# 1fni/cuda-spmv-benchmark

Hardware: AMD Instinct MI355X
Metric: cg_iterations_per_second (higher is better)
Workload: dtype f64; 1 GPU; CG on the 20000x20000 5-point stencil (400000000 unknowns, 1999920000 nnz), b=1, x0=0, tol 1e-6; grid=20000, unknowns=400000000, nnz=1999920000, partition=1 row slab(s), transport=single rank (no communicator), converged=True

## Files before the change

### cuda-spmv-benchmark_amd/binding.py

```python
import ctypes as C
import os
import subprocess

import numpy as np

PKG_DIR = os.path.dirname(os.path.abspath(__file__))
LAB_LIB_PATH = os.path.join(PKG_DIR, "lib", "libspmv_amd_lab.so")
LIB_PATH = os.environ.get("SPMV_AMD_LIB") or os.path.join(PKG_DIR, "lib", "libspmv_amd.so")
if LIB_PATH == "lab":
    LIB_PATH = LAB_LIB_PATH

ENTRY_DTYPE = np.dtype([("row", np.int32), ("col", np.int32), ("value", np.float64)], align=True)
assert ENTRY_DTYPE.itemsize == 16
COMM_ID_BYTES = 256


class MatrixData(C.Structure):
    _fields_ = [("rows", C.c_int), ("cols", C.c_int), ("nnz", C.c_int), ("grid_size", C.c_int), ("entries", C.c_void_p)]


class CSRMatrix(C.Structure):
    _fields_ = [("nb_rows", C.c_int), ("nb_cols", C.c_int), ("nb_nonzeros", C.c_int), ("row_ptr", C.POINTER(C.c_int)), ("col_indices", C.POINTER(C.c_int)), ("values", C.POINTER(C.c_double))]


class ELLPACKMatrix(C.Structure):
    _fields_ = [("nb_rows", C.c_int), ("nb_cols", C.c_int), ("ell_width", C.c_int), ("grid_size", C.c_int), ("indices", C.POINTER(C.c_int)), ("nb_nonzeros", C.c_int), ("values", C.POINTER(C.c_double))]


INIT_FN = C.CFUNCTYPE(C.c_int, C.POINTER(MatrixData))
RUN_TIMED_FN = C.CFUNCTYPE(C.c_int, C.c_void_p, C.c_void_p, C.POINTER(C.c_double))
RUN_DEVICE_FN = C.CFUNCTYPE(C.c_int, C.c_void_p, C.c_void_p)
FREE_FN = C.CFUNCTYPE(None)


class SpmvOperator(C.Structure):
    _fields_ = [("name", C.c_char_p), ("init", INIT_FN), ("run_timed", RUN_TIMED_FN), ("run_device", RUN_DEVICE_FN), ("free", FREE_FN)]


class BenchmarkStats(C.Structure):
    _fields_ = [("median_ms", C.c_double), ("mean_ms", C.c_double), ("std_dev_ms", C.c_double), ("min_ms", C.c_double), ("max_ms", C.c_double), ("valid_runs", C.c_int), ("outliers_removed", C.c_int)]


class CGConfig(C.Structure):
    _fields_ = [("max_iters", C.c_int), ("tolerance", C.c_double), ("verbose", C.c_int), ("enable_detailed_timers", C.c_int)]


class CGStats(C.Structure):
    _fields_ = [("iterations", C.c_int), ("residual_norm", C.c_double), ("time_total_ms", C.c_double), ("time_spmv_ms", C.c_double), ("time_blas1_ms", C.c_double), ("time_reductions_ms", C.c_double), ("converged", C.c_int), ("solution_sum", C.c_double), ("solution_norm", C.c_double)]


CGConfigMultiGPU = CGConfig


class CGStatsMultiGPU(C.Structure):
    _fields_ = [
        ("iterations", C.c_int), ("residual_norm", C.c_double), ("time_total_ms", C.c_double), ("time_spmv_ms", C.c_double),
        ("time_blas1_ms", C.c_double), ("time_reductions_ms", C.c_double), ("time_allreduce_ms", C.c_double),
        ("time_allgather_ms", C.c_double), ("converged", C.c_int), ("time_dot_rs_initial_ms", C.c_double),
        ("time_dot_pAp_ms", C.c_double), ("time_dot_rs_new_ms", C.c_double), ("time_axpy_update_x_ms", C.c_double),
        ("time_axpy_update_r_ms", C.c_double), ("time_axpby_update_p_ms", C.c_double), ("time_initial_r_ms", C.c_double),
        ("solution_sum", C.c_double), ("solution_norm", C.c_double),
    ]


class PcgScalars(C.Structure):
    _fields_ = [("rz", C.c_double), ("pAp", C.c_double), ("alpha", C.c_double), ("beta", C.c_double), ("b_norm", C.c_double),
                ("residual", C.c_double), ("iterations", C.c_int), ("converged", C.c_int), ("breakdown", C.c_int), ("skip_update", C.c_int)]


class PcgStageArgs(C.Structure):
    _fields_ = [("n", C.c_size_t), ("b", C.c_void_p), ("Ap", C.c_void_p), ("dinv", C.c_void_p), ("r", C.c_void_p), ("p", C.c_void_p),
                ("x", C.c_void_p), ("partials", C.c_void_p), ("count", C.c_int), ("which", C.c_int), ("tol", C.c_double),
                ("hist", C.c_void_p), ("hist_cap", C.c_int)]


class MultiColumn(C.Structure):
    _fields_ = [("rr_old", C.c_double), ("pAp", C.c_double), ("alpha", C.c_double), ("beta", C.c_double), ("b_norm", C.c_double),
                ("residual", C.c_double), ("active", C.c_int), ("done", C.c_int), ("iterations", C.c_int), ("pad", C.c_int)]


class CgMultiStageArgs(C.Structure):
    _fields_ = [("mode", C.c_char_p), ("n", C.c_size_t), ("X", C.c_void_p), ("R", C.c_void_p), ("P", C.c_void_p), ("AP", C.c_void_p),
                ("cols", C.c_void_p), ("partials", C.c_void_p), ("count", C.c_longlong), ("which", C.c_int), ("tol", C.c_double),
                ("hist", C.c_void_p), ("hist_cap", C.c_int), ("xcd_run", C.c_int)]


HALO_FN = C.CFUNCTYPE(C.c_int, C.c_void_p, C.POINTER(C.c_double), C.POINTER(C.c_double), C.POINTER(C.c_double), C.POINTER(C.c_double), C.c_int)
ALLREDUCE_FN = C.CFUNCTYPE(C.c_int, C.c_void_p, C.POINTER(C.c_double), C.c_int)
GATHER_FN = C.CFUNCTYPE(C.c_int, C.c_void_p, C.POINTER(C.c_double), C.c_int, C.POINTER(C.c_double), C.POINTER(C.c_int), C.POINTER(C.c_int))
BARRIER_FN = C.CFUNCTYPE(C.c_int, C.c_void_p)

DECLARED_SYMBOLS = [
    "csr_mat", "ellpack_matrix", "build_ellpack_from_csr_local", "ensure_ellpack_structure_built", "get_operator",
    "calculate_spmv_metrics", "get_gpu_properties", "print_benchmark_metrics", "print_metrics_json", "print_metrics_csv",
    "read_matrix_type", "read_matrix_general", "read_matrix_symtogen", "load_matrix_market", "convert_csr_to_ellpack",
    "write_matrix_market_stencil5", "benchmark_with_stats", "cg_benchmark_with_stats_device",
    "cg_benchmark_with_stats_mgpu_partitioned", "export_cg_json", "export_cg_mgpu_json", "export_cg_csv",
    "spmv_amd_build_csr_struct", "spmv_amd_build_ellpack_from_csr_struct", "spmv_amd_cg_solve", "spmv_amd_cg_solve_device",
    "spmv_amd_cg_solve_mgpu_partitioned", "spmv_amd_reset_host_matrices", "spmv_amd_interior_csr_offset",
    "spmv_amd_partition_rows", "spmv_amd_device_count", "spmv_amd_set_device", "spmv_amd_current_device", "spmv_amd_stream_ceiling", "spmv_amd_stream_ceiling_mix", "spmv_amd_device_alloc", "spmv_amd_device_free",
    "spmv_amd_copy_to_device", "spmv_amd_copy_to_host", "spmv_amd_device_fill_f64", "spmv_amd_device_synchronize",
    "spmv_amd_init_stencil5_synthetic", "spmv_amd_ellpack_run_device_scaled", "spmv_amd_download_device_csr", "spmv_amd_time_run_device", "spmv_amd_operator_variant",
    "spmv_amd_operator_select_variant", "spmv_amd_cg_last_history", "spmv_amd_comm_unique_id", "spmv_amd_comm_create_rccl",
    "spmv_amd_comm_create_staged", "spmv_amd_comm_destroy", "spmv_amd_comm_set_world", "spmv_amd_comm_rank", "spmv_amd_comm_size", "spmv_amd_comm_selftest",
    "spmv_amd_comm_barrier", "spmv_amd_comm_transport", "spmv_amd_comm_transport_ranks",
    "spmv_amd_comm_mailbox_enable", "spmv_amd_comm_mailbox_prepare", "spmv_amd_comm_mailbox_connect", "spmv_amd_comm_mailbox_selftest",
    "spmv_amd_comm_mailbox_disable", "spmv_amd_comm_mailbox_ready",
    "spmv_amd_cg_slab_create", "spmv_amd_cg_slab_create_stencil5", "spmv_amd_cg_slab_set_vectors", "spmv_amd_cg_slab_solve",
    "spmv_amd_cg_slab_gather", "spmv_amd_cg_slab_loop_shape", "spmv_amd_cg_slab_history", "spmv_amd_cg_slab_spmv", "spmv_amd_cg_slab_info",
    "spmv_amd_cg_slab_time_spmv", "spmv_amd_cg_slab_set_timeline", "spmv_amd_operator_placement", "spmv_amd_cg_slab_placement", "spmv_amd_cg_slab_tile_runs", "spmv_amd_cg_slab_setup_ms", "spmv_amd_cg_slab_coefficient_form", "spmv_amd_cg_slab_uniform_tiles", "spmv_amd_cg_slab_spmv_launch_ms",  "spmv_amd_cg_release_workspace", "spmv_amd_cg_slab_timeline_names", "spmv_amd_cg_slab_timeline", "spmv_amd_cg_slab_variant", "spmv_amd_cg_slab_destroy", "spmv_amd_version", "spmv_amd_write_stencil5_values",
    "spmv_amd_blas1_axpy", "spmv_amd_blas1_axpby", "spmv_amd_blas1_axpy_dev", "spmv_amd_blas1_update_p_dev", "spmv_amd_blas1_dot",
    "spmv_amd_cg_fused_step",
    "spmv_amd_spmm_device", "spmv_amd_spmm_variant", "spmv_amd_block_to_device", "spmv_amd_block_to_host",
    "spmv_amd_cg_solve_device_multi", "spmv_amd_cg_last_history_multi", "spmv_amd_cg_multi_workspace_bytes",
    "spmv_amd_precond_create", "spmv_amd_precond_create_from_diagonal", "spmv_amd_precond_destroy", "spmv_amd_precond_kind",
    "spmv_amd_precond_inverse_diagonal", "spmv_amd_pcg_solve_device", "spmv_amd_pcg_last_history", "spmv_amd_pcg_release_workspace",
    "spmv_amd_precond_create_chebyshev", "spmv_amd_precond_chebyshev_info", "spmv_amd_precond_apply_device",
]
LAB_ONLY_SYMBOLS = ["spmv_amd_cg_slab_create_stencil5_as", "spmv_amd_cg_slab_set_option", "spmv_amd_cg_slab_tile_classes", "spmv_amd_cg_slab_block_map", "spmv_amd_pcg_stage",
                    "spmv_amd_pcg_last_step_launches", "spmv_amd_cg_multi_stage"]
DECLARED_CXX_SYMBOLS = [
    "SPMV_CSR", "SPMV_STENCIL5_CSR", "SPMV_STENCIL_HALO_MGPU", "SPMV_ELLPACK", "SPMV_STENCIL5_ELLPACK",
    "_Z16build_csr_structP10MatrixData",
    "_Z29build_ellpack_from_csr_structPK9CSRMatrixP13ELLPACKMatrixPi",
    "_Z8cg_solveP12SpmvOperatorP10MatrixDataPKdPd8CGConfigP7CGStats",
    "_Z15cg_solve_deviceP12SpmvOperatorP10MatrixDataPKdPd8CGConfigP7CGStats",
    "_Z25cg_solve_mgpu_partitionedP12SpmvOperatorP10MatrixDataPKdPd16CGConfigMultiGPUP15CGStatsMultiGPU",
]


def build(force=False):
    if force:
        subprocess.check_call(["make", "-C", PKG_DIR, "clean"], stdout=subprocess.DEVNULL)
    done = subprocess.run(["make", "-C", PKG_DIR, "-j8"], stdout=subprocess.PIPE, stderr=subprocess.STDOUT, text=True)
    if done.returncode != 0:
        raise RuntimeError(f"building libspmv_amd.so failed (make exit {done.returncode}); compiler output:\n{done.stdout[-8000:]}")
    for path in (LIB_PATH, LAB_LIB_PATH):
        if not os.path.exists(path):
            raise RuntimeError(f"{os.path.basename(path)} was not produced by the build")


_lib = None


def lib():
    global _lib
    if _lib is not None:
        return _lib
    if not os.path.exists(LIB_PATH):
        raise RuntimeError(f"{LIB_PATH} is missing: run `python -c 'import __graft_entry__ as g; g.build()'` (needs hipcc)")
    L = C.CDLL(LIB_PATH)
    L.get_operator.restype = C.POINTER(SpmvOperator)
    L.get_operator.argtypes = [C.c_char_p]
    L.spmv_amd_version.restype = C.c_char_p
    L.spmv_amd_operator_variant.restype = C.c_char_p
    L.spmv_amd_operator_variant.argtypes = [C.c_char_p]
    L.spmv_amd_operator_select_variant.argtypes = [C.c_char_p, C.c_char_p]
    L.spmv_amd_device_alloc.restype = C.c_void_p
    L.spmv_amd_device_alloc.argtypes = [C.c_size_t]
    L.spmv_amd_device_free.argtypes = [C.c_void_p]
    L.spmv_amd_blas1_axpy.argtypes = [C.c_size_t, C.c_double, C.c_void_p, C.c_void_p]
    L.spmv_amd_blas1_axpby.argtypes = [C.c_size_t, C.c_double, C.c_void_p, C.c_double, C.c_void_p, C.c_void_p]
    L.spmv_amd_blas1_axpy_dev.argtypes = [C.c_size_t, C.c_double, C.c_void_p, C.c_void_p, C.c_int]
    L.spmv_amd_blas1_update_p_dev.argtypes = [C.c_size_t, C.c_void_p, C.c_double, C.c_void_p]
    L.spmv_amd_blas1_dot.argtypes = [C.c_size_t, C.c_void_p, C.c_void_p, C.POINTER(C.c_double)]
    L.spmv_amd_cg_fused_step.argtypes = [C.c_int, C.c_size_t, C.POINTER(C.c_double), C.c_void_p, C.c_void_p, C.c_void_p, C.c_int, C.POINTER(C.c_double)]
    L.spmv_amd_current_device.argtypes = [C.c_char_p, C.c_int]
    L.spmv_amd_stream_ceiling.restype = C.c_double
    L.spmv_amd_stream_ceiling.argtypes = [C.c_size_t, C.c_int, C.c_int, C.POINTER(C.c_float)]
    L.spmv_amd_stream_ceiling_mix.restype = C.c_double
    L.spmv_amd_stream_ceiling_mix.argtypes = [C.c_int, C.c_size_t, C.c_int, C.c_int, C.POINTER(C.c_float)]
    L.spmv_amd_copy_to_device.argtypes = [C.c_void_p, C.c_void_p, C.c_size_t]
    L.spmv_amd_copy_to_host.argtypes = [C.c_void_p, C.c_void_p, C.c_size_t]
    L.spmv_amd_device_fill_f64.argtypes = [C.c_void_p, C.c_size_t, C.c_double]
    L.spmv_amd_init_stencil5_synthetic.argtypes = [C.c_char_p, C.c_int]
    L.spmv_amd_download_device_csr.argtypes = [C.c_char_p, C.c_void_p, C.c_void_p, C.c_void_p]
    L.spmv_amd_ellpack_run_device_scaled.argtypes = [C.c_char_p, C.c_void_p, C.c_void_p, C.c_double, C.c_double]
    L.spmv_amd_time_run_device.argtypes = [C.c_char_p, C.c_void_p, C.c_void_p, C.c_int, C.POINTER(C.c_float)]
    L.spmv_amd_cg_solve.argtypes = [C.POINTER(SpmvOperator), C.POINTER(MatrixData), C.c_void_p, C.c_void_p, C.POINTER(CGConfig), C.POINTER(CGStats)]
    L.spmv_amd_cg_solve_device.argtypes = L.spmv_amd_cg_solve.argtypes
    L.spmv_amd_cg_solve_mgpu_partitioned.argtypes = [C.POINTER(MatrixData), C.c_void_p, C.c_void_p, C.POINTER(CGConfig), C.POINTER(CGStatsMultiGPU)]
    L.spmv_amd_cg_last_history.argtypes = [C.c_void_p, C.c_int]
    L.spmv_amd_comm_unique_id.argtypes = [C.c_void_p]
    L.spmv_amd_comm_create_rccl.restype = C.c_void_p
    L.spmv_amd_comm_create_rccl.argtypes = [C.c_int, C.c_int, C.c_void_p]
    L.spmv_amd_comm_create_staged.restype = C.c_void_p
    L.spmv_amd_comm_create_staged.argtypes = [C.c_int, C.c_int, HALO_FN, ALLREDUCE_FN, GATHER_FN, BARRIER_FN, C.c_void_p]
    L.spmv_amd_comm_destroy.argtypes = [C.c_void_p]
    L.spmv_amd_comm_set_world.argtypes = [C.c_void_p]
    L.spmv_amd_comm_rank.argtypes = [C.c_void_p]
    L.spmv_amd_comm_size.argtypes = [C.c_void_p]
    L.spmv_amd_comm_selftest.argtypes = [C.c_void_p]
    L.spmv_amd_comm_barrier.argtypes = [C.c_void_p]
    L.spmv_amd_comm_mailbox_enable.argtypes = [C.c_void_p]
    L.spmv_amd_comm_mailbox_prepare.argtypes = [C.c_void_p, C.c_void_p]
    L.spmv_amd_comm_mailbox_connect.argtypes = [C.c_void_p, C.c_void_p, C.c_int]
    L.spmv_amd_comm_mailbox_selftest.argtypes = [C.c_void_p, C.c_int]
    L.spmv_amd_comm_mailbox_disable.argtypes = [C.c_void_p]
    L.spmv_amd_comm_mailbox_ready.argtypes = [C.c_void_p]
    L.spmv_amd_comm_transport.restype = C.c_char_p
    L.spmv_amd_comm_transport.argtypes = [C.c_void_p]
    L.spmv_amd_comm_transport_ranks.argtypes = [C.c_void_p]
    if hasattr(L, "spmv_amd_cg_slab_create_stencil5_as"):
        L.spmv_amd_cg_slab_create_stencil5_as.restype = C.c_void_p
        L.spmv_amd_cg_slab_create_stencil5_as.argtypes = [C.c_int, C.c_int, C.c_int, C.c_void_p]
        L.spmv_amd_cg_slab_set_option.argtypes = [C.c_void_p, C.c_char_p, C.c_longlong]
        L.spmv_amd_cg_slab_set_option.restype = C.c_int
        L.spmv_amd_cg_slab_tile_classes.argtypes = [C.c_void_p, C.c_void_p, C.c_longlong]
        L.spmv_amd_cg_slab_tile_classes.restype = C.c_longlong
        L.spmv_amd_cg_slab_block_map.argtypes = [C.c_void_p, C.c_int, C.c_void_p, C.c_longlong]
        L.spmv_amd_cg_slab_block_map.restype = C.c_longlong
        L.spmv_amd_pcg_stage.argtypes = [C.c_char_p, C.c_char_p, C.POINTER(PcgStageArgs), C.POINTER(PcgScalars)]
        L.spmv_amd_pcg_stage.restype = C.c_int
        L.spmv_amd_pcg_last_step_launches.argtypes = []
        L.spmv_amd_pcg_last_step_launches.restype = C.c_int
        L.spmv_amd_cg_multi_stage.argtypes = [C.c_char_p, C.c_int, C.POINTER(CgMultiStageArgs)]
        L.spmv_amd_cg_multi_stage.restype = C.c_int
    L.spmv_amd_cg_slab_create.restype = C.c_void_p
    L.spmv_amd_cg_slab_create.argtypes = [C.POINTER(MatrixData), C.c_void_p]
    L.spmv_amd_cg_slab_create_stencil5.restype = C.c_void_p
    L.spmv_amd_cg_slab_create_stencil5.argtypes = [C.c_int, C.c_void_p]
    L.spmv_amd_cg_slab_set_vectors.argtypes = [C.c_void_p, C.c_void_p, C.c_void_p]
    L.spmv_amd_cg_slab_solve.argtypes = [C.c_void_p, C.POINTER(CGConfig), C.POINTER(CGStatsMultiGPU)]
    L.spmv_amd_cg_slab_gather.argtypes = [C.c_void_p, C.c_void_p]
    L.spmv_amd_cg_slab_history.argtypes = [C.c_void_p, C.c_void_p, C.c_int]
    L.spmv_amd_cg_slab_spmv.argtypes = [C.c_void_p, C.c_void_p, C.c_void_p]
    L.spmv_amd_cg_slab_info.argtypes = [C.c_void_p, C.POINTER(C.c_int), C.POINTER(C.c_int), C.POINTER(C.c_int)]
    L.spmv_amd_cg_slab_time_spmv.argtypes = [C.c_void_p, C.c_int, C.POINTER(C.c_float)]
    L.spmv_amd_cg_slab_destroy.argtypes = [C.c_void_p]
    L.spmv_amd_cg_slab_set_timeline.argtypes = [C.c_void_p, C.c_int]
    L.spmv_amd_cg_slab_set_timeline.restype = None
    L.spmv_amd_cg_slab_timeline_names.restype = C.c_char_p
    L.spmv_amd_cg_slab_timeline.argtypes = [C.c_void_p, C.c_void_p, C.c_int]
    L.spmv_amd_cg_slab_variant.restype = C.c_char_p
    L.spmv_amd_cg_slab_variant.argtypes = [C.c_void_p]
    L.spmv_amd_cg_slab_coefficient_form.argtypes = [C.c_void_p]
    L.spmv_amd_cg_slab_coefficient_form.restype = C.c_int
    L.spmv_amd_cg_slab_uniform_tiles.argtypes = [C.c_void_p, C.POINTER(C.c_longlong), C.POINTER(C.c_longlong)]
    L.spmv_amd_cg_slab_uniform_tiles.restype = C.c_int
    L.spmv_amd_cg_slab_loop_shape.restype = C.c_char_p
    L.spmv_amd_cg_slab_loop_shape.argtypes = [C.c_void_p]
    L.load_matrix_market.argtypes = [C.c_char_p, C.POINTER(MatrixData)]
    L.write_matrix_market_stencil5.argtypes = [C.c_int, C.c_char_p]
    L.spmv_amd_write_stencil5_values.argtypes = [C.c_int, C.c_char_p, C.c_char_p, C.c_char_p]
    L.read_matrix_type.argtypes = [C.c_char_p]
    L.spmv_amd_partition_rows.argtypes = [C.c_int, C.c_int, C.c_int, C.POINTER(C.c_int), C.POINTER(C.c_int)]
    L.benchmark_with_stats.argtypes = [RUN_TIMED_FN, C.c_void_p, C.c_void_p, C.c_int, C.POINTER(BenchmarkStats)]
    _lib = L
    return L


def is_lab():
    return hasattr(lib(), "spmv_amd_cg_slab_set_option")


def use_lab():
    import importlib.util

    spec = importlib.util.spec_from_file_location("spmv_amd_binding_lab", os.path.abspath(__file__))
    mod = importlib.util.module_from_spec(spec)
    spec.loader.exec_module(mod)
    mod.LIB_PATH = LAB_LIB_PATH
    return mod


def require_gpu():
    if lib().spmv_amd_device_count() < 1:
        raise RuntimeError("no HIP device visible: libspmv_amd has no CPU path")


def current_device():
    buf = C.create_string_buffer(64)
    dev = lib().spmv_amd_current_device(buf, 64)
    return dev, buf.value.decode()


def stream_ceiling(rows, warmup=3, reps=20, mix="stencil5"):
    require_gpu()
    ms = (C.c_float * reps)()
    nbytes = lib().spmv_amd_stream_ceiling_mix({"stencil5": 0, "csr": 1, "ellpack": 2, "read-only": 3}[mix], int(rows), int(warmup), int(reps), ms)
    if nbytes <= 0:
        raise RuntimeError("spmv_amd_stream_ceiling failed")
    return np.array(ms[:], dtype=np.float64), nbytes


def csr_mat():
    return CSRMatrix.in_dll(lib(), "csr_mat")


def ellpack_matrix():
    return ELLPACKMatrix.in_dll(lib(), "ellpack_matrix")


class HostMatrix:

    def __init__(self, entries, rows, cols, grid_size=-1):
        self.entries = np.ascontiguousarray(entries, dtype=ENTRY_DTYPE)
        self.c = MatrixData(int(rows), int(cols), len(self.entries), int(grid_size), self.entries.ctypes.data)

    @property
    def ptr(self):
        return C.byref(self.c)


def load_matrix_market(path):
    m = MatrixData()
    rc = lib().load_matrix_market(os.fsencode(path), C.byref(m))
    if rc != 0:
        raise IOError(f"load_matrix_market({path}) -> {rc}")
    e = np.ctypeslib.as_array((C.c_byte * (16 * m.nnz)).from_address(m.entries)).view(ENTRY_DTYPE).copy()
    C.CDLL(None).free(C.c_void_p(m.entries))
    return HostMatrix(e, m.rows, m.cols, m.grid_size)


def read_matrix_symtogen(path):
    m = MatrixData()
    rows, cols, nnz, full = C.c_int(), C.c_int(), C.c_int(), C.c_int()
    rp, ci, va = C.POINTER(C.c_int)(), C.POINTER(C.c_int)(), C.POINTER(C.c_double)()
    lib().read_matrix_symtogen(C.byref(m), os.fsencode(path), C.byref(rows), C.byref(cols), C.byref(nnz), C.byref(rp), C.byref(ci),
                               C.byref(va), C.byref(full))
    if not m.entries:
        raise IOError(f"read_matrix_symtogen({path}) failed")
    out = (rows.value, cols.value, nnz.value, full.value, np.ctypeslib.as_array(rp, shape=(rows.value + 1,)).copy(),
           np.ctypeslib.as_array(ci, shape=(full.value,)).copy(), np.ctypeslib.as_array(va, shape=(full.value,)).copy(),
           np.ctypeslib.as_array((C.c_byte * (16 * m.nnz)).from_address(m.entries)).view(ENTRY_DTYPE).copy())
    libc = C.CDLL(None)
    for ptr in (rp, ci, va, C.c_void_p(m.entries)):
        libc.free(ptr)
    return out


def host_csr_arrays():
    m = csr_mat()
    rp = np.ctypeslib.as_array(m.row_ptr, shape=(m.nb_rows + 1,)).copy()
    ci = np.ctypeslib.as_array(m.col_indices, shape=(m.nb_nonzeros,)).copy()
    va = np.ctypeslib.as_array(m.values, shape=(m.nb_nonzeros,)).copy()
    return rp, ci, va


def host_ell_arrays():
    m = ellpack_matrix()
    n = m.nb_rows * m.ell_width
    return m.ell_width, np.ctypeslib.as_array(m.indices, shape=(n,)).copy(), np.ctypeslib.as_array(m.values, shape=(n,)).copy()


def partition_rows(n, world, rank):
    off, nl = C.c_int(), C.c_int()
    lib().spmv_amd_partition_rows(n, world, rank, C.byref(off), C.byref(nl))
    return off.value, nl.value


class DeviceVector:
    def __init__(self, count, fill=None):
        self.count = int(count)
        self.ptr = lib().spmv_amd_device_alloc(self.count * 8)
        if fill is not None:
            lib().spmv_amd_device_fill_f64(self.ptr, self.count, float(fill))

    @classmethod
    def from_host(cls, a):
        a = np.ascontiguousarray(a, dtype=np.float64)
        v = cls(len(a))
        lib().spmv_amd_copy_to_device(v.ptr, a.ctypes.data, a.nbytes)
        return v
# ... 346 lines not shown
                    t = torch.zeros(counts[r], dtype=torch.float64)
                    dist.recv(t, r)
                    out[displs[r]:displs[r] + counts[r]] = t.numpy()
            else:
                dist.send(mine, 0)
            return 0

        def barrier_cb(user):
            dist.barrier()
            return 0

        return cls.staged(rank, world, halo_cb, allreduce_cb, gather_cb, barrier_cb)

    def selftest(self):
        return lib().spmv_amd_comm_selftest(self.handle)

    def barrier(self):
        return lib().spmv_amd_comm_barrier(self.handle)

    def mailbox_enable(self):
        return lib().spmv_amd_comm_mailbox_enable(self.handle) == 1

    def mailbox_prepare(self):
        buf = C.create_string_buffer(64)
        return buf.raw if lib().spmv_amd_comm_mailbox_prepare(self.handle, buf) == 0 else None

    def mailbox_connect(self, handles):
        blob = b"".join(handles)
        return lib().spmv_amd_comm_mailbox_connect(self.handle, C.create_string_buffer(blob, len(blob)), len(handles)) == 0

    def mailbox_selftest(self, rounds=8):
        return lib().spmv_amd_comm_mailbox_selftest(self.handle, int(rounds))

    def mailbox_ready(self):
        return lib().spmv_amd_comm_mailbox_ready(self.handle) == 1

    def mailbox_disable(self):
        lib().spmv_amd_comm_mailbox_disable(self.handle)

    def transport(self):
        return lib().spmv_amd_comm_transport(self.handle).decode()

    def transport_ranks(self):
        return lib().spmv_amd_comm_transport_ranks(self.handle)

    @classmethod
    def staged(cls, rank, world, halo, allreduce, gather=None, barrier=None):
        cbs = (HALO_FN(halo), ALLREDUCE_FN(allreduce), GATHER_FN(gather) if gather else GATHER_FN(), BARRIER_FN(barrier) if barrier else BARRIER_FN())
        h = lib().spmv_amd_comm_create_staged(rank, world, cbs[0], cbs[1], cbs[2], cbs[3], None)
        if not h:
            raise RuntimeError("spmv_amd_comm_create_staged failed")
        return cls(h, cbs)

    @staticmethod
    def unique_id():
        buf = C.create_string_buffer(COMM_ID_BYTES)
        lib().spmv_amd_comm_unique_id(buf)
        return buf.raw

    def destroy(self):
        if self.handle:
            lib().spmv_amd_comm_destroy(self.handle)
            self.handle = None


class CgSlab:

    def __init__(self, handle, n_rows):
        if not handle:
            raise RuntimeError("spmv_amd_cg_slab_create failed")
        self.h = handle
        self.n_rows = n_rows
        off, nl, nz = C.c_int(), C.c_int(), C.c_int()
        lib().spmv_amd_cg_slab_info(self.h, C.byref(off), C.byref(nl), C.byref(nz))
        self.row_offset, self.n_local, self.local_nnz = off.value, nl.value, nz.value

    @classmethod
    def from_matrix(cls, host_matrix, comm=None):
        require_gpu()
        return cls(lib().spmv_amd_cg_slab_create(host_matrix.ptr, comm.handle if comm else None), host_matrix.c.rows)

    @classmethod
    def stencil5(cls, n, comm=None):
        require_gpu()
        return cls(lib().spmv_amd_cg_slab_create_stencil5(int(n), comm.handle if comm else None), n * n)

    @classmethod
    def stencil5_as(cls, n, as_rank, as_world, comm):
        require_gpu()
        if not is_lab():
            raise RuntimeError("stand-in slabs exist in the LAB build only (binding.use_lab(), lib/libspmv_amd_lab.so)")
        return cls(lib().spmv_amd_cg_slab_create_stencil5_as(int(n), int(as_rank), int(as_world), comm.handle), n * n)

    def set_vectors(self, b=None, x0=None):
        b = None if b is None else np.ascontiguousarray(b, dtype=np.float64)
        x0 = None if x0 is None else np.ascontiguousarray(x0, dtype=np.float64)
        lib().spmv_amd_cg_slab_set_vectors(self.h, None if b is None else b.ctypes.data, None if x0 is None else x0.ctypes.data)

    def solve(self, max_iters=1000, tol=1e-6, verbose=0, timers=0):
        cfg = CGConfig(max_iters, tol, verbose, timers)
        st = CGStatsMultiGPU()
        rc = lib().spmv_amd_cg_slab_solve(self.h, C.byref(cfg), C.byref(st))
        if rc != 0:
            raise RuntimeError(f"cg_slab_solve -> {rc}")
        return st

    def history(self, cap=1001):
        h = np.zeros(cap, dtype=np.float64)
        count = lib().spmv_amd_cg_slab_history(self.h, h.ctypes.data, cap)
        return h[: min(count, cap)].copy()

    def gather(self):
        x = np.zeros(self.n_rows, dtype=np.float64)
        lib().spmv_amd_cg_slab_gather(self.h, x.ctypes.data)
        return x

    def spmv(self, x_full):
        x_full = np.ascontiguousarray(x_full, dtype=np.float64)
        y = np.zeros(self.n_local, dtype=np.float64)
        lib().spmv_amd_cg_slab_spmv(self.h, x_full.ctypes.data, y.ctypes.data)
        return y

    def variant(self):
        return lib().spmv_amd_cg_slab_variant(self.h).decode()

    def coefficient_form(self):
        return int(lib().spmv_amd_cg_slab_coefficient_form(self.h))

    def uniform_tiles(self):
        u, t = C.c_longlong(), C.c_longlong()
        lib().spmv_amd_cg_slab_uniform_tiles(self.h, C.byref(u), C.byref(t))
        return int(u.value), int(t.value)

    def tile_classes(self):
        if not is_lab():
            raise RuntimeError("the tile class map is read through the LAB build only (binding.use_lab(), lib/libspmv_amd_lab.so)")
        count = int(lib().spmv_amd_cg_slab_tile_classes(self.h, None, 0))
        if count == 0:
            return None
        out = np.zeros(count, dtype=np.uint8)
        lib().spmv_amd_cg_slab_tile_classes(self.h, out.ctypes.data, count)
        return out

    def block_map(self, which):
        if not is_lab():
            raise RuntimeError("the block maps are read through the LAB build only (binding.use_lab(), lib/libspmv_amd_lab.so)")
        count = int(lib().spmv_amd_cg_slab_block_map(self.h, int(which), None, 0))
        if count == 0:
            return None
        out = np.zeros(count, dtype=np.uint8)
        lib().spmv_amd_cg_slab_block_map(self.h, int(which), out.ctypes.data, count)
        return out

    def set_block_rows(self, rows):
        self.set_option("block_rows", rows)

    def loop_shape(self):
        return lib().spmv_amd_cg_slab_loop_shape(self.h).decode()

    def timeline_solve(self, max_iters=1000, tol=1e-6):
        lib().spmv_amd_cg_slab_set_timeline(self.h, 1)
        try:
            st = self.solve(max_iters=max_iters, tol=tol)
        finally:
            lib().spmv_amd_cg_slab_set_timeline(self.h, 0)
        names = lib().spmv_amd_cg_slab_timeline_names().decode().split(",")
        v = np.zeros(len(names), dtype=np.float64)
        count = lib().spmv_amd_cg_slab_timeline(self.h, v.ctypes.data, len(v))
        return st, ({k: float(x) for k, x in zip(names, v)} if count == len(names) else {})

    def placement(self):
        v = (C.c_double * 4)()
        lib().spmv_amd_cg_slab_placement.argtypes = [C.c_void_p, C.c_void_p, C.c_int]
        if lib().spmv_amd_cg_slab_placement(self.h, v, 4) != 4:
            return None
        return {"kind": "coefficient candidates", "candidates": int(v[1]), "spmv_ms_before": float(v[2]), "spmv_ms_kept": float(v[3])}

    def setup_ms(self):
        v = (C.c_double * 5)()
        lib().spmv_amd_cg_slab_setup_ms.argtypes = [C.c_void_p, C.c_void_p, C.c_int]
        lib().spmv_amd_cg_slab_setup_ms(self.h, v, 5)
        return dict(zip(("matrix_to_hbm", "streams_and_vectors", "verify_and_plans", "coefficient_placement", "tile_runs"), (float(x) for x in v)))

    def tile_runs(self):
        v = (C.c_double * 4)()
        lib().spmv_amd_cg_slab_tile_runs.argtypes = [C.c_void_p, C.c_void_p, C.c_int]
        if lib().spmv_amd_cg_slab_tile_runs(self.h, v, 4) != 4:
            return None
        return {"rule": int(v[0]), "kept": int(v[1]), "spmv_ms_rule": float(v[2]), "spmv_ms_kept": float(v[3])}

    def spmv_launch_ms(self):
        out = (C.c_float * 1024)()
        lib().spmv_amd_cg_slab_spmv_launch_ms.argtypes = [C.c_void_p, C.c_void_p, C.c_int]
        count = lib().spmv_amd_cg_slab_spmv_launch_ms(self.h, out, 1024)
        return np.array(out[:min(count, 1024)], dtype=np.float64)

    def set_option(self, name, value):
        if not is_lab():
            raise RuntimeError("slab options exist in the LAB build only (binding.use_lab(), lib/libspmv_amd_lab.so)")
        if lib().spmv_amd_cg_slab_set_option(self.h, name.encode(), int(value)) != 0:
            raise ValueError(f"unknown slab option {name!r}")

    def time_spmv(self, reps):
        ms = (C.c_float * reps)()
        lib().spmv_amd_cg_slab_time_spmv(self.h, reps, ms)
        return np.array(ms[:], dtype=np.float64)

    def destroy(self):
        if self.h:
            lib().spmv_amd_cg_slab_destroy(self.h)
            self.h = None
```

### cuda-spmv-benchmark_amd/csrc/cg_kernels.hip

```cpp
#include "kernels.hpp"

#include <stdlib.h>

#include "reduce_device.hpp"
#include "spmv_amd/hip_check.h"
#include "stream_device.hpp"

namespace spmv_amd {
namespace {

constexpr int kBlock = kReduceBlock;
constexpr int kStream = 64;

#define SPMV_AMD_STREAM_LOOP(n)                                                     \
    const size_t pairs = (n) >> 1;                                                  \
    const size_t i = (size_t)blockIdx.x * kStream + threadIdx.x;                    \
    if (i < pairs)

__device__ __forceinline__ void block_partial(double acc, double* __restrict__ partials) {
    acc = wave_sum(acc);
    if (threadIdx.x == 0) partials[blockIdx.x] = acc;
}

__global__ __launch_bounds__(kStream) void fill_kernel(double* __restrict__ d, size_t n, double value) {
    SPMV_AMD_STREAM_LOOP(n) {
        d2 v = {value, value};
        reinterpret_cast<d2*>(d)[i] = v;
    }
    if ((n & 1) && blockIdx.x == 0 && threadIdx.x == 0) d[n - 1] = value;
}

__global__ __launch_bounds__(kStream) void axpy_kernel(size_t n, double a, const double* __restrict__ x,
                                                      double* __restrict__ y) {
    SPMV_AMD_STREAM_LOOP(n) {
        const d2 xv = load_once(x, i);
        d2 yv = load_once(y, i);
        yv.x = fma(a, xv.x, yv.x);
        yv.y = fma(a, xv.y, yv.y);
        store_once(y, i, yv);
    }
    if ((n & 1) && blockIdx.x == 0 && threadIdx.x == 0) y[n - 1] = fma(a, x[n - 1], y[n - 1]);
}

__global__ __launch_bounds__(kStream) void axpby_kernel(size_t n, double a, const double* __restrict__ x,
                                                       double b, const double* y, double* z) {
    SPMV_AMD_STREAM_LOOP(n) {
        const d2 xv = load_once(x, i);
        const d2 yv = load_once(y, i);
        d2 zv;
        zv.x = fma(a, xv.x, b * yv.x);
        zv.y = fma(a, xv.y, b * yv.y);
        store_once(z, i, zv);
    }
    if ((n & 1) && blockIdx.x == 0 && threadIdx.x == 0) z[n - 1] = fma(a, x[n - 1], b * y[n - 1]);
}

template <bool kSubtract>
__global__ __launch_bounds__(kStream) void axpy_dev_kernel(size_t n, const double* __restrict__ d_a,
                                                          const double* __restrict__ x,
                                                          double* __restrict__ y) {
    const double a = kSubtract ? -(*d_a) : *d_a;
    SPMV_AMD_STREAM_LOOP(n) {
        const d2 xv = load_once(x, i);
        d2 yv = load_once(y, i);
        yv.x = fma(a, xv.x, yv.x);
        yv.y = fma(a, xv.y, yv.y);
        store_once(y, i, yv);
    }
    if ((n & 1) && blockIdx.x == 0 && threadIdx.x == 0) y[n - 1] = fma(a, x[n - 1], y[n - 1]);
}

__global__ __launch_bounds__(kStream) void update_p_dev_kernel(size_t n, const double* __restrict__ r,
                                                              const double* __restrict__ d_b,
                                                              double* __restrict__ p) {
    const double b = *d_b;
    SPMV_AMD_STREAM_LOOP(n) {
        const d2 rv = load_once(r, i);
        d2 pv = load_once(p, i);
        pv.x = fma(b, pv.x, rv.x);
        pv.y = fma(b, pv.y, rv.y);
        reinterpret_cast<d2*>(p)[i] = pv;
    }
    if ((n & 1) && blockIdx.x == 0 && threadIdx.x == 0) p[n - 1] = fma(b, p[n - 1], r[n - 1]);
}

__global__ __launch_bounds__(kStream) void dot_partials_kernel(size_t n, const double* __restrict__ x,
                                                              const double* __restrict__ y,
                                                              double* __restrict__ partials) {
    double acc = 0.0;
    SPMV_AMD_STREAM_LOOP(n) {
        const d2 xv = load_once(x, i);
        const d2 yv = load_once(y, i);
        acc = fma(xv.x, yv.x, acc);
        acc = fma(xv.y, yv.y, acc);
    }
    if ((n & 1) && blockIdx.x == 0 && threadIdx.x == 0) acc = fma(x[n - 1], y[n - 1], acc);
    block_partial(acc, partials);
}


__global__ __launch_bounds__(kBlock) void reduce_one_launch_kernel(const double* __restrict__ partials, int count, int slice,
                                                                   const double* extra, int extra_count, ReduceStage stage, ReduceTail tail) {
    __shared__ double s[kBlock];
    __shared__ int s_last;
    if (tail.skip_flag != nullptr && *tail.skip_flag != 0) {
        reduce_skipped(tail, blockIdx.x == 0);
        return;
    }
    reduce_slice_block(partials, count, slice, (int)blockIdx.x, (int)gridDim.x, reinterpret_cast<const unsigned long long*>(extra), extra_count,
                       (int)gridDim.x, stage, tail, s, &s_last);
}

__global__ __launch_bounds__(kBlock) void reduce_single_kernel(const double* __restrict__ partials, int count, const double* __restrict__ extra,
                                                               int extra_count, ReduceTail tail) {
    __shared__ double s[kBlock];
    if (tail.skip_flag != nullptr && *tail.skip_flag != 0) {
        reduce_skipped(tail, true);
        return;
    }
    block_tree(strided_sum(partials, 0, count), s);
    const double slice_sum = s[0];
    __syncthreads();
    reduce_finish(1 + extra_count, [&](int i) { return i == 0 ? slice_sum : extra[i - 1]; }, s, tail);
}

__global__ void scalar_divide_kernel(const double* num, const double* den, double* out) {
    if (threadIdx.x == 0 && blockIdx.x == 0) *out = (*num) / (*den);
}

__global__ void check_convergence_kernel(const double* rr_new, double b_norm, double tol,
                                         int* converged, double* residual) {
    if (threadIdx.x == 0 && blockIdx.x == 0) {
        *residual = sqrt(*rr_new);
        const double rel = (*residual) / b_norm;
        *converged = (rel < tol) ? 1 : 0;
    }
}


__global__ __launch_bounds__(kStream) void cg_init_residual_kernel(size_t n, const double* __restrict__ b,
                                                                  const double* __restrict__ Ap,
                                                                  double* __restrict__ r,
                                                                  double* __restrict__ p,
                                                                  double* __restrict__ partials) {
    double acc = 0.0;
    SPMV_AMD_STREAM_LOOP(n) {
        const d2 bv = load_once(b, i);
        const d2 av = load_once(Ap, i);
        d2 rv;
        rv.x = fma(-1.0, av.x, bv.x);
        rv.y = fma(-1.0, av.y, bv.y);
        store_once(r, i, rv);
        reinterpret_cast<d2*>(p)[i] = rv;
        acc = fma(rv.x, rv.x, acc);
        acc = fma(rv.y, rv.y, acc);
    }
    if ((n & 1) && blockIdx.x == 0 && threadIdx.x == 0) {
        const double rv = fma(-1.0, Ap[n - 1], b[n - 1]);
        r[n - 1] = rv;
        p[n - 1] = rv;
        acc = fma(rv, rv, acc);
    }
    block_partial(acc, partials);
}

__global__ __launch_bounds__(kStream) void cg_update_r_kernel(size_t n, const CgScalars* __restrict__ s,
                                                             const double* __restrict__ Ap,
                                                             double* __restrict__ r,
                                                             double* __restrict__ partials, int reverse) {
    const unsigned block = reverse ? gridDim.x - 1 - blockIdx.x : blockIdx.x;
    const size_t pairs = n >> 1;
    const size_t i = (size_t)block * kStream + threadIdx.x;
    d2 av = {0.0, 0.0}, rv = {0.0, 0.0};
    if (i < pairs) {
        av = load_once(Ap, i);
        rv = load_once(r, i);
    }
    const int converged = s->converged;
    const double rr_old = s->rr_old, pAp = s->pAp;
    if (converged) return;
    const double alpha = rr_old / pAp;
    double acc = 0.0;
    if (i < pairs) {
        rv.x = fma(-alpha, av.x, rv.x);
        rv.y = fma(-alpha, av.y, rv.y);
        store_once(r, i, rv);
        acc = fma(rv.x, rv.x, acc);
        acc = fma(rv.y, rv.y, acc);
    }
    if ((n & 1) && block == 0 && threadIdx.x == 0) {
        const double rl = fma(-alpha, Ap[n - 1], r[n - 1]);
        r[n - 1] = rl;
        acc = fma(rl, rl, acc);
    }
    acc = wave_sum(acc);
    if (threadIdx.x == 0) partials[block] = acc;
}

__device__ __forceinline__ double direction(double r, double beta, double p, int fma_form) {
    return fma_form ? fma(beta, p, r) : fma(1.0, r, beta * p);
}

__global__ __launch_bounds__(kStream) void cg_update_px_kernel(size_t n, const CgScalars* __restrict__ s,
                                                              const double* __restrict__ r,
                                                              double* __restrict__ p,
                                                              const double* x_in, double* x, int iteration,
                                                              int reverse, int fma_form) {
    if (s->iterations != iteration) return;
    const bool advance = s->converged == 0;
    const double alpha = s->alpha, beta = s->beta;
    const unsigned block = reverse ? gridDim.x - 1 - blockIdx.x : blockIdx.x;
    const size_t pairs = n >> 1;
    const size_t i = (size_t)block * kStream + threadIdx.x;
    if (i < pairs) {
        d2 pv = load_once(p, i);
        d2 xv = load_once(x_in, i);
        xv.x = fma(alpha, pv.x, xv.x);
        xv.y = fma(alpha, pv.y, xv.y);
        store_once(x, i, xv);
        if (advance) {
            const d2 rv = load_once(r, i);
            pv.x = direction(rv.x, beta, pv.x, fma_form);
            pv.y = direction(rv.y, beta, pv.y, fma_form);
            reinterpret_cast<d2*>(p)[i] = pv;
        }
    }
    if ((n & 1) && block == 0 && threadIdx.x == 0) {
        const double pv = p[n - 1];
        x[n - 1] = fma(alpha, pv, x_in[n - 1]);
        if (advance) p[n - 1] = direction(r[n - 1], beta, pv, fma_form);
    }
}

__global__ void cg_scalars_init_kernel(CgScalars* s, double* history) {
    if (threadIdx.x != 0 || blockIdx.x != 0) return;
    s->rr_old = s->rr_new;
    s->rr_ring[0] = s->rr_new;
    s->b_norm = sqrt(s->rr_new);
    s->residual = s->b_norm;
    s->converged = 0;
    s->iterations = 0;
    if (history != nullptr && s->max_history > 0) history[0] = s->b_norm;
}

__global__ void cg_scalars_step_kernel(CgScalars* s, double tol, double* history, int* host_record,
                                       int sequence, double* alpha_ring, int ring_slots) {
    if (threadIdx.x != 0 || blockIdx.x != 0) return;
    cg_scalars_step(s, tol, history, host_record, sequence, alpha_ring, ring_slots);
}

struct DirectionArgs {
    StepArgs step;
    int iteration;
    const double* r;
    const double* p_in;
    double* p_out;
    size_t bulk_lo, bulk_pairs;
    unsigned edge_blocks;
    int reverse, fma_form;
};
__global__ __launch_bounds__(kStream) void cg_direction_kernel(DirectionArgs a, EdgeRows e, ReduceStage stage) {
    CgScalars* s = a.step.scalars;
    const bool edge_block = blockIdx.x < a.edge_blocks;
    const size_t pairs_a = e.count_a >> 1, edge_pairs = (e.count_a + e.count_b) >> 1, shift = (e.second - e.count_a) >> 1;
    size_t at = 0;
    bool live_lane = false;
    if (edge_block) {
        const size_t i = (size_t)blockIdx.x * kStream + threadIdx.x;
        live_lane = i < edge_pairs;
        at = i < pairs_a ? i : i + shift;
    } else {
        const unsigned bulk_blocks = gridDim.x - a.edge_blocks, logical = blockIdx.x - a.edge_blocks;
        const size_t i = (size_t)(a.reverse ? bulk_blocks - 1 - logical : logical) * kStream + threadIdx.x;
        live_lane = i < a.bulk_pairs;
        at = (a.bulk_lo >> 1) + i;
    }
    const int was_converged = __hip_atomic_load(&s->converged, __ATOMIC_RELAXED, __HIP_MEMORY_SCOPE_AGENT);
    const double rr_new = s->rr_new, rr_prev = s->rr_ring[(a.iteration - 1) & 1], b_norm = s->b_norm;
    const int stop_at = cg_stop_at(s);
    if (blockIdx.x == 0 && threadIdx.x == 0 && a.step.host_record != nullptr)
        cg_scalars_step(s, a.step.tol, a.step.history, a.step.host_record, a.step.sequence, a.step.alpha_ring, a.step.ring_slots);
    const bool live = was_converged == 0 && !cg_converging(rr_new, b_norm, a.step.tol, stop_at, a.iteration);
    if (live && live_lane) {
        const double beta = rr_new / rr_prev;
        const d2 rv = load_once(a.r, at);
        d2 pv = load_once(a.p_in, at);
        pv.x = direction(rv.x, beta, pv.x, a.fma_form);
        pv.y = direction(rv.y, beta, pv.y, a.fma_form);
        if (edge_block) {
            __hip_atomic_store(reinterpret_cast<unsigned long long*>(a.p_out + 2 * at), (unsigned long long)__double_as_longlong(pv.x),
                               __ATOMIC_RELAXED, __HIP_MEMORY_SCOPE_AGENT);
            __hip_atomic_store(reinterpret_cast<unsigned long long*>(a.p_out + 2 * at + 1), (unsigned long long)__double_as_longlong(pv.y),
                               __ATOMIC_RELAXED, __HIP_MEMORY_SCOPE_AGENT);
        } else {
            reinterpret_cast<d2*>(a.p_out)[at] = pv;
        }
    }
    if (edge_block) {
        asm volatile("s_waitcnt vmcnt(0)" ::: "memory");
        if (threadIdx.x == 0) {
            const unsigned drawn = __hip_atomic_fetch_add(stage.ticket, 1u, __ATOMIC_RELAXED, __HIP_MEMORY_SCOPE_AGENT);
            if (drawn == a.edge_blocks - 1) {
                __hip_atomic_store(stage.ticket, 0u, __ATOMIC_RELAXED, __HIP_MEMORY_SCOPE_AGENT);
                __hip_atomic_store(stage.edges_ready, (unsigned)a.step.sequence, __ATOMIC_RELAXED, __HIP_MEMORY_SCOPE_AGENT);
            }
        }
    }
}

__global__ void edges_wait_kernel(const unsigned* ready, unsigned sequence, long long timeout_ticks, int* late) {
    if (threadIdx.x != 0 || blockIdx.x != 0) return;
    const long long t0 = wall_clock64();
    while ((int)(__hip_atomic_load(ready, __ATOMIC_RELAXED, __HIP_MEMORY_SCOPE_AGENT) - sequence) < 0) {
        if (wall_clock64() - t0 > timeout_ticks) {
            __hip_atomic_store(late, 3, __ATOMIC_RELAXED, __HIP_MEMORY_SCOPE_SYSTEM);
            break;
        }
        __builtin_amdgcn_s_sleep(8);
    }
}

__global__ __launch_bounds__(kStream) void cg_update_p_ring_kernel(size_t n, const CgScalars* __restrict__ s,
                                                                   const double* __restrict__ r,
                                                                   const double* __restrict__ p_in,
                                                                   double* __restrict__ p_out, int iteration,
                                                                   int reverse, int fma_form) {
    if (s->iterations != iteration || s->converged != 0) return;
    const double beta = s->beta;
    const unsigned block = reverse ? gridDim.x - 1 - blockIdx.x : blockIdx.x;
    const size_t pairs = n >> 1;
    const size_t i = (size_t)block * kStream + threadIdx.x;
    if (i < pairs) {
        const d2 rv = load_once(r, i);
        d2 pv = load_once(p_in, i);
        pv.x = direction(rv.x, beta, pv.x, fma_form);
        pv.y = direction(rv.y, beta, pv.y, fma_form);
        reinterpret_cast<d2*>(p_out)[i] = pv;
    }
    if ((n & 1) && block == 0 && threadIdx.x == 0) p_out[n - 1] = direction(r[n - 1], beta, p_in[n - 1], fma_form);
}

template <int K>
__device__ __forceinline__ void flush_chunk(d2& xv, const RingSlots& ring, const double* __restrict__ alphas, int slots,
                                            int& slot, size_t i) {
    d2 pv[K];
    double a[K];
#pragma unroll
    for (int u = 0; u < K; ++u) {
        const int sl = (slot + u) % slots;
        pv[u] = load_once(ring.p[sl], i);
        a[u] = alphas[sl];
    }
#pragma unroll
    for (int u = 0; u < K; ++u) {
// ... 207 lines not shown
```

### cuda-spmv-benchmark_amd/csrc/cg_slab.hip

```cpp
#include <math.h>
#include <stdlib.h>
#include <string.h>

#include <algorithm>
#include <atomic>
#include <chrono>
#include <mutex>
#include <thread>
#include <vector>

#include "comm.hpp"
#include "device_runtime.hpp"
#include "multi_rhs.hpp"
#include "solve_common.hpp"
#include "stencil_geometry.hpp"
#include "trace_ranges.hpp"
#include "watchdog.hpp"

using namespace spmv_amd;

namespace spmv_amd {
std::vector<double>& last_cg_history();
}

struct SpmvAmdCgSlab {
    SpmvAmdComm* comm = nullptr;
    int part_rank = 0, part_world = 1;
    SpmvOperator* op = nullptr;
    bool op_failed = false;
    FusedSpmv fused;
    const char* label = nullptr;
    bool device_form = false;
    int n = 0, grid = -1, row_offset = 0, n_local = 0, halo = 0;
    bool has_prev = false, has_next = false;
    DeviceCsr A;
    double *x = nullptr, *x0 = nullptr, *r = nullptr, *Ap = nullptr, *b = nullptr;
    double* x0_alloc = nullptr;
    double* vec_arena = nullptr;
    double* planes_alloc = nullptr;
    size_t planes_doubles = 0, planes_s_offset = 0;
    SymPlanes planes;
    bool planes_on = false;
    unsigned char* tile_classes = nullptr;
    size_t tile_class_count = 0;
    long long tiles_uniform = 0, tiles_total = 0;
    double quintuple[5] = {0.0, 0.0, 0.0, 0.0, 0.0};
    bool stream_everywhere = false;
    unsigned char *block_map_whole = nullptr, *block_map_interior = nullptr;
    bool spmv_with_dot = false;
    const SymPlanes* sym() const { return planes_on ? &planes : nullptr; }
    std::vector<double> placement;
    std::vector<double> tile_runs;
    double setup_ms[5] = {0.0, 0.0, 0.0, 0.0, 0.0};
    bool setup_trials = true;
    double* p_alloc = nullptr;
    double* p = nullptr;
    size_t slot_doubles = 0, slot_lead = 0;
    std::vector<double*> ring_alloc;
    std::vector<double*> ring;
    int ring_slots = 1;
    double* d_alpha_ring = nullptr;
    double* partials_spmv = nullptr;
    double* partials_blas = nullptr;
    double* reduce_stage = nullptr;
    ReduceScratch scratch() const { return ReduceScratch{reduce_stage}; }
    CgScalars* d_s = nullptr;
    double* d_hist = nullptr;
    int hist_cap = 0;
    struct Poll { int sequence; int converged; int iterations; int progress; int halo_late; }* h_poll = nullptr;
    unsigned* d_halo_flag = nullptr;
    unsigned halo_sequence = 0;
#ifdef SPMV_AMD_LAB
    int stop_at = 0;
    int test_wedge_overlapped_exchange = 0;
    bool guess_far_always = false;
#endif
    const PeerMailbox* reduce_mailbox = nullptr;
    int* spmv_progress = nullptr;
    int spmv_progress_value = 0;
    const char* enqueued_stage = "";
    int enqueued_iteration = -1;
    hipStream_t compute = nullptr, side = nullptr;
    bool owns_streams = true;
    hipEvent_t ev_p_ready = nullptr, ev_halo_done = nullptr;
    bool timeline_on = false;
    std::vector<hipEvent_t> tl_compute, tl_side;
    hipEvent_t tl_after_interior = nullptr;
    std::vector<double> timeline_us;
    LaunchShape shape;
    Stencil5Plan plan_whole, plan_interior, plan_head, plan_tail;
    int partials_cap = 0;
    int spmv_split_at = -1;
    const char* variant_name = "";
    bool fused_dot = false;
    bool fuse_init_residual = false;
    std::vector<double> history;
    std::vector<hipEvent_t> spmv_ev;
    int spmv_event_stride = 7;
    int spmv_event_phase = 0;
    bool roctx_always = false;
    bool no_overlap = false;
    bool selfcheck = false, selfcheck_late = false;
    double wait_limit_s = 0.0;
    bool late_bulk = false;
    bool late_predict = true;
    bool run_ahead = true;
    size_t lead_rows = (size_t)1 << 25;
    int poll_sequence = 0;
    double last_spmv_ms = 0.0;
    int last_spmv_launches = 0;
    std::vector<float> last_spmv_each;
};

namespace {
constexpr int kTimelineMarks = 7;
const char* const kTimelineNames =
    "iterations,solve_ms,initial_residual_us,spmv_interior_us,halo_wait_and_boundary_rows_us,reduce_pAp_and_allreduce_us,"
    "update_r_us,reduce_rr_allreduce_and_scalar_step_us,direction_update_us,gap_before_next_iteration_us,iteration_us,"
    "halo_exchange_on_side_stream_us,final_x_flush_us,direction_updates";
}

namespace {

void adopt_operator(SpmvAmdCgSlab* s, SpmvOperator* op) {
    s->op = op;
    s->fused = fused_spmv_of(op);
    s->fused_dot = s->fused.partials > 0;
    s->fuse_init_residual = s->fused_dot && s->fused.can_init;
    s->variant_name = s->fused_dot ? "operator/fused-launch" : "operator/run_device+dot";
    if (s->fused.partials > s->partials_cap) {
        device_release(s->partials_spmv);
        s->partials_cap = s->fused.partials;
        s->partials_spmv = device_alloc<double>((size_t)s->partials_cap);
        HIP_CHECK(hipMemset(s->partials_spmv, 0, (size_t)s->partials_cap * sizeof(double)));
    }
}

void place_coefficients(SpmvAmdCgSlab* s);
void tune_tile_runs(SpmvAmdCgSlab* s);

SymPlanes plane_view(const SpmvAmdCgSlab* s, const double* base) {
    SymPlanes v;
    v.ce = base;
    v.s = base + s->planes_s_offset;
    v.cls = s->stream_everywhere ? nullptr : s->tile_classes;
    v.w = s->quintuple[0], v.c = s->quintuple[1], v.e = s->quintuple[2], v.n = s->quintuple[3], v.s5 = s->quintuple[4];
    return v;
}

bool may_take_planes(const SpmvAmdCgSlab* s) {
    const int n = s->grid;
    return s->op == nullptr && n >= 2 && n >= s->shape.knobs.rowlds_min_grid && s->n_local > 0 && s->n_local % n == 0 &&
           s->row_offset % n == 0;
}

void classify_tiles(SpmvAmdCgSlab* s) {
    const int n = s->grid;
    const int gfirst = s->row_offset / n, rows = s->n_local / n;
    const int lo = std::max(gfirst, 1), hi = std::min(gfirst + rows, n - 1);
    if (hi <= lo || n < 3) return;
    const int col_tiles = rowlds_col_tiles(n);
    s->tiles_total = (long long)(hi - lo) * col_tiles;
    const long long lr = (long long)(lo + (hi - lo) / 2 - gfirst) * n + n / 2;
    int first = 0;
    HIP_CHECK(hipMemcpy(&first, s->A.view.row_ptr + lr, sizeof(int), hipMemcpyDeviceToHost));
    double row[5];
    HIP_CHECK(hipMemcpy(row, s->A.view.values + first, sizeof(row), hipMemcpyDeviceToHost));
    const double q[5] = {row[1], row[2], row[3], row[0], row[4]};
    memcpy(s->quintuple, q, sizeof(q));
    s->tile_class_count = (size_t)rows * col_tiles;
    const size_t bytes = s->tile_class_count;
    s->tile_classes = device_try_alloc<unsigned char>(bytes);
    if (s->tile_classes == nullptr) {
        s->tile_class_count = 0;
        return;
    }
    unsigned long long* d_count = device_alloc<unsigned long long>(1);
    HIP_CHECK(hipMemsetAsync(s->tile_classes, 0, bytes, s->compute));
    HIP_CHECK(hipMemsetAsync(d_count, 0, sizeof(unsigned long long), s->compute));
    launch_classify_tiles(s->A.view, q, s->tile_classes, d_count, s->compute);
    unsigned long long h_count = 0;
    HIP_CHECK(hipMemcpyAsync(&h_count, d_count, sizeof(h_count), hipMemcpyDeviceToHost, s->compute));
    HIP_CHECK(hipStreamSynchronize(s->compute));
    device_release(d_count);
    s->tiles_uniform = (long long)h_count;
}

void attach_block_maps(SpmvAmdCgSlab* s) {
    s->plan_whole.block_map = s->block_map_whole;
    s->plan_interior.block_map = s->block_map_interior;
}

void build_block_maps(SpmvAmdCgSlab* s) {
    HIP_CHECK(hipStreamSynchronize(s->compute));
    device_release(s->block_map_whole);
    device_release(s->block_map_interior);
    if (s->tile_classes != nullptr) {
        const auto map_of = [&](const Stencil5Plan& p) -> unsigned char* {
            const int blocks = rowlds_block_tiles(p);
            unsigned char* map = blocks > 0 ? device_try_alloc<unsigned char>((size_t)blocks) : nullptr;
            if (map != nullptr) launch_block_map(s->tile_classes, p, map, s->compute);
            return map;
        };
        s->block_map_whole = map_of(s->plan_whole);
        s->block_map_interior = map_of(s->plan_interior);
        HIP_CHECK(hipStreamSynchronize(s->compute));
    }
    attach_block_maps(s);
}

void settle_planes(SpmvAmdCgSlab* s) {
    if (s->planes_alloc == nullptr) return;
    bool keep = s->A.view.verified_stencil && s->fuse_init_residual;
    if (keep) {
        launch_fill_sym_planes(s->A.view, s->planes_alloc, s->planes_alloc + s->planes_s_offset, s->compute);
        s->planes = plane_view(s, s->planes_alloc);
        int* d_flag = device_alloc<int>(1);
        HIP_CHECK(hipMemsetAsync(d_flag, 0, sizeof(int), s->compute));
        launch_verify_sym_planes(s->A.view, s->planes, d_flag, s->compute);
        int h_flag = 1;
        HIP_CHECK(hipMemcpyAsync(&h_flag, d_flag, sizeof(int), hipMemcpyDeviceToHost, s->compute));
        HIP_CHECK(hipStreamSynchronize(s->compute));
        device_release(d_flag);
        keep = h_flag == 0;
    }
    if (!keep) {
        device_release(s->planes_alloc);
        s->planes = SymPlanes{};
    } else {
        classify_tiles(s);
        s->planes = plane_view(s, s->planes_alloc);
        build_block_maps(s);
    }
    s->planes_on = keep;
}

double setup_phase_ms(std::chrono::steady_clock::time_point& from) {
    HIP_CHECK(hipDeviceSynchronize());
    const auto now = std::chrono::steady_clock::now();
    const double ms = std::chrono::duration<double, std::milli>(now - from).count();
    from = now;
    return ms;
}

void make_common(SpmvAmdCgSlab* s) {
    const size_t nl = (size_t)s->n_local;
    auto phase = std::chrono::steady_clock::now();
    const bool whole_grid_probe = s->comm->self_neighbour && s->part_world == 1;
    s->has_prev = s->comm->exchanges_halos() && (s->part_rank > 0 || whole_grid_probe);
    s->has_next = s->comm->exchanges_halos() && (s->part_rank < s->part_world - 1 || whole_grid_probe);
    s->halo = s->comm->exchanges_halos() ? s->grid : 0;
    s->A.view.halo_before = s->has_prev ? s->halo : 0;
    s->A.view.halo_after = s->has_next ? s->halo : 0;
    if (s->op != nullptr) {
        s->compute = nullptr;
        s->side = nullptr;
        s->owns_streams = false;
    } else {
        HIP_CHECK(hipStreamCreateWithFlags(&s->compute, hipStreamNonBlocking));
        HIP_CHECK(hipStreamCreateWithFlags(&s->side, hipStreamNonBlocking));
    }
    HIP_CHECK(hipEventCreateWithFlags(&s->ev_p_ready, hipEventDisableTiming));
    HIP_CHECK(hipEventCreateWithFlags(&s->ev_halo_done, hipEventDisableTiming));
    s->shape = current_launch_shape();
    constexpr size_t kLeadUnit = 512;
    const size_t lead = s->halo == 0 ? 0 : ((size_t)s->halo + kLeadUnit - 1) / kLeadUnit * kLeadUnit;
    const size_t slot_doubles = lead + nl + (size_t)s->halo + 2;
    s->slot_doubles = slot_doubles;
    s->slot_lead = lead;
    s->x = device_alloc<double>(nl);
    s->b = device_alloc<double>(nl);
    s->x0_alloc = device_alloc<double>(slot_doubles);
    s->x0 = s->x0_alloc + lead;
    HIP_CHECK(hipMemset(s->x0_alloc, 0, slot_doubles * sizeof(double)));
    {
        int want = kMaxRingSlots;
        const char* forced = getenv("SPMV_AMD_P_RING");
        if (forced) want = atoi(forced);
        want = want < 1 ? 1 : (want > kMaxRingSlots ? kMaxRingSlots : want);
        constexpr size_t k2MiB = (size_t)2 << 20, k4KiB = 4096;
        const size_t pitch = ((slot_doubles * sizeof(double) + k2MiB - 1) / k2MiB * k2MiB + k4KiB) / sizeof(double);
        size_t free_b = 0, total_b = 0;
        HIP_CHECK(hipMemGetInfo(&free_b, &total_b));
        const size_t keep_free = (size_t)4 << 30;
        const size_t per_slot = pitch * sizeof(double);
        const int asked = want;
        const size_t fixed = 3 * per_slot;
        if (may_take_planes(s)) {
            const size_t ce = (2 * nl + kLeadUnit - 1) / kLeadUnit * kLeadUnit;
            const size_t halo_lead = ((size_t)s->grid + kLeadUnit - 1) / kLeadUnit * kLeadUnit;
            const size_t bytes = (ce + halo_lead + nl) * sizeof(double);
            if (free_b > bytes + keep_free + fixed + 3 * per_slot) {
                s->planes_alloc = device_try_alloc<double>(ce + halo_lead + nl);
                if (s->planes_alloc != nullptr) {
                    s->planes_doubles = ce + halo_lead + nl;
                    s->planes_s_offset = ce + halo_lead;
                    HIP_CHECK(hipMemGetInfo(&free_b, &total_b));
                }
            }
        }
        const size_t budget = s->op != nullptr ? free_b / 4 : (free_b > keep_free + fixed ? free_b - keep_free - fixed : 0);
        while (want > 1 && (size_t)(want - 1) * per_slot > budget) --want;
        if (want < asked && want < 4) want = 1;
        s->vec_arena = device_alloc<double>((size_t)(2 + want) * pitch);
        HIP_CHECK(hipMemset(s->vec_arena, 0, (size_t)(2 + want) * pitch * sizeof(double)));
        s->r = s->vec_arena;
        s->Ap = s->vec_arena + pitch;
        s->ring_alloc.clear();
        s->ring.clear();
        for (int k = 0; k < want; ++k) {
            double* a = s->vec_arena + (size_t)(2 + k) * pitch;
            s->ring_alloc.push_back(a);
            s->ring.push_back(a + lead);
        }
        s->p_alloc = s->ring_alloc[0];
        s->p = s->ring[0];
        s->ring_slots = want;
        s->d_alpha_ring = device_alloc<double>(kMaxRingSlots);
        HIP_CHECK(hipMemset(s->d_alpha_ring, 0, kMaxRingSlots * sizeof(double)));
    }
    if (const char* v = getenv("SPMV_AMD_NO_OVERLAP")) s->no_overlap = v[0] == '1';
#ifdef SPMV_AMD_LAB
    if (const char* v = getenv("SPMV_AMD_TEST_WEDGE_OVERLAPPED_EXCHANGE")) s->test_wedge_overlapped_exchange = atoi(v);
#endif
    if (const char* v = getenv("SPMV_AMD_ROCTX")) s->roctx_always = v[0] == '1';
    s->late_bulk = nl >= 100000000;
    s->partials_blas = device_alloc<double>(dot_scratch_doubles(nl));
    HIP_CHECK(hipMemset(s->partials_blas, 0, dot_scratch_doubles(nl) * sizeof(double)));
    s->reduce_stage = reduce_scratch_alloc();
    s->d_halo_flag = device_alloc<unsigned>(1);
    HIP_CHECK(hipMemset(s->d_halo_flag, 0, sizeof(unsigned)));
    s->d_s = device_alloc<CgScalars>(1);
    HIP_CHECK(hipMemset(s->d_s, 0, sizeof(CgScalars)));
    HIP_CHECK(hipHostMalloc((void**)&s->h_poll, sizeof(*s->h_poll), hipHostMallocCoherent | hipHostMallocMapped));
    memset(s->h_poll, 0, sizeof(*s->h_poll));
    if (s->op != nullptr) {
        adopt_operator(s, s->op);
        launch_fill(s->b, nl, 1.0, s->compute);
        launch_fill(s->x0, nl, 0.0, s->compute);
        HIP_CHECK(hipDeviceSynchronize());
        return;
    }
    s->setup_ms[1] = setup_phase_ms(phase);
    s->A.verify_stencil(s->compute);
    {
        const SlabCsr& A = s->A.view;
        const int lo = s->has_prev ? s->halo : 0, hi = s->n_local - (s->has_next ? s->halo : 0);
        const auto plan = [&](int a, int b) { return plan_stencil5(A, a, b > a ? b : a, Stencil5Variant::Auto, s->shape); };
        s->plan_whole = plan(0, s->n_local);
        s->plan_interior = plan(lo, hi);
        s->plan_head = plan(0, lo);
        s->plan_tail = plan(hi, s->n_local);
        const int whole = s->plan_whole.partials;
        const int split = (hi > lo ? s->plan_interior.partials : 0) + (lo > 0 ? s->plan_head.partials : 0) +
                          (hi < s->n_local ? s->plan_tail.partials : 0);
        s->partials_cap = whole > split ? whole : split;
        s->partials_spmv = device_alloc<double>((size_t)s->partials_cap);
        HIP_CHECK(hipMemset(s->partials_spmv, 0, (size_t)s->partials_cap * sizeof(double)));
        s->variant_name = s->plan_whole.name;
        s->fused_dot = s->plan_whole.variant != Stencil5Variant::RowGeneric;
        const auto rowlds = [&](const Stencil5Plan& p) { return p.last_row <= p.first_row || p.variant == Stencil5Variant::RowLds; };
        s->fuse_init_residual = s->plan_whole.variant == Stencil5Variant::RowLds && rowlds(s->plan_interior) && rowlds(s->plan_head) && rowlds(s->plan_tail);
    }
    settle_planes(s);
    s->setup_ms[2] = setup_phase_ms(phase);
    if (s->setup_trials) place_coefficients(s);
    s->setup_ms[3] = setup_phase_ms(phase);
    if (s->setup_trials) tune_tile_runs(s);
    launch_fill(s->b, nl, 1.0, s->compute);
    launch_fill(s->x0, nl, 0.0, s->compute);
    s->setup_ms[4] = setup_phase_ms(phase);
}

bool wants_coefficient_placement(size_t n_local) { return n_local >= ((size_t)16 << 20) && placement_candidates() > 1; }

void place_coefficients(SpmvAmdCgSlab* s) {
    const size_t nl = (size_t)s->n_local;
    if (s->op != nullptr || !wants_coefficient_placement(nl) || s->ring.size() < 4 || s->A.values == nullptr) return;
    hipStream_t q = s->compute;
    const bool nothing_streamed = s->planes_on && s->tiles_total > 0 && s->tiles_uniform == s->tiles_total && !s->stream_everywhere;
    const bool planes = s->planes_on;
    const size_t count = planes ? s->planes_doubles : (size_t)s->A.view.nnz_local;
    const double* early = s->ring[1];
    const double* late = s->ring[s->ring.size() - 3];
    launch_fill(s->ring[1], nl, 1.0, q);
    launch_fill(s->ring[s->ring.size() - 3], nl, 1.0, q);
    HIP_CHECK(hipMemsetAsync(&s->d_s->converged, 0, sizeof(int), q));
    EventTimer timer;
    double* const original = planes ? s->planes_alloc : s->A.values;
    const auto point_at = [&](double* values) {
        if (planes) s->planes = plane_view(s, values);
        else s->A.view.values = values;
    };
    auto cost = [&](double* values) {
        point_at(values);
        double total = 0.0;
        for (const double* x : {early, late}) {
            float ms[3];
            for (int i = 0; i < 4; ++i) {
                timer.begin(q);
                (void)launch_stencil5_spmv(s->A.view, s->plan_whole, x, s->Ap, 1.0, s->fused_dot ? s->partials_spmv : nullptr, nullptr, false, q,
                                           nullptr, s->sym());
                timer.end(q);
                const float t = timer.elapsed_ms();
                if (i > 0) ms[i - 1] = t;
            }
            std::sort(ms, ms + 3);
            total += ms[1];
        }
        point_at(original);
        return 0.5 * total;
    };
    int tried = 0;
    double before = 0.0, after = 0.0;
    double* best = device_alloc_best_of<double>(count, 0, [&](double* cand) {
        if (cand != original && !nothing_streamed) HIP_CHECK(hipMemcpyAsync(cand, original, count * sizeof(double), hipMemcpyDeviceToDevice, q));
        const double ms = cost(cand);
        if (cand == original) before = ms;
        return ms;
    }, &tried, nullptr, original, false);
    after = best == original ? before : cost(best);
    HIP_CHECK(hipStreamSynchronize(q));
    const bool moved = best != original && after < 0.99 * before;
    if (moved && nothing_streamed) {
        HIP_CHECK(hipMemcpyAsync(best, original, count * sizeof(double), hipMemcpyDeviceToDevice, q));
        HIP_CHECK(hipStreamSynchronize(q));
    }
    if (best != original) {
        if (!moved) device_release(best);
        else if (planes) device_release(s->planes_alloc), s->planes_alloc = best;
        else s->A.replace_values(best);
    }
    s->A.view.values = s->A.values;
    if (planes) s->planes = plane_view(s, s->planes_alloc);
    for (double* a : s->ring_alloc) HIP_CHECK(hipMemsetAsync(a, 0, s->slot_doubles * sizeof(double), q));
    HIP_CHECK(hipStreamSynchronize(q));
    s->placement = {0.0, (double)tried, before, moved ? after : before};
}

void tune_tile_runs(SpmvAmdCgSlab* s) {
    if (s->op != nullptr || s->ring.size() < 2) return;
    const size_t nl = (size_t)s->n_local;
    hipStream_t q = s->compute;
    double* x = s->ring[1];
    launch_fill(x, nl, 1.0, q);
    HIP_CHECK(hipMemsetAsync(&s->d_s->converged, 0, sizeof(int), q));
    double rec[4] = {0, 0, 0, 0};
    const int run = tune_rowlds_xcd_run(s->A.view, s->shape, x, s->Ap, s->fused_dot ? s->partials_spmv : nullptr, q, rec, s->sym(),
                                        s->plan_whole.block_map);
    HIP_CHECK(hipMemsetAsync(s->ring_alloc[1], 0, s->slot_doubles * sizeof(double), q));
    HIP_CHECK(hipStreamSynchronize(q));
    if (run <= 0) return;
    s->shape.knobs.rowlds_group = run;
    const int lo = s->has_prev ? s->halo : 0, hi = s->n_local - (s->has_next ? s->halo : 0);
    const auto plan = [&](int a, int b) { return plan_stencil5(s->A.view, a, b > a ? b : a, Stencil5Variant::Auto, s->shape); };
    s->plan_whole = plan(0, s->n_local);
    s->plan_interior = plan(lo, hi);
    s->plan_head = plan(0, lo);
    s->plan_tail = plan(hi, s->n_local);
    attach_block_maps(s);
    s->tile_runs.assign(rec, rec + 4);
}

double halo_wait_limit_s(const SpmvAmdCgSlab* s) {
    if (s->wait_limit_s > 0.0) return s->wait_limit_s;
    const double w = watchdog_limit_seconds();
    return w > 0.0 && w < 40.0 ? 0.5 * w : 20.0;
}

bool partition_ok(const SpmvAmdComm* comm, int n, int grid, int n_local) {
    if (!comm->exchanges_halos()) return true;
    if (grid <= 0) {
        fprintf(stderr, "[cg-slab] multi-GPU solve needs a stencil matrix (grid_size > 0)\n");
        return false;
    }
    if (n_local < grid) {
        fprintf(stderr, "[cg-slab] slab of %d rows is thinner than one grid row (%d)\n", n_local, grid);
        return false;
    }
    (void)n;
    return true;
}

int slab_boundary_spmv(SpmvAmdCgSlab* s, const double* in, double* part, const int* skip, hipStream_t stream,
                       const ResidualOut* init = nullptr) {
    const SlabCsr& A = s->A.view;
    const int lo = s->has_prev ? s->halo : 0;
    const int hi = s->n_local - (s->has_next ? s->halo : 0);
    double* at = part ? part + (hi > lo ? s->plan_interior.partials : 0) : nullptr;
    int used = 0;
    if (lo > 0 && hi < s->n_local && lo == A.grid_size && s->n_local - hi == A.grid_size) {
        used += launch_stencil5_spmv_first_and_last_gridrow(A, s->plan_head, s->plan_tail, in, s->Ap, 1.0, at, skip, stream, init, s->sym());
    } else {
        if (lo > 0) used += launch_stencil5_spmv(A, s->plan_head, in, s->Ap, 1.0, at, skip, false, stream, init, s->sym());
        if (hi < s->n_local)
            used += launch_stencil5_spmv(A, s->plan_tail, in, s->Ap, 1.0, at ? at + used : nullptr, skip, false, stream, init, s->sym());
    }
    return part ? used : 0;
}

void reduce_spmv_partials(SpmvAmdCgSlab* s, int used, double* d_out, const int* skip, int* progress, int progress_value, const PeerMailbox* mailbox) {
    const int first = s->spmv_split_at >= 0 && s->spmv_split_at < used ? s->spmv_split_at : used;
    launch_reduce_partials(s->partials_spmv, first, d_out, skip, s->compute, s->scratch(), progress, progress_value, mailbox,
                           s->partials_spmv + first, used - first);
}

int slab_spmv(SpmvAmdCgSlab* s, bool with_dot, bool overlap, const int* skip,
              const double* input = nullptr, hipEvent_t spmv_done = nullptr, const ResidualOut* init = nullptr) {
    const SlabCsr& A = s->A.view;
    const double* in = input ? input : s->p;
    double* part = ((with_dot && s->fused_dot) || init) ? s->partials_spmv : nullptr;
    const int lo = s->has_prev ? s->halo : 0;
    const int hi = s->n_local - (s->has_next ? s->halo : 0);
    int used = 0;
    s->spmv_split_at = -1;
    if (s->op != nullptr) {
        if (part != nullptr) {
            used = s->fused.launch(in, s->Ap, part, skip, s->shape.reverse, init, s->compute);
        } else if (s->op->run_device(in, s->Ap) != 0) {
            fprintf(stderr, "[cg] operator '%s': run_device failed\n", s->op->name);
            s->op_failed = true;
        }
        if (s->tl_after_interior) HIP_CHECK(hipEventRecord(s->tl_after_interior, s->compute));
    } else if (hi <= lo || (lo == 0 && hi == s->n_local) || (part == nullptr && !overlap)) {
        if (overlap) HIP_CHECK(hipStreamWaitEvent(s->compute, s->ev_halo_done, 0));
        used = launch_stencil5_spmv(A, s->plan_whole, in, s->Ap, 1.0, part, skip, s->shape.reverse, s->compute, init, s->sym());
        if (s->tl_after_interior) HIP_CHECK(hipEventRecord(s->tl_after_interior, s->compute));
    } else {
        used = launch_stencil5_spmv(A, s->plan_interior, in, s->Ap, 1.0, part, skip, s->shape.reverse, s->compute, init, s->sym());
        s->spmv_split_at = used;
        if (s->tl_after_interior) HIP_CHECK(hipEventRecord(s->tl_after_interior, s->compute));
        const bool fused_tail = with_dot && part != nullptr && init == nullptr && lo % A.grid_size == 0 &&
                                (s->n_local - hi) % A.grid_size == 0 && lo <= A.grid_size && s->n_local - hi <= A.grid_size;
        if (fused_tail && spmv_done) HIP_CHECK(hipEventRecord(spmv_done, s->compute));
        HaloArrival arrival;
        if (fused_tail && overlap) {
            arrival = HaloArrival{s->d_halo_flag, s->halo_sequence, (long long)(halo_wait_limit_s(s) * 1e8), &s->h_poll->halo_late};
        } else if (overlap) {
            HIP_CHECK(hipStreamWaitEvent(s->compute, s->ev_halo_done, 0));
        }
        if (fused_tail && launch_stencil5_edges_and_reduce(A, s->plan_interior, lo > 0, hi < s->n_local, in, s->Ap, 1.0, part, &s->d_s->pAp, skip,
                                                           s->scratch(), s->spmv_progress, s->spmv_progress_value, s->reduce_mailbox, s->compute,
                                                           arrival, s->sym())) {
            return used;
        }
        if (arrival.flag != nullptr) HIP_CHECK(hipStreamWaitEvent(s->compute, s->ev_halo_done, 0));
        if (fused_tail) spmv_done = nullptr;
        used += slab_boundary_spmv(s, in, part, skip, s->compute, init);
    }
    if (spmv_done) HIP_CHECK(hipEventRecord(spmv_done, s->compute));
    if (with_dot) {
        if (part)
            reduce_spmv_partials(s, used, &s->d_s->pAp, skip, s->spmv_progress, s->spmv_progress_value, s->reduce_mailbox);
        else
            launch_dot((size_t)s->n_local, s->p, s->Ap, s->partials_blas, &s->d_s->pAp, s->compute);
    }
    return used;
}

const char* query_name(hipError_t e) {
    return e == hipSuccess ? "idle (all work done)" : e == hipErrorNotReady ? "busy (work pending)" : hipGetErrorString(e);
}

void report_slab_state(void* user, FILE* out) {
    const SpmvAmdCgSlab* s = static_cast<const SpmvAmdCgSlab*>(user);
    const int seq = __atomic_load_n(&s->h_poll->sequence, __ATOMIC_ACQUIRE);
    const int prog = __atomic_load_n(&s->h_poll->progress, __ATOMIC_ACQUIRE);
    fprintf(out, "[cg-slab] rank %d (slab %d of %d, rows [%d, %d)): last work enqueued by the host: %s of iteration %d\n",
            s->comm->rank, s->part_rank, s->part_world, s->row_offset, s->row_offset + s->n_local, s->enqueued_stage,
            s->enqueued_iteration);
    fprintf(out, "[cg-slab] status records: waiting for #%d, GPU has published #%d (iterations counted %d, converged %d)\n",
            s->poll_sequence, seq, s->h_poll->iterations, s->h_poll->converged);
    const char* where = "before the local p.Ap sum: in the SpMV, or waiting for the halo rows (see the events below)";
    if (prog == 4 * s->poll_sequence + 1)
        where = "local p.Ap summed: in the all-reduce of p.Ap, the r update or the local r.r sum";
    else if (prog == 4 * s->poll_sequence + 2)
        where = "local r.r summed: in the all-reduce of r.r or the scalar step";
    if (seq != s->poll_sequence) fprintf(out, "[cg-slab] GPU progress inside that iteration: %s\n", where);
    fprintf(out, "[cg-slab] compute stream: %s; side (halo) stream: %s\n", query_name(hipStreamQuery(s->compute)),
            query_name(hipStreamQuery(s->side)));
    fprintf(out, "[cg-slab] event 'direction vector ready for the halo exchange': %s; event 'halo rows received': %s\n",
            query_name(hipEventQuery(s->ev_p_ready)), query_name(hipEventQuery(s->ev_halo_done)));
    s->comm->describe(out);
}

bool record_arrived(const SpmvAmdCgSlab* s, int sequence) {
    return (int)(__atomic_load_n(&s->h_poll->sequence, __ATOMIC_ACQUIRE) - sequence) >= 0;
}

void wait_for_record(SpmvAmdCgSlab* s, int sequence) {
    if (record_arrived(s, sequence)) return;
    WatchdogScope guard("waiting for the iteration's status record", s->comm->rank, s->enqueued_iteration,
                        report_slab_state, s);
    long spins = 0;
    while (!record_arrived(s, sequence)) {
        __builtin_ia32_pause();
        if (++spins % (1L << 20) == 0) {
            const hipError_t e = hipStreamQuery(s->compute);
            if (e != hipSuccess && e != hipErrorNotReady) HIP_CHECK(e);
            if (e == hipSuccess && !record_arrived(s, sequence)) {
                fprintf(stderr, "[cg-slab] status record missing after the stream drained\n");
                exit(EXIT_FAILURE);
            }
        }
    }
}

void exchange_halo(SpmvAmdCgSlab* s, double* v, hipStream_t stream) {
    if (!s->comm->exchanges_halos()) return;
    WatchdogScope guard("halo exchange (send/recv of the first and last grid row)", s->comm->rank, s->enqueued_iteration,
                        report_slab_state, s);
#ifdef SPMV_AMD_LAB
    while (s->test_wedge_overlapped_exchange == 1 && stream == s->side && s->side != nullptr) std::this_thread::sleep_for(std::chrono::milliseconds(200));
    if (s->test_wedge_overlapped_exchange == 2 && stream == s->side && s->side != nullptr) {
        static const double nudged = 1.001;
        HIP_CHECK(hipMemcpyAsync(s->b, &nudged, sizeof nudged, hipMemcpyHostToDevice, stream));
        s->test_wedge_overlapped_exchange = 0;
    }
    if (s->test_wedge_overlapped_exchange == 3 && stream == s->side && s->side != nullptr) return;
#endif
    s->comm->halo_exchange(s->has_prev ? v : nullptr, s->has_next ? v + (s->n_local - s->halo) : nullptr,
                           s->has_prev ? v - s->halo : nullptr, s->has_next ? v + s->n_local : nullptr, s->halo, stream);
}
void allreduce_scalar(SpmvAmdCgSlab* s, double* d_value, const char* stage) {
    if (s->comm->mailbox_ready()) {
        launch_mailbox_allreduce(s->comm, d_value, s->compute);
        return;
    }
    WatchdogScope guard(stage, s->comm->rank, s->enqueued_iteration, report_slab_state, s);
    s->comm->allreduce_sum(d_value, 1, s->compute);
}

}

namespace {
struct LoopShape {
    bool multi = false;
    bool reduce = false;
    bool separate = false;
    const PeerMailbox* mailbox = nullptr;
    bool detail = false;
    bool pipeline = false;
    bool late = false;
    int slots = 1;
    EdgeRows edges{0, 0, 0};
    size_t bulk_lo = 0, bulk_hi = 0;
};


LoopShape loop_shape(const SpmvAmdCgSlab* s, const CGConfigMultiGPU* config) {
    LoopShape L;
    const SpmvAmdComm* comm = s->comm;
    const size_t nl = (size_t)s->n_local;
    L.multi = comm->exchanges_halos();
    L.reduce = comm->collective();
    L.mailbox = (L.reduce && comm->mailbox_ready()) ? comm->d_mailbox : nullptr;
    L.separate = L.reduce && L.mailbox == nullptr;
    L.detail = config->enable_detailed_timers != 0;
    L.slots = s->ring_slots;
    L.late = s->late_bulk && !L.detail && L.slots > 1;
    constexpr size_t kAlign = 512;
    const size_t head_rows = s->has_prev ? ((size_t)s->halo + kAlign - 1) / kAlign * kAlign : 0;
    const size_t tail_start = s->has_next ? (nl - (size_t)s->halo) / kAlign * kAlign : nl;
    L.pipeline = L.multi && !L.detail && !s->no_overlap && L.slots > 1 && s->reduce_stage != nullptr && (nl % 2) == 0 &&
                 nl >= 4 * (size_t)s->halo + 4 * kAlign && head_rows < tail_start;
    if (L.pipeline) {
        L.edges = EdgeRows{head_rows, tail_start, nl - tail_start};
        L.bulk_lo = head_rows, L.bulk_hi = tail_start;
    } else {
        L.bulk_lo = 0, L.bulk_hi = nl;
    }
    return L;
}

void poison_halos(SpmvAmdCgSlab* s) {
    if (s->halo == 0 || s->op != nullptr) return;
    const size_t bytes = (size_t)s->halo * sizeof(double);
    auto both_sides = [&](double* local) {
        if (s->has_prev) HIP_CHECK(hipMemsetAsync(local - s->halo, 0xFF, bytes, s->compute));
        if (s->has_next) HIP_CHECK(hipMemsetAsync(local + s->n_local, 0xFF, bytes, s->compute));
    };
    both_sides(s->x0);
    for (double* local : s->ring) both_sides(local);
}

void verify_pipeline(SpmvAmdCgSlab* s) {
    SpmvAmdComm* comm = s->comm;
    if (s->op != nullptr || !comm->exchanges_halos()) return;
    if (s->no_overlap) return;
    const CGConfigMultiGPU few = {4, 0.0, 0, 0};
    const bool mine = loop_shape(s, &few).pipeline;
    if (comm->world == 1 && !mine) return;
    if (comm->pipeline_verdict == 0) {
        CGStatsMultiGPU st;
        s->selfcheck = true, s->selfcheck_late = false, s->wait_limit_s = 2.0;
        s->no_overlap = true;
        poison_halos(s);
        spmv_amd_cg_slab_solve(s, &few, &st);
        const std::vector<double> plain = s->history;
        s->no_overlap = false;
        poison_halos(s);
        spmv_amd_cg_slab_solve(s, &few, &st);
        poison_halos(s);
        HIP_CHECK(hipStreamSynchronize(s->compute));
        if (s->side) HIP_CHECK(hipStreamSynchronize(s->side));
        __atomic_store_n(&s->h_poll->halo_late, 0, __ATOMIC_RELEASE);
        bool finite = true;
        for (double v : plain) finite = finite && std::isfinite(v);
        if (!finite)
            fprintf(stderr, "[cg-slab] rank %d: the plain order's residual history is not finite in the creation check: the communicator's halo "
                            "exchange does not deliver this rank's neighbour rows (transport: %s)\n", comm->rank, comm->transport());
        const bool same = finite && !s->selfcheck_late && plain.size() == s->history.size() && plain.size() == 5 &&
                          memcmp(plain.data(), s->history.data(), plain.size() * sizeof(double)) == 0;
        s->selfcheck = false, s->selfcheck_late = false, s->wait_limit_s = 0.0;
        double votes[2] = {same ? 0.0 : 1.0, mine ? 1.0 : 0.0};
        if (!same)
            fprintf(stderr, "[cg-slab] rank %d: the overlapped pipeline did NOT reproduce the plain order's residual history in the creation check\n", comm->rank);
        if (comm->world > 1) {
            double* d = device_alloc<double>(2);
            upload(d, votes, 2);
            WatchdogScope guard("creation check: all-reduce of the ranks' verdicts", comm->rank, -1, report_slab_state, s);
            comm->allreduce_sum(d, 2, s->compute);
            HIP_CHECK(hipStreamSynchronize(s->compute));
            download(votes, d, 2);
            device_release(d);
        }
        if (votes[0] != 0.0 || votes[1] != 0.0) comm->pipeline_verdict = votes[0] == 0.0 ? 1 : -1;
        if (comm->pipeline_verdict < 0 && comm->rank == 0)
            fprintf(stderr, "[cg-slab] %g rank(s) refused the overlapped pipeline: every solve on this communicator runs the plain order "
                            "(halo exchange on the compute stream, the reference's own)\n", votes[0]);
    }
    if (comm->pipeline_verdict < 0) s->no_overlap = true;
}

SpmvAmdCgSlab* create_from_matrix(MatrixData* mat, SpmvAmdComm* comm, bool setup_trials) {
    if (comm == nullptr) comm = self_comm();
    if (mat->rows != mat->cols) {
        fprintf(stderr, "[cg-slab] CG needs a square matrix\n");
        return nullptr;
    }
    int row_offset = 0, n_local = 0;
    spmv_amd_partition_rows(mat->rows, comm->world, comm->rank, &row_offset, &n_local);
    if (!partition_ok(comm, mat->rows, mat->grid_size, n_local)) return nullptr;
    if (build_csr_struct(mat) != EXIT_SUCCESS) return nullptr;
    SpmvAmdCgSlab* s = new SpmvAmdCgSlab();
    s->comm = comm;
    s->part_rank = comm->rank;
    s->part_world = comm->world;
    s->n = mat->rows;
    s->grid = mat->grid_size;
    s->row_offset = row_offset;
    s->n_local = n_local;
    s->setup_trials = setup_trials;
    s->A.separate_values = setup_trials && wants_coefficient_placement((size_t)n_local);
    auto phase = std::chrono::steady_clock::now();
    s->A.upload_slab(csr_mat, row_offset, n_local, mat->grid_size);
    s->setup_ms[0] = setup_phase_ms(phase);
    make_common(s);
    verify_pipeline(s);
    return s;
}
}

extern "C" SpmvAmdCgSlab* spmv_amd_cg_slab_create(MatrixData* mat, SpmvAmdComm* comm) { return create_from_matrix(mat, comm, true); }

extern "C" const char* spmv_amd_cg_slab_loop_shape(const SpmvAmdCgSlab* s) {
    if (!s->comm->exchanges_halos()) return "single rank";
    if (!s->no_overlap) {
        const CGConfigMultiGPU any = {1, 0.0, 0, 0};
        if (!loop_shape(s, &any).pipeline) return "plain: the in-place form (ring 1) or a slab too thin to split";
        return s->comm->pipeline_verdict > 0 ? "pipeline (verified against the plain order at creation)" : "pipeline";
    }
    return s->comm->pipeline_verdict < 0 ? "plain: the pipeline's residual history differed from the plain order's in the creation check"
                                         : "plain: SPMV_AMD_NO_OVERLAP=1";
}

namespace {
SpmvAmdCgSlab* create_stencil5_slab(int n, int part_rank, int part_world, SpmvAmdComm* comm) {
    if (n < 2 || (long long)n * n > 0x7fffffffLL || 5LL * n * n - 4LL * n > 0x7fffffffLL) {
        fprintf(stderr, "[cg-slab] grid %d does not fit 32-bit CSR indices\n", n);
        return nullptr;
    }
    int row_offset = 0, n_local = 0;
    spmv_amd_partition_rows(n * n, part_world, part_rank, &row_offset, &n_local);
    if (!partition_ok(comm, n * n, n, n_local)) return nullptr;
    SpmvAmdCgSlab* s = new SpmvAmdCgSlab();
    s->comm = comm;
    s->part_rank = part_rank;
    s->part_world = part_world;
    s->n = n * n;
    s->grid = n;
    s->row_offset = row_offset;
    s->n_local = n_local;
    s->A.separate_values = wants_coefficient_placement((size_t)n_local);
    auto phase = std::chrono::steady_clock::now();
    s->A.generate_stencil5(n, row_offset, n_local, 5.0, -1.0, nullptr);
    s->setup_ms[0] = setup_phase_ms(phase);
    make_common(s);
    verify_pipeline(s);
    return s;
}
}

extern "C" SpmvAmdCgSlab* spmv_amd_cg_slab_create_stencil5(int n, SpmvAmdComm* comm) {
    if (comm == nullptr) comm = self_comm();
    return create_stencil5_slab(n, comm->rank, comm->world, comm);
}

#ifdef SPMV_AMD_LAB
extern "C" SpmvAmdCgSlab* spmv_amd_cg_slab_create_stencil5_as(int n, int as_rank, int as_world, SpmvAmdComm* comm) {
    if (comm == nullptr || comm->world != 1 || (as_world > 1 && !comm->self_neighbour)) {
        fprintf(stderr, "[cg-slab] a stand-in slab needs a single-rank self-neighbour communicator\n");
        return nullptr;
    }
    if (as_world < 1 || as_rank < 0 || as_rank >= as_world) return nullptr;
    return create_stencil5_slab(n, as_rank, as_world, comm);
}
#endif

extern "C" int spmv_amd_cg_slab_set_vectors(SpmvAmdCgSlab* s, const double* b_full,
                                            const double* x0_full) {
    if (b_full) upload(s->b, b_full + s->row_offset, (size_t)s->n_local);
    if (x0_full) upload(s->x0, x0_full + s->row_offset, (size_t)s->n_local);
    return 0;
}

namespace {

struct SolveRun {
    SpmvAmdCgSlab* s;
    const CGConfigMultiGPU* config;
    CGStatsMultiGPU* stats;
    const LoopShape L;
    const TraceRanges trace;
    EventTimer total, part;
    const size_t nl;
    const int* skip;
    const bool timeline;
    RingSlots ring_view;
    int window_start = 0;
    int tl_exchanges = 0;
    bool halo_in_flight = false;
    bool step_in_direction = false;
    int sequence0 = 0, records_read = 0;
    bool backward = false;
    int enqueued = 0, sampled = 0;
    std::vector<int> sampled_iteration;

    SolveRun(SpmvAmdCgSlab* slab, const CGConfigMultiGPU* cfg, CGStatsMultiGPU* st)
        : s(slab), config(cfg), stats(st), L(loop_shape(slab, cfg)), trace(L.detail || slab->roctx_always), nl((size_t)slab->n_local),
          skip(&slab->d_s->converged), timeline(slab->timeline_on && !L.detail) {
        for (int k = 0; k < kMaxRingSlots; ++k) ring_view.p[k] = s->ring[(size_t)k % s->ring.size()];
    }

    template <class Work>
    void timed(double* bucket, double* bucket2, Work&& work) {
        if (!L.detail) {
            work();
            return;
        }
        part.begin(s->compute);
        work();
        part.end(s->compute);
        WatchdogScope guard("detailed timers: waiting for the stage just enqueued", s->comm->rank, s->enqueued_iteration, report_slab_state, s);
        const double ms = part.elapsed_ms();
        if (bucket) *bucket += ms;
        if (bucket2) *bucket2 += ms;
    }
    static hipEvent_t tl_event(std::vector<hipEvent_t>& pool, size_t index) {
        while (pool.size() <= index) {
            hipEvent_t e;
            HIP_CHECK(hipEventCreate(&e));
            pool.push_back(e);
        }
        return pool[index];
    }
    size_t mark_index(int iteration, int k) const { return 2 + (size_t)iteration * kTimelineMarks + k; }
    void mark(int iteration, int k) {
        if (timeline) HIP_CHECK(hipEventRecord(tl_event(s->tl_compute, mark_index(iteration, k)), s->compute));
    }

    void begin();
    void initial_residual();
    void start_halo(double* v, bool released_by_flag);
    void stage_spmv();
    void stage_allreduce_pAp();
    void stage_update_r();
    void stage_sum_rr_and_step();
    void stage_direction_and_halo();
    bool far_from_convergence(int iteration, int basis) const;
    bool converged_at(int k) const;
    void await_record(int iteration);
    bool read_status();
    void finish();
    void resolve_timeline(const CgScalars& fin, float total_ms);
};

void SolveRun::begin() {
    s->reduce_mailbox = nullptr;
    s->op_failed = false;
    memset(stats, 0, sizeof(*stats));
    const int want_hist = config->max_iters < (1 << 20) ? config->max_iters + 1 : (1 << 20);
    if (s->hist_cap < want_hist) {
        if (s->d_hist) HIP_CHECK(hipHostFree(s->d_hist));
        s->hist_cap = want_hist;
        HIP_CHECK(hipHostMalloc((void**)&s->d_hist, (size_t)s->hist_cap * sizeof(double), hipHostMallocCoherent | hipHostMallocMapped));
    }
    CgScalars init;
    memset(&init, 0, sizeof init);
    init.max_history = s->hist_cap;
#ifdef SPMV_AMD_LAB
    init.stop_at = s->stop_at;
#endif
    HIP_CHECK(hipMemcpyAsync(s->d_s, &init, sizeof init, hipMemcpyHostToDevice, s->compute));
#ifdef SPMV_AMD_LAB
    poison_halos(s);
#endif
    HIP_CHECK(hipStreamSynchronize(s->compute));
    s->timeline_us.clear();
    s->p = s->ring[0];
    sequence0 = s->poll_sequence;
    records_read = 0;
    s->h_poll->converged = 0, s->h_poll->iterations = 0;
    s->enqueued_stage = "barrier before the timed region";
    s->enqueued_iteration = -1;
    {
        WatchdogScope guard("barrier before the timed region", s->comm->rank, -1, report_slab_state, s);
        s->comm->barrier(s->compute);
    }
    total.begin(s->compute);
    if (timeline) HIP_CHECK(hipEventRecord(tl_event(s->tl_compute, 0), s->compute));
}

void SolveRun::start_halo(double* v, bool released_by_flag) {
    if (!L.multi) return;
    if (!L.pipeline) {
        timed(&stats->time_allgather_ms, nullptr, [&] { exchange_halo(s, v, s->compute); });
        halo_in_flight = false;
        return;
    }
    if (released_by_flag) {
        launch_edges_wait(s->scratch(), s->poll_sequence, (long long)(halo_wait_limit_s(s) * 1e8), &s->h_poll->halo_late, s->side);
    } else {
        HIP_CHECK(hipEventRecord(s->ev_p_ready, s->compute));
        HIP_CHECK(hipStreamWaitEvent(s->side, s->ev_p_ready, 0));
    }
    const bool in_loop = v != s->x0;
    if (timeline && in_loop) HIP_CHECK(hipEventRecord(tl_event(s->tl_side, 2 * (size_t)tl_exchanges), s->side));
    exchange_halo(s, v, s->side);
    ++s->halo_sequence;
#ifdef SPMV_AMD_LAB
    if (s->test_wedge_overlapped_exchange != 4)
#endif
        launch_halo_arrived(s->d_halo_flag, s->halo_sequence, s->side);
    if (timeline && in_loop) HIP_CHECK(hipEventRecord(tl_event(s->tl_side, 2 * (size_t)tl_exchanges++ + 1), s->side));
    HIP_CHECK(hipEventRecord(s->ev_halo_done, s->side));
    halo_in_flight = true;
}

void SolveRun::initial_residual() {
    start_halo(s->x0, false);
    if (s->fuse_init_residual) {
        const ResidualOut init{s->b, s->r, s->p};
        int used = 0;
        timed(&stats->time_initial_r_ms, nullptr, [&] { used = slab_spmv(s, false, halo_in_flight, nullptr, s->x0, nullptr, &init); });
        timed(&stats->time_dot_rs_initial_ms, nullptr, [&] { reduce_spmv_partials(s, used, &s->d_s->rr_new, nullptr, nullptr, 0, L.mailbox); });
    } else {
        slab_spmv(s, false, halo_in_flight, nullptr, s->x0);
        timed(&stats->time_initial_r_ms, nullptr, [&] { launch_cg_init_residual(nl, s->b, s->Ap, s->r, s->p, s->partials_blas, s->compute); });
        timed(&stats->time_dot_rs_initial_ms, nullptr, [&] {
            launch_reduce_partials(s->partials_blas, cg_partial_count(nl), &s->d_s->rr_new, nullptr, s->compute, s->scratch(), nullptr, 0, L.mailbox);
        });
    }
    s->enqueued_stage = "initial residual";
    if (L.separate) allreduce_scalar(s, &s->d_s->rr_new, "all-reduce of the initial r.r");
    s->reduce_mailbox = s->fused_dot ? L.mailbox : nullptr;
    launch_cg_scalars_init(s->d_s, s->d_hist, s->compute);
    if (timeline) HIP_CHECK(hipEventRecord(tl_event(s->tl_compute, 1), s->compute));
    if (s->label && config->verbose >= 1) {
        CgScalars now;
        HIP_CHECK(hipStreamSynchronize(s->compute));
        HIP_CHECK(hipMemcpy(&now, s->d_s, sizeof now, hipMemcpyDeviceToHost));
        printf("[%s] Initial residual: %e\n", s->label, now.b_norm);
    }
    start_halo(s->p, false);
}

void SolveRun::stage_spmv() {
    backward = (enqueued & 1) == 0;
    s->shape.reverse = backward;
    s->enqueued_iteration = enqueued;
    s->enqueued_stage = "SpMV";
    TraceScope range(trace, "SpMV");
    s->spmv_progress = &s->h_poll->progress;
    s->spmv_progress_value = 4 * (s->poll_sequence + 1) + 1;
    mark(enqueued, 0);
    if (timeline) {
        s->tl_after_interior = tl_event(s->tl_compute, mark_index(enqueued, 1));
        slab_spmv(s, true, halo_in_flight, skip, nullptr, tl_event(s->tl_compute, mark_index(enqueued, 2)));
        s->tl_after_interior = nullptr;
    } else if (L.detail) {
        timed(&stats->time_spmv_ms, nullptr, [&] { slab_spmv(s, true, halo_in_flight, skip); });
    } else if (s->spmv_event_stride > 0 && (enqueued + s->spmv_event_phase) % s->spmv_event_stride == 0) {
        while (s->spmv_ev.size() < 2 * (size_t)(sampled + 1)) {
            hipEvent_t e;
            HIP_CHECK(hipEventCreate(&e));
            s->spmv_ev.push_back(e);
        }
        HIP_CHECK(hipEventRecord(s->spmv_ev[2 * sampled], s->compute));
        slab_spmv(s, true, halo_in_flight, skip, nullptr, s->spmv_ev[2 * sampled + 1]);
        sampled_iteration.push_back(enqueued);
        ++sampled;
    } else {
        slab_spmv(s, true, halo_in_flight, skip);
    }
    s->spmv_progress = nullptr;
}

void SolveRun::stage_allreduce_pAp() {
    s->enqueued_stage = "all-reduce of p.Ap";
    if (L.separate || (L.reduce && !s->fused_dot)) {
        TraceScope r(trace, "AllReduce");
        timed(&stats->time_allreduce_ms, nullptr, [&] { allreduce_scalar(s, &s->d_s->pAp, "all-reduce of p.Ap"); });
    }
    mark(enqueued, 3);
}

void SolveRun::stage_update_r() {
    s->enqueued_stage = "r update";
    TraceScope range(trace, "BLAS_AXPY");
    timed(&stats->time_blas1_ms, &stats->time_axpy_update_r_ms,
          [&] { launch_cg_update_r(nl, s->d_s, s->Ap, s->r, s->partials_blas, s->compute, !backward); });
    mark(enqueued, 4);
}

void SolveRun::stage_sum_rr_and_step() {
    step_in_direction = L.pipeline && L.separate && (enqueued + 1) - window_start < L.slots;
    ++s->poll_sequence;
    TraceScope range(trace, "Dot_Product");
    if (L.separate) {
        timed(&stats->time_reductions_ms, &stats->time_dot_rs_new_ms, [&] {
            launch_reduce_partials(s->partials_blas, cg_partial_count(nl), &s->d_s->rr_new, skip, s->compute, s->scratch(), &s->h_poll->progress,
                                   4 * s->poll_sequence + 2);
        });
        s->enqueued_stage = "all-reduce of r.r";
        {
            TraceScope r(trace, "AllReduce");
            timed(&stats->time_allreduce_ms, nullptr, [&] { allreduce_scalar(s, &s->d_s->rr_new, "all-reduce of r.r"); });
        }
        if (!step_in_direction)
            launch_cg_scalars_step(s->d_s, config->tolerance, s->d_hist, &s->h_poll->sequence, s->poll_sequence, s->compute, s->d_alpha_ring, L.slots);
    } else {
        timed(&stats->time_reductions_ms, &stats->time_dot_rs_new_ms, [&] {
            launch_reduce_partials_and_step(s->partials_blas, cg_partial_count(nl), &s->d_s->rr_new, skip, s->compute, s->scratch(), s->d_s,
                                            config->tolerance, s->d_hist, &s->h_poll->sequence, s->poll_sequence, s->d_alpha_ring, L.slots, L.mailbox,
                                            &s->h_poll->progress, 4 * s->poll_sequence + 2);
        });
    }
    mark(enqueued, 5);
    ++enqueued;
}

bool SolveRun::far_from_convergence(int iteration, int basis) const {
#ifdef SPMV_AMD_LAB
    if (s->guess_far_always) return true;
    if (s->stop_at > 0) return iteration + 3 < s->stop_at;
#endif
    if (basis < 0 || basis > records_read || basis >= s->hist_cap || iteration <= basis) return false;
    const double ratio = basis == 0 ? 1.0 : s->d_hist[basis] / s->d_hist[0];
    double bar = config->tolerance;
    for (int k = basis; k < iteration; ++k) bar *= 16.0;
    return ratio > bar;
}

bool SolveRun::converged_at(int k) const {
    if (k < 1 || k >= s->hist_cap) return s->h_poll->converged != 0;
#ifdef SPMV_AMD_LAB
    if (s->stop_at > 0 && k == s->stop_at) return true;
#endif
    return s->d_hist[k] / s->d_hist[0] < config->tolerance;
}

void SolveRun::await_record(int iteration) {
    wait_for_record(s, sequence0 + iteration);
    if (iteration > records_read) records_read = iteration;
}

void SolveRun::stage_direction_and_halo() {
    trace.push("BLAS_AXPBY");
    const size_t lo = L.bulk_lo, hi = L.bulk_hi;
    const bool two_pieces = L.late && hi - lo >= 4 * s->lead_rows && !(s->late_predict && far_from_convergence(enqueued, records_read));
    const size_t cut = !two_pieces ? (backward ? lo : hi) : backward ? (hi - s->lead_rows) / 512 * 512 : lo + s->lead_rows;
    const size_t first_lo = backward ? cut : lo, first_rows = backward ? hi - cut : cut - lo;
    const size_t rest_lo = backward ? lo : cut, rest_rows = backward ? cut - lo : hi - cut;
    auto pieces = [&](auto&& first, auto&& rest) {
        timed(&stats->time_blas1_ms, &stats->time_axpby_update_p_ms, [&] {
            first(first_lo, first_rows);
            if (!two_pieces) return;
            s->enqueued_stage = "direction update (lead piece)";
            await_record(enqueued);
            if (!s->h_poll->converged) rest(rest_lo, rest_rows);
        });
    };
    if (L.slots == 1) {
        const double* x_in = enqueued == 1 ? s->x0 : s->x;
        auto px = [&](size_t off, size_t count) {
            if (count > 0) launch_cg_update_px(count, s->d_s, s->r + off, s->p + off, x_in + off, s->x + off, enqueued, s->compute, backward, s->device_form);
        };
        pieces(px, px);
    } else {
        if (enqueued - window_start == L.slots) {
            timed(&stats->time_blas1_ms, nullptr, [&] {
                launch_cg_flush_x(nl, s->d_alpha_ring, ring_view, L.slots, window_start % L.slots, L.slots, window_start == 0 ? s->x0 : s->x, s->x, s->compute,
                                  s->d_s, window_start);
            });
            window_start = enqueued;
        }
        double* p_next = s->ring[(size_t)(enqueued % L.slots)];
        const double* p_in = s->p;
        auto plain = [&](size_t off, size_t count) {
            if (count > 0) launch_cg_update_p_ring(count, s->d_s, s->r + off, p_in + off, p_next + off, enqueued, s->compute, backward, s->device_form);
        };
        auto fused = [&](size_t off, size_t count) {
            launch_cg_direction(DirectionLaunch{s->d_s, config->tolerance, enqueued, s->d_hist, step_in_direction ? &s->h_poll->sequence : nullptr,
                                                s->poll_sequence, s->d_alpha_ring, L.slots, s->r, p_in, p_next, off, count, backward, s->device_form},
                                &L.edges, s->scratch(), s->compute);
            s->p = p_next;
            trace.pop();
            {
                TraceScope r(trace, "Halo_Exchange");
                start_halo(s->p, true);
            }
            trace.push("BLAS_AXPBY");
        };
        if (L.pipeline) pieces(fused, plain);
        else pieces(plain, plain);
        s->p = p_next;
    }
    trace.pop();
    mark(enqueued - 1, 6);
    s->enqueued_stage = "direction update and halo exchange";
    if (!L.pipeline) {
        TraceScope r(trace, "Halo_Exchange");
        start_halo(s->p, false);
    }
}

bool SolveRun::read_status() {
    const int j = enqueued;
    if (records_read < j - 1) {
        await_record(j - 1);
        if (converged_at(j - 1)) {
            await_record(j);
            return true;
        }
    }
    const bool deferred = s->run_ahead && config->verbose < 2 && j + 1 < s->hist_cap && far_from_convergence(j, j - 1);
    if (!deferred) await_record(j);
    mailbox_check(s->comm);
    if (const int gave_up = __atomic_load_n(&s->h_poll->halo_late, __ATOMIC_ACQUIRE)) {
        if (s->selfcheck) {
            s->selfcheck_late = true;
            __atomic_store_n(&s->h_poll->halo_late, 0, __ATOMIC_RELEASE);
            return true;
        }
        fprintf(stderr, "\n[spmv_amd watchdog] rank %d: no progress for %.1f s in stage '%s' (CG iteration %d)\n", s->comm->rank, halo_wait_limit_s(s),
                gave_up == 3 ? "edge rows' ready flag (side-stream wait in front of the halo exchange)"
                             : "halo arrival flag (in-kernel wait of the boundary rows)",
                enqueued - 1);
        report_slab_state(s, stderr);
        exit(EXIT_FAILURE);
    }
    if (config->verbose >= 2 && s->comm->rank == 0) {
        CgScalars now;
        HIP_CHECK(hipMemcpy(&now, s->d_s, sizeof now, hipMemcpyDeviceToHost));
        if (s->label)
            printf("[%s] Iter %3d: residual = %e (rel = %e)\n", s->label, now.iterations, now.residual, now.residual / now.b_norm);
        else
            printf("[Iter %3d] Residual: %.6e (rel: %.6e, alpha: %.4e)\n", now.iterations, now.residual, now.residual / now.b_norm, now.alpha);
    }
    return deferred ? false : s->h_poll->converged != 0;
}

void SolveRun::resolve_timeline(const CgScalars& fin, float total_ms) {
    auto us = [&](hipEvent_t a, hipEvent_t b) {
        float ms = 0.f;
        HIP_CHECK(hipEventElapsedTime(&ms, a, b));
        return (double)ms * 1e3;
    };
    const std::vector<hipEvent_t>& E = s->tl_compute;
    const size_t tl_flush = mark_index(enqueued, 0);
    const int its = fin.iterations < enqueued ? fin.iterations : enqueued;
    const int direction_updates = fin.converged && its > 0 ? its - 1 : its;
    double stage[kTimelineMarks] = {0, 0, 0, 0, 0, 0, 0};
    double iteration_us = 0.0;
    for (int it = 0; it < its; ++it) {
        const size_t base = mark_index(it, 0);
        for (int k = 0; k < kTimelineMarks - 1; ++k)
            if (k != 5 || it < direction_updates) stage[k] += us(E[base + k], E[base + k + 1]);
        const hipEvent_t next = it + 1 < enqueued ? E[base + kTimelineMarks] : E[tl_flush];
        stage[6] += us(E[base + 6], next);
        iteration_us += us(E[base], next);
    }
    double side_us = 0.0;
    const int exchanges = tl_exchanges < its ? tl_exchanges : its;
    for (int j = 0; j < exchanges; ++j) side_us += us(s->tl_side[2 * (size_t)j], s->tl_side[2 * (size_t)j + 1]);
    const double per = its > 0 ? 1.0 / its : 0.0;
    s->timeline_us = {(double)its, (double)total_ms, us(E[0], E[1]), stage[0] * per, stage[1] * per, stage[2] * per, stage[3] * per,
                      stage[4] * per, direction_updates > 0 ? stage[5] / direction_updates : 0.0, stage[6] * per, iteration_us * per,
                      exchanges > 0 ? side_us / exchanges : 0.0, us(E[tl_flush], E[tl_flush + 1]), (double)direction_updates};
    stats->time_spmv_ms = (s->timeline_us[3] + s->timeline_us[4]) * s->timeline_us[0] / 1e3;
}

void SolveRun::finish() {
    s->shape.reverse = false;
    s->reduce_mailbox = nullptr;
    const size_t tl_flush = mark_index(enqueued, 0);
    if (timeline) HIP_CHECK(hipEventRecord(tl_event(s->tl_compute, tl_flush), s->compute));
    if (L.slots > 1 && enqueued > window_start)
        timed(&stats->time_blas1_ms, nullptr, [&] {
            launch_cg_flush_x(nl, s->d_alpha_ring, ring_view, L.slots, window_start % L.slots, enqueued - window_start, window_start == 0 ? s->x0 : s->x,
                              s->x, s->compute, s->d_s, window_start);
        });
    s->p = s->ring[0];
    if (enqueued == 0)
        HIP_CHECK(hipMemcpyAsync(s->x, s->x0, nl * sizeof(double), hipMemcpyDeviceToDevice, s->compute));
    if (timeline) HIP_CHECK(hipEventRecord(tl_event(s->tl_compute, tl_flush + 1), s->compute));
    total.end(s->compute);
    float total_ms = 0.f;
    {
        WatchdogScope guard("draining the streams after the loop", s->comm->rank, enqueued, report_slab_state, s);
        total_ms = total.elapsed_ms();
        if (s->side) HIP_CHECK(hipStreamSynchronize(s->side));
    }
    HIP_CHECK(hipGetLastError());
    CgScalars fin;
    memset(&fin, 0, sizeof fin);
    if (enqueued > 0 && !s->op_failed) {
        fin.iterations = s->h_poll->iterations;
        fin.converged = s->h_poll->converged;
    }
    if (fin.iterations < s->hist_cap && !s->op_failed) {
        fin.residual = s->d_hist[fin.iterations];
        fin.rr_old = fin.residual * fin.residual;
    } else {
        HIP_CHECK(hipMemcpy(&fin, s->d_s, sizeof fin, hipMemcpyDeviceToHost));
    }
    if (timeline) {
        resolve_timeline(fin, total_ms);
    } else if (!L.detail) {
        double ms_sum = 0.0;
        s->last_spmv_each.clear();
        for (int k = 0; k < sampled; ++k) {
            if (sampled_iteration[k] >= fin.iterations) continue;
            float ms = 0.f;
            HIP_CHECK(hipEventElapsedTime(&ms, s->spmv_ev[2 * k], s->spmv_ev[2 * k + 1]));
            ms_sum += ms;
            s->last_spmv_each.push_back(ms);
        }
        stats->time_spmv_ms = s->last_spmv_each.empty() ? 0.0 : ms_sum / (double)s->last_spmv_each.size() * fin.iterations;
    }
    ++s->spmv_event_phase;
    s->last_spmv_ms = stats->time_spmv_ms;
    s->last_spmv_launches = fin.iterations;
    stats->iterations = fin.iterations;
    stats->converged = fin.converged;
    stats->residual_norm = (fin.converged || fin.iterations < s->hist_cap) ? fin.residual : sqrt(fin.rr_old);
    stats->time_total_ms = total_ms;
    if (!fin.converged && s->comm->rank == 0 && s->label == nullptr) printf("\nMax iterations reached without convergence\n");
    if (L.detail && stats->iterations > 0) {
        stats->time_dot_rs_new_ms /= stats->iterations;
        stats->time_axpy_update_r_ms /= stats->iterations;
        stats->time_axpby_update_p_ms /= stats->iterations;
    }
    const int count = fin.iterations + 1 < s->hist_cap ? fin.iterations + 1 : s->hist_cap;
    s->history.assign(s->d_hist, s->d_hist + count);
    last_cg_history() = s->history;
}

}

extern "C" int spmv_amd_cg_slab_solve(SpmvAmdCgSlab* s, const CGConfigMultiGPU* config, CGStatsMultiGPU* stats) {
    SolveRun run(s, config, stats);
    TraceScope solver_range(run.trace, "CG_Solver");
    run.begin();
    run.initial_residual();
    bool done = false;
    while (!done && !s->op_failed && run.enqueued < config->max_iters) {
        TraceScope iteration_range(run.trace, "CG_Iteration");
        run.stage_spmv();
        if (s->op_failed) break;
        run.stage_allreduce_pAp();
        run.stage_update_r();
        run.stage_sum_rr_and_step();
        run.stage_direction_and_halo();
        done = run.read_status();
    }
    run.finish();
    return s->op_failed ? 1 : 0;
}

extern "C" int spmv_amd_cg_slab_gather(SpmvAmdCgSlab* s, double* x_full) {
    const int P = s->comm->world;
    std::vector<int> counts((size_t)P), displs((size_t)P);
    for (int r = 0; r < P; ++r) spmv_amd_partition_rows(s->n, P, r, &displs[r], &counts[r]);
    HIP_CHECK(hipStreamSynchronize(s->compute));
    if (s->comm->rank != 0)
        download(x_full + s->row_offset, s->x, (size_t)s->n_local);
    WatchdogScope guard("gathering the solution on rank 0", s->comm->rank, -1, report_slab_state, s);
    s->comm->gather_to_root(s->x, s->n_local, x_full, counts.data(), displs.data());
    return 0;
}

extern "C" int spmv_amd_cg_slab_history(SpmvAmdCgSlab* s, double* out, int cap) {
    return copy_history(s->history, out, cap);
}

extern "C" int spmv_amd_cg_slab_spmv(SpmvAmdCgSlab* s, const double* x_full, double* y_local) {
    upload(s->p, x_full + s->row_offset, (size_t)s->n_local);
    if (s->has_prev && s->row_offset >= s->halo)
        upload(s->p - s->halo, x_full + s->row_offset - s->halo, (size_t)s->halo);
    if (s->has_next && s->row_offset + s->n_local + s->halo <= s->n)
        upload(s->p + s->n_local, x_full + s->row_offset + s->n_local, (size_t)s->halo);
    slab_spmv(s, s->spmv_with_dot, false, nullptr);
    HIP_CHECK(hipStreamSynchronize(s->compute));
    HIP_CHECK(hipGetLastError());
    download(y_local, s->Ap, (size_t)s->n_local);
    return 0;
}

extern "C" void spmv_amd_cg_slab_info(const SpmvAmdCgSlab* s, int* row_offset, int* n_local,
                                      int* local_nnz) {
    if (row_offset) *row_offset = s->row_offset;
    if (n_local) *n_local = s->n_local;
    if (local_nnz) *local_nnz = (int)s->A.view.nnz_local;
}

extern "C" const char* spmv_amd_cg_slab_variant(const SpmvAmdCgSlab* s) { return s->variant_name; }

extern "C" int spmv_amd_cg_slab_coefficient_form(const SpmvAmdCgSlab* s) { return s->planes_on ? 1 : 0; }

extern "C" int spmv_amd_cg_slab_uniform_tiles(const SpmvAmdCgSlab* s, long long* uniform, long long* total) {
    const bool have = s->planes_alloc != nullptr && s->tile_classes != nullptr;
    if (uniform) *uniform = have ? s->tiles_uniform : 0;
    if (total) *total = have ? s->tiles_total : 0;
    return 0;
}

extern "C" int spmv_amd_cg_slab_placement(const SpmvAmdCgSlab* s, double* out, int cap) {
    const int count = (int)s->placement.size();
    for (int i = 0; i < count && i < cap; ++i) out[i] = s->placement[i];
    return count;
}
extern "C" int spmv_amd_cg_slab_setup_ms(const SpmvAmdCgSlab* s, double* out, int cap) {
    for (int i = 0; i < 5 && i < cap; ++i) out[i] = s->setup_ms[i];
    return 5;
}
extern "C" int spmv_amd_cg_slab_tile_runs(const SpmvAmdCgSlab* s, double* out, int cap) {
    const int count = (int)s->tile_runs.size();
    for (int i = 0; i < count && i < cap; ++i) out[i] = s->tile_runs[i];
    return count;
}

extern "C" int spmv_amd_cg_slab_spmv_launch_ms(const SpmvAmdCgSlab* s, float* out, int cap) {
    const int count = (int)s->last_spmv_each.size();
    for (int i = 0; i < count && i < cap; ++i) out[i] = s->last_spmv_each[i];
    return count;
}

extern "C" void spmv_amd_cg_slab_set_timeline(SpmvAmdCgSlab* s, int on) { s->timeline_on = on != 0; }

#ifdef SPMV_AMD_LAB
extern "C" int spmv_amd_cg_slab_set_option(SpmvAmdCgSlab* s, const char* name, long long value) {
    if (strcmp(name, "late_bulk") == 0) s->late_bulk = value != 0, s->late_predict = value == 2;
    else if (strcmp(name, "lead_rows") == 0) s->lead_rows = value < 512 ? 512 : (size_t)value / 512 * 512;
    else if (strcmp(name, "run_ahead") == 0) s->run_ahead = value != 0, s->guess_far_always = value == 2;
    else if (strcmp(name, "no_overlap") == 0) s->no_overlap = value != 0 || s->comm->pipeline_verdict < 0;
    else if (strcmp(name, "stop_at") == 0) s->stop_at = value > 0 ? (int)value : 0;
    else if (strcmp(name, "spmv_event_stride") == 0) s->spmv_event_stride = (int)value;
    else if (strcmp(name, "csr_coefficients") == 0) s->planes_on = value == 0 && s->planes_alloc != nullptr;
    else if (strcmp(name, "stream_coefficients") == 0) {
        s->stream_everywhere = value != 0;
        if (s->planes_alloc != nullptr) s->planes = plane_view(s, s->planes_alloc);
    }
    else if (strcmp(name, "block_rows") == 0) {
        if (value != 0 && value != 4 && value != 8) return -1;
        s->shape.knobs.rowlds_block_rows = (int)value;
        for (Stencil5Plan* p : {&s->plan_whole, &s->plan_interior, &s->plan_head, &s->plan_tail})
            if (p->variant == Stencil5Variant::RowLds) p->block_rows = (int)value;
        build_block_maps(s);
    }
    else if (strcmp(name, "spmv_with_dot") == 0) s->spmv_with_dot = value != 0;
    else return -1;
    return 0;
}

extern "C" long long spmv_amd_cg_slab_block_map(const SpmvAmdCgSlab* s, int which, unsigned char* out, long long cap) {
    const Stencil5Plan& p = which == 0 ? s->plan_whole : s->plan_interior;
    if (p.block_map == nullptr) return 0;
    const long long count = rowlds_block_tiles(p);
    if (out != nullptr && cap > 0) HIP_CHECK(hipMemcpy(out, p.block_map, (size_t)std::min(count, cap), hipMemcpyDeviceToHost));
    return count;
}

extern "C" long long spmv_amd_cg_slab_tile_classes(const SpmvAmdCgSlab* s, unsigned char* out, long long cap) {
    if (s->tile_classes == nullptr) return 0;
    const long long count = (long long)s->tile_class_count;
    if (out != nullptr && cap > 0) HIP_CHECK(hipMemcpy(out, s->tile_classes, (size_t)std::min(count, cap), hipMemcpyDeviceToHost));
    return count;
}
#endif
extern "C" const char* spmv_amd_cg_slab_timeline_names(void) { return kTimelineNames; }
extern "C" int spmv_amd_cg_slab_timeline(const SpmvAmdCgSlab* s, double* out, int cap) {
    const int count = (int)s->timeline_us.size();
    for (int i = 0; i < count && i < cap; ++i) out[i] = s->timeline_us[i];
    return count;
}

extern "C" int spmv_amd_cg_slab_time_spmv(SpmvAmdCgSlab* s, int reps, float* ms_each) {
    HIP_CHECK(hipMemsetAsync(&s->d_s->converged, 0, sizeof(int), s->compute));
    EventTimer t;
    for (int i = 0; i < reps; ++i) {
        t.begin(s->compute);
        (void)launch_stencil5_spmv(s->A.view, s->plan_whole, s->p, s->Ap, 1.0, s->fused_dot ? s->partials_spmv : nullptr,
                                   nullptr, false, s->compute, nullptr, s->sym());
        t.end(s->compute);
        ms_each[i] = t.elapsed_ms();
    }
    HIP_CHECK(hipGetLastError());
    return 0;
}

extern "C" void spmv_amd_cg_slab_destroy(SpmvAmdCgSlab* s) {
    if (!s) return;
    (void)hipStreamSynchronize(s->compute);
    (void)hipStreamSynchronize(s->side);
    s->A.release();
    device_release(s->x);
    device_release(s->x0_alloc);
    device_release(s->b);
    s->x0 = nullptr;
    device_release(s->vec_arena);
    device_release(s->planes_alloc);
    device_release(s->tile_classes);
    device_release(s->block_map_whole);
    device_release(s->block_map_interior);
    s->planes_on = false;
    s->r = s->Ap = s->p_alloc = s->p = nullptr;
    s->ring_alloc.clear();
    s->ring.clear();
    device_release(s->d_alpha_ring);
    device_release(s->partials_spmv);
    device_release(s->partials_blas);
    device_release(s->reduce_stage);
    device_release(s->d_halo_flag);
    device_release(s->d_s);
    if (s->d_hist) (void)hipHostFree(s->d_hist);
    if (s->h_poll) (void)hipHostFree(s->h_poll);
    for (hipEvent_t e : s->spmv_ev) (void)hipEventDestroy(e);
    for (hipEvent_t e : s->tl_compute) (void)hipEventDestroy(e);
    for (hipEvent_t e : s->tl_side) (void)hipEventDestroy(e);
    (void)hipEventDestroy(s->ev_p_ready);
    (void)hipEventDestroy(s->ev_halo_done);
    if (s->owns_streams) {
        (void)hipStreamDestroy(s->compute);
        (void)hipStreamDestroy(s->side);
    }
    delete s;
}

namespace {
SpmvAmdCgSlab* g_workspace = nullptr;
int g_workspace_device = -1;
std::mutex g_workspace_lock;
std::atomic<std::thread::id> g_workspace_owner{std::thread::id()};
bool g_release_pending = false;
void release_cg_workspace_locked() {
    spmv_amd::release_cg_multi_workspace_locked();
    spmv_amd::release_pcg_workspace_locked();
    if (g_workspace == nullptr) return;
    spmv_amd_cg_slab_destroy(g_workspace);
    g_workspace = nullptr;
}
}

namespace spmv_amd {

void release_cg_workspace() {
    if (g_workspace_owner.load(std::memory_order_acquire) == std::this_thread::get_id()) {
        g_release_pending = true;
        return;
    }
    std::lock_guard<std::mutex> guard(g_workspace_lock);
    release_cg_workspace_locked();
}

CgWorkspaceScope::CgWorkspaceScope() {
    g_workspace_lock.lock();
    g_release_pending = false;
    g_workspace_owner.store(std::this_thread::get_id(), std::memory_order_release);
}

CgWorkspaceScope::~CgWorkspaceScope() {
    g_workspace_owner.store(std::thread::id(), std::memory_order_release);
    if (g_release_pending) release_cg_workspace_locked();
    g_release_pending = false;
    g_workspace_lock.unlock();
}

int cg_solve_on_operator(SpmvOperator* op, int n, const double* b, double* x, const CGConfig& config, CGStats* stats,
                         std::vector<double>* history) {
    std::lock_guard<std::mutex> guard(g_workspace_lock);
    struct Owner {
        Owner() { g_release_pending = false, g_workspace_owner.store(std::this_thread::get_id(), std::memory_order_release); }
        ~Owner() {
            g_workspace_owner.store(std::thread::id(), std::memory_order_release);
            if (g_release_pending) release_cg_workspace_locked();
            g_release_pending = false;
        }
    } owner;
    int device = 0;
    HIP_CHECK(hipGetDevice(&device));
    if (g_workspace != nullptr && (g_workspace->n != n || g_workspace_device != device)) release_cg_workspace_locked();
    if (g_workspace == nullptr) {
        SpmvAmdCgSlab* s = new SpmvAmdCgSlab();
        s->comm = self_comm();
        s->op = op;
        s->n = s->n_local = n;
        s->grid = -1;
        s->label = "CG-DEVICE";
        s->device_form = true;
        make_common(s);
        g_workspace = s;
        g_workspace_device = device;
    } else {
        adopt_operator(g_workspace, op);
    }
    SpmvAmdCgSlab* s = g_workspace;
    upload(s->b, b, (size_t)n);
    upload(s->x0, x, (size_t)n);
    const CGConfigMultiGPU cfg = {config.max_iters, config.tolerance, config.verbose, config.enable_detailed_timers};
    CGStatsMultiGPU st;
    if (spmv_amd_cg_slab_solve(s, &cfg, &st) != 0) return 1;
    download(x, s->x, (size_t)n);
    *history = s->history;
    const double r0 = s->history.empty() ? 0.0 : s->history.front();
    const double last = st.converged ? st.residual_norm : (s->history.empty() ? 0.0 : s->history.back());
    fill_device_stats(stats, st.iterations, st.converged != 0, last, r0, config, st.time_total_ms,
                      st.time_spmv_ms + (config.enable_detailed_timers ? st.time_initial_r_ms : 0.0), st.time_blas1_ms,
                      st.time_reductions_ms + st.time_dot_rs_initial_ms);
    return 0;
}

}

int cg_solve_mgpu_partitioned(SpmvOperator* spmv_op, MatrixData* mat, const double* b, double* x,
                              CGConfigMultiGPU config, CGStatsMultiGPU* stats) {
    (void)spmv_op;
    SpmvAmdComm* comm = world_comm();
    const int rank = comm->rank, world = comm->world;
    if (rank == 0 && config.verbose >= 1) {
        printf("\n========================================\n");
        printf("Multi-GPU CG Solver (PARTITIONED CSR)\n");
        printf("========================================\n");
        printf("Ranks: %d (transport: %s)\n", world, comm->transport());
        printf("Problem size: %d unknowns\n", mat->rows);
        printf("Max iterations: %d\n", config.max_iters);
        printf("Tolerance: %.1e\n", config.tolerance);
        printf("========================================\n\n");
    }
    SpmvAmdCgSlab* s = create_from_matrix(mat, comm, false);
    if (!s) return 1;
    if (config.verbose >= 1)
        printf("[Rank %d] Rows: [%d:%d) (%d rows), local nnz %lld\n", rank, s->row_offset,
               s->row_offset + s->n_local, s->n_local, s->A.view.nnz_local);
    spmv_amd_cg_slab_set_vectors(s, b, x);
    spmv_amd_cg_slab_solve(s, &config, stats);

    if (world > 1) {
        std::vector<double> slots((size_t)world * 6, 0.0);
        double mine[6] = {stats->time_total_ms,       stats->time_spmv_ms,      stats->time_blas1_ms,
                          stats->time_reductions_ms, stats->time_allreduce_ms, stats->time_allgather_ms};
        memcpy(&slots[(size_t)rank * 6], mine, sizeof mine);
        double* d_slots = device_alloc<double>(slots.size());
        upload(d_slots, slots.data(), slots.size());
        {
            WatchdogScope guard("all-reduce of the ranks' timers", rank, -1, report_slab_state, s);
            comm->allreduce_sum(d_slots, (int)slots.size(), s->compute);
            HIP_CHECK(hipStreamSynchronize(s->compute));
        }
        download(slots.data(), d_slots, slots.size());
        device_release(d_slots);
        if (rank == 0) {
            double mx[6], mn[6];
            for (int k = 0; k < 6; ++k) {
                mx[k] = mn[k] = slots[k];
                for (int r = 1; r < world; ++r) {
                    const double v = slots[(size_t)r * 6 + k];
                    mx[k] = v > mx[k] ? v : mx[k];
// ... 30 lines not shown
```

### cuda-spmv-benchmark_amd/csrc/kernels.hpp

```cpp
#pragma once

#include <hip/hip_runtime.h>
#include <stddef.h>

struct PeerMailbox;

namespace spmv_amd {

struct SlabCsr {
    const int* row_ptr = nullptr;
    const int* col_idx = nullptr;
    const double* values = nullptr;
    int n_local = 0;
    int row_offset = 0;
    long long nnz_local = 0;
    int max_row_nnz = 0;
    long long nnz_base = 0;
    int n_global = 0;
    int grid_size = -1;
    bool verified_stencil = false;
    int halo_before = 0;
    int halo_after = 0;
};

struct Tunables {
    int rowlds_min_grid = 512;
    int rowlds_group = 0;
    int rowlds_block_rows = 4;
};

inline int xcd_run_group(int n, int block_columns, int small_grid_group) {
    if (n < 8000) return small_grid_group;
    const int g = (n + 1100 + 8 * block_columns - 1) / (8 * block_columns);
    return g < 1 ? 1 : (g > 64 ? 64 : g);
}

struct LaunchShape {
    Tunables knobs;
    bool reverse = false;
};

void launch_generate_stencil5_csr(int n, int row_offset, int n_local, long long nnz_base,
                                  double center, double off, int* row_ptr, int* col_idx,
                                  double* values, hipStream_t stream);
void launch_verify_stencil5_csr(const SlabCsr& m, int* d_mismatch, hipStream_t stream);

enum class Stencil5Variant { Auto, RowDirect, RowGeneric, RowLds };
struct Stencil5Plan {
    Stencil5Variant variant = Stencil5Variant::RowGeneric;
    int first_row = 0, last_row = 0;
    int gi_lo = 0, gi_hi = 0;
    int row_blocks = 0;
    int xcd_run = 0;
    int block_rows = 0;
    const unsigned char* block_map = nullptr;
    int partials = 0;
    const char* name = "";
};
Stencil5Plan plan_stencil5(const SlabCsr& m, int first_row, int last_row, Stencil5Variant variant,
                           const LaunchShape& shape);
int rowlds_xcd_run_rule(int n);
struct ResidualOut {
    const double* b;
    double* r;
    double* p;
};
struct SymPlanes {
    const double* ce = nullptr;
    const double* s = nullptr;
    const unsigned char* cls = nullptr;
    double w = 0.0, c = 0.0, e = 0.0, n = 0.0, s5 = 0.0;
};
void launch_fill_sym_planes(const SlabCsr& m, double* ce, double* s, hipStream_t stream);
void launch_classify_tiles(const SlabCsr& m, const double quintuple[5], unsigned char* cls, unsigned long long* d_uniform, hipStream_t stream);
struct ChebStep {
    const double* r = nullptr;
    const double* dinv = nullptr;
    double* d = nullptr;
    double* z_out = nullptr;
    double g = 0.0, h = 0.0;
    int last = 0;
    int* work_count = nullptr;
};
int rowlds_col_tiles(int n);
int rowlds_block_tiles(const Stencil5Plan& plan);
void launch_block_map(const unsigned char* cls, const Stencil5Plan& plan, unsigned char* out, hipStream_t stream);
void launch_verify_sym_planes(const SlabCsr& m, const SymPlanes& planes, int* d_mismatch, hipStream_t stream);

int launch_stencil5_spmv(const SlabCsr& m, const Stencil5Plan& plan, const double* x, double* y, double alpha,
                         double* d_dot_partials, const int* d_skip_flag, bool reverse, hipStream_t stream,
                         const ResidualOut* init = nullptr, const SymPlanes* planes = nullptr);
int launch_stencil5_cheb_step(const SlabCsr& m, const Stencil5Plan& plan, const double* z, const ChebStep& step, double* d_dot_partials,
                              const int* d_skip_flag, hipStream_t stream);
int launch_stencil5_spmv(const SlabCsr& m, const double* x, double* y, double alpha,
                          int first_row, int last_row, double* d_dot_partials,
                          const int* d_skip_flag, Stencil5Variant variant,
                          const LaunchShape& shape, hipStream_t stream);

int launch_stencil5_spmv_first_and_last_gridrow(const SlabCsr& m, const Stencil5Plan& head, const Stencil5Plan& tail, const double* x,
                                                double* y, double alpha, double* d_dot_partials, const int* d_skip_flag,
                                                hipStream_t stream, const ResidualOut* init = nullptr, const SymPlanes* planes = nullptr);

enum class CsrVariant { Auto, Stream, Adaptive, RowScalar, Wavefront };
CsrVariant csr_auto_variant(const SlabCsr& m);
void launch_csr_spmv(const SlabCsr& m, const double* x, double* y, double alpha,
                     CsrVariant variant, hipStream_t stream, double* d_dot_partials = nullptr);
int csr_fused_dot_partials(const SlabCsr& m, CsrVariant variant);

void launch_ell_transpose(int rows, int width, const int* idx_rowmajor, const double* val_rowmajor,
                          int* idx_slotmajor, double* val_slotmajor, hipStream_t stream);
void launch_ell_spmv(int rows, int width, const int* idx, const double* val, const double* x,
                     double* y, double alpha, double beta, hipStream_t stream,
                     int grid_hint = 0, double* d_dot_partials = nullptr);
int ell_fused_dot_partials(int rows);
void launch_ell_stencil5_spmv(int rows, int width, int grid_size, const int* idx,
                              const double* val, const double* x, double* y, double alpha,
                              double beta, hipStream_t stream, double* d_dot_partials = nullptr);

struct CgScalars {
    double rr_old;
    double rr_new;
    double pAp;
    double b_norm;
    double residual;
    double alpha;
    double beta;
    int converged;
    int iterations;
    int max_history;
    int stop_at;
    double rr_ring[2];
};

void launch_fill(double* d, size_t n, double value, hipStream_t stream);
void launch_axpy(size_t n, double a, const double* x, double* y, hipStream_t stream);
void launch_axpby(size_t n, double a, const double* x, double b, const double* y, double* z,
                  hipStream_t stream);
void launch_axpy_dev(size_t n, const double* d_a, const double* x, double* y, bool subtract,
                     hipStream_t stream);
void launch_update_p_dev(size_t n, const double* r, const double* d_b, double* p,
                         hipStream_t stream);
size_t dot_scratch_doubles(size_t n);
unsigned stream_grid(size_t n);
void launch_dot_partials(size_t n, const double* x, const double* y, double* partials, hipStream_t stream);
void launch_dot(size_t n, const double* x, const double* y, double* scratch, double* d_result,
                hipStream_t stream);
void launch_scalar_divide(const double* d_num, const double* d_den, double* d_out,
                          hipStream_t stream);
void launch_check_convergence(const double* d_rr_new, double b_norm, double tol, int* d_converged,
                              double* d_residual, hipStream_t stream);

struct ReduceScratch {
    double* base = nullptr;
};
int reduce_scratch_doubles();
double* reduce_scratch_alloc();

struct HaloArrival {
    const unsigned* flag = nullptr;
    unsigned expected = 0;
    long long timeout_ticks = 0;
    int* late = nullptr;
};
void launch_halo_arrived(unsigned* d_flag, unsigned sequence, hipStream_t stream);

bool launch_stencil5_edges_and_reduce(const SlabCsr& m, const Stencil5Plan& interior, bool first_gridrow, bool last_gridrow, const double* x,
                                      double* y, double alpha, const double* d_interior_partials, double* d_out, const int* d_skip_flag,
                                      const ReduceScratch& scratch, int* host_progress, int progress_value, const PeerMailbox* mailbox,
                                      hipStream_t stream, const HaloArrival& halo = HaloArrival{}, const SymPlanes* planes = nullptr);

void launch_cg_init_residual(size_t n, const double* b, const double* Ap, double* r, double* p,
                             double* partials, hipStream_t stream);
void launch_cg_update_r(size_t n, const CgScalars* s, const double* Ap, double* r, double* partials,
                        hipStream_t stream, bool reverse = false);
void launch_cg_update_px(size_t n, const CgScalars* s, const double* r, double* p, const double* x_in,
                         double* x, int iteration, hipStream_t stream, bool reverse = false, bool fma_form = false);
void launch_cg_update_p_ring(size_t n, const CgScalars* s, const double* r, const double* p_in, double* p_out,
                             int iteration, hipStream_t stream, bool reverse = false, bool fma_form = false);
constexpr int kMaxRingSlots = 16;
struct RingSlots {
    const double* p[kMaxRingSlots];
};
void launch_cg_flush_x(size_t n, const double* alphas, const RingSlots& ring, int slots, int first_slot, int count,
                       const double* x_in, double* x, hipStream_t stream, const CgScalars* s = nullptr, int window_start = 0);
int cg_partial_count(size_t n);
void launch_reduce_partials(const double* partials, int count, double* d_out,
                            const int* d_skip_flag, hipStream_t stream, const ReduceScratch& scratch = ReduceScratch{},
                            int* host_progress = nullptr, int progress_value = 0,
                            const PeerMailbox* mailbox = nullptr, const double* extra = nullptr, int extra_count = 0);
struct EdgeRows {
    size_t count_a, second, count_b;
};
void launch_reduce_partials_and_step(const double* partials, int count, double* d_out, const int* d_skip_flag,
                                     hipStream_t stream, const ReduceScratch& scratch, CgScalars* s, double tol, double* history,
                                     int* host_record, int sequence, double* alpha_ring = nullptr, int ring_slots = 0,
                                     const PeerMailbox* mailbox = nullptr, int* host_progress = nullptr,
                                     int progress_value = 0);
struct DirectionLaunch {
    CgScalars* s;
    double tol;
    int iteration;
    double* history;
    int* step_host_record;
    int sequence;
    double* alpha_ring;
    int ring_slots;
    const double* r;
    const double* p_in;
    double* p_out;
    size_t bulk_lo, bulk_rows;
    bool reverse, fma_form;
};
void launch_cg_direction(const DirectionLaunch& d, const EdgeRows* edge_rows, const ReduceScratch& scratch, hipStream_t stream);
void launch_edges_wait(const ReduceScratch& scratch, int sequence, long long timeout_ticks, int* late, hipStream_t stream);
void launch_cg_scalars_init(CgScalars* s, double* history, hipStream_t stream);
void launch_cg_scalars_step(CgScalars* s, double tol, double* history, int* host_record, int sequence,
                            hipStream_t stream, double* alpha_ring = nullptr, int ring_slots = 0);

}
```

### cuda-spmv-benchmark_amd/csrc/spmv_kernels.hip

```cpp
#include "kernels.hpp"

#include <stdlib.h>

#include <type_traits>

#include "reduce_device.hpp"
#include "stencil_geometry.hpp"
#include "stencil_row_device.hpp"
#include "stream_device.hpp"

namespace spmv_amd {
namespace {

constexpr int kBlock = 256;
constexpr int kWavesPerBlock = 4;
__device__ __forceinline__ long long logical_block(int group, long long total) {
    const long long b = blockIdx.x;
    if (group <= 1) return b;
    const long long t = xcd_run_tile<long long>(b, group);
    return t < total ? t : -1;
}

__device__ __forceinline__ double x_at(const double* __restrict__ x, long long local_col,
                                       int lo, int hi) {
    return (local_col >= lo && local_col < hi) ? x[local_col] : 0.0;
}

template <bool kAnalyticInterior>
__device__ __forceinline__ double row_reference(const SlabCsr& m, const double* __restrict__ x,
                                                int local_row, int i, int j) {
    const int n = m.grid_size;
    if (kAnalyticInterior && stencil_is_interior(i, j, n)) {
        const long long o = stencil_row_start(i, j, n) - m.nnz_base;
        const double* __restrict__ v = m.values + o;
        const double* __restrict__ xl = x + local_row;
        return stencil5_interior(v[1], xl[-1], v[2], xl[0], v[3], xl[1], v[0], xl[-n], v[4], xl[n]);
    }
    const int lo = -m.halo_before, hi = m.n_local + m.halo_after;
    const int k0 = m.row_ptr[local_row], k1 = m.row_ptr[local_row + 1];
    double sum = 0.0;
    for (int k = k0; k < k1; ++k)
        sum = fma(m.values[k], x_at(x, (long long)m.col_idx[k] - m.row_offset, lo, hi), sum);
    return sum;
}


template <bool kDot>
__global__ __launch_bounds__(kBlock) void stencil5_rowdirect_kernel(
    SlabCsr m, const double* __restrict__ x, double* __restrict__ y, double alpha, int gi_lo,
    int col_blocks, double* __restrict__ dot_partials, const int* __restrict__ skip_flag) {
    __shared__ double wave_part[kWavesPerBlock];
    if (skip_flag != nullptr && *skip_flag != 0) return;
    const int n = m.grid_size;
    const int row_group = (int)blockIdx.x / col_blocks;
    const int col_block = (int)blockIdx.x - row_group * col_blocks;
    const int li = gi_lo + row_group;
    const int gi = m.row_offset / n + li;
    const int j = col_block * kBlock + (int)threadIdx.x;
    double dot_acc = 0.0;
    if (j < n) {
        const long long lr = (long long)li * n + j;
        const double* __restrict__ xl = x + lr;
        double sum;
        if (j > 0 && j < n - 1 && gi > 0 && gi < n - 1) {
            const double* __restrict__ v = m.values + (stencil_gridrow_base(gi, n) + 5LL * j - 1 - m.nnz_base);
            const double v0 = v[0], v1 = v[1], v2 = v[2], v3 = v[3], v4 = v[4];
            sum = stencil5_interior(v1, xl[-1], v2, xl[0], v3, xl[1], v0, xl[-n], v4, xl[n]);
        } else {
            sum = row_reference<false>(m, x, (int)lr, gi, j);
        }
        if (kDot) dot_acc = fma(xl[0], sum, dot_acc);
        y[lr] = alpha * sum;
    }
    if (kDot) {
#pragma unroll
        for (int off = 32; off > 0; off >>= 1) dot_acc += __shfl_down(dot_acc, off);
        if ((threadIdx.x & 63) == 0) wave_part[threadIdx.x >> 6] = dot_acc;
        __syncthreads();
        if (threadIdx.x == 0)
            dot_partials[blockIdx.x] = ((wave_part[0] + wave_part[1]) + wave_part[2]) + wave_part[3];
    }
}

constexpr int kLdsTileCols = 128;

template <int kMode, bool kFreshHalo = false, bool kSym = false>
__device__ __forceinline__ bool rowlds_tile(const SlabCsr& m, const double* __restrict__ x, double* __restrict__ y, double alpha,
                                            int li, int gi, int j0, int lane, int skip, double* __restrict__ strip,
                                            double* __restrict__ xrow, const ResidualOut& res, double* dot, const SymPlanes& sp = SymPlanes{},
                                            int tile_class = 0, const ChebStep& step = ChebStep{}) {
    constexpr bool kDot = kMode == 1;
    constexpr bool kInit = kMode == 2;
    constexpr bool kCheb = kMode == 3;
    const int n = m.grid_size;
    double dot_acc = 0.0;
    if (gi > 0 && gi < n - 1) {
        const long long e = stencil_gridrow_base(gi, n) + 5LL * j0 - 1 - m.nnz_base + lane;
        const double* __restrict__ vals = m.values;
        double c[10];
        d2 ce[2];
        double cs[2], cn[2], cw = 0.0;
        if constexpr (kSym) {
        } else if (j0 == 0 || j0 + kLdsTileCols > n - 1) {
            const long long hi = m.nnz_local - 1;
#pragma unroll
            for (int k = 0; k < 10; ++k) {
                long long idx = e + 64 * k;
                idx = idx < 0 ? 0 : (idx > hi ? hi : idx);
                c[k] = __builtin_nontemporal_load(vals + idx);
            }
        } else {
#pragma unroll
            for (int k = 0; k < 10; ++k) c[k] = __builtin_nontemporal_load(vals + e + 64 * k);
        }
        double xc[2], xw[2], xe[2], xn[2], xs[2], bv[2];
        double cr[2] = {0.0, 0.0}, cdv[2] = {0.0, 0.0}, cd[2] = {0.0, 0.0};
#pragma unroll
        for (int h = 0; h < 2; ++h) {
            const int j = j0 + lane + 64 * h;
            xc[h] = xw[h] = xe[h] = xn[h] = xs[h] = bv[h] = 0.0;
            if (j < n) {
                const double* __restrict__ xl = x + ((long long)li * n + j);
                xc[h] = xl[0];
                if (kFreshHalo) {
                    xn[h] = published_by_any_agent(reinterpret_cast<const unsigned long long*>(xl - n));
                    xs[h] = published_by_any_agent(reinterpret_cast<const unsigned long long*>(xl + n));
                } else {
                    xn[h] = xl[-n], xs[h] = xl[n];
                }
                if (kInit) bv[h] = __builtin_nontemporal_load(res.b + ((long long)li * n + j));
                if constexpr (kCheb) {
                    cr[h] = __builtin_nontemporal_load(step.r + ((long long)li * n + j));
                    cdv[h] = __builtin_nontemporal_load(step.dinv + ((long long)li * n + j));
                    cd[h] = __builtin_nontemporal_load(step.d + ((long long)li * n + j));
                }
                if (h == 0 && lane == 0 && j > 0) xw[0] = xl[-1];
                if (h == 1 && lane == 63 && j < n - 1) xe[1] = xl[1];
            }
        }
        const auto finish = [&](auto uniform_tile) {
            constexpr bool kUniform = decltype(uniform_tile)::value;
            if constexpr (kSym) {
                if constexpr (!kUniform) {
                    strip[1 + lane] = ce[0].y;
                    strip[65 + lane] = ce[1].y;
                    if (lane == 0) strip[0] = cw;
                }
            } else {
#pragma unroll
                for (int k = 0; k < 10; ++k) strip[64 * k + lane] = c[k];
            }
            xrow[1 + lane] = xc[0];
            xrow[65 + lane] = xc[1];
            wave_lds_sync();
            tile_west_east(xrow, lane, j0, n, xw[0], xe[1], xw, xe);
            double cwv[2] = {0.0, 0.0};
            if constexpr (kSym && !kUniform) {
                cwv[0] = strip[lane];
                cwv[1] = strip[64 + lane];
            }
#pragma unroll
            for (int h = 0; h < 2; ++h) {
                const int j = j0 + lane + 64 * h;
                if (j < n) {
                    const double* __restrict__ v = strip + 5 * (lane + 64 * h);
                    double sum;
                    if constexpr (kSym) {
                        const double vw = kUniform ? sp.w : cwv[h], vc = kUniform ? sp.c : ce[h].x, ve = kUniform ? sp.e : ce[h].y,
                                     vn = kUniform ? sp.n : cn[h], vs = kUniform ? sp.s5 : cs[h];
                        sum = stencil5_row(j, n, vw, xw[h], vc, xc[h], ve, xe[h], vn, xn[h], vs, xs[h]);
                    }
                    else if (j > 0 && j < n - 1) {
                        sum = v[1] * xw[h];
                        sum = fma(v[2], xc[h], sum);
                        sum = fma(v[3], xe[h], sum);
                        sum = fma(v[0], xn[h], sum);
                        sum = fma(v[4], xs[h], sum);
                    } else if (j == 0) {
                        sum = fma(v[1], xn[h], 0.0);
                        sum = fma(v[2], xc[h], sum);
                        sum = fma(v[3], xe[h], sum);
                        sum = fma(v[4], xs[h], sum);
                    } else {
                        sum = fma(v[0], xn[h], 0.0);
                        sum = fma(v[1], xw[h], sum);
                        sum = fma(v[2], xc[h], sum);
                        sum = fma(v[3], xs[h], sum);
                    }
                    if (kDot) dot_acc = fma(xc[h], sum, dot_acc);
                    if constexpr (kCheb) {
                        const long long lr = (long long)li * n + j;
                        const double t = fma(-1.0, sum, cr[h]);
                        const double u = cdv[h] * t;
                        const double dn = fma(step.g, u, step.h * cd[h]);
                        const double zn = xc[h] + dn;
                        __builtin_nontemporal_store(dn, step.d + lr);
                        step.z_out[lr] = zn;
                        if (step.last) dot_acc = fma(cr[h], zn, dot_acc);
                    } else if (kInit) {
                        const long long lr = (long long)li * n + j;
                        const double rv = fma(-1.0, alpha * sum, bv[h]);
                        __builtin_nontemporal_store(rv, res.r + lr);
                        res.p[lr] = rv;
                        dot_acc = fma(rv, rv, dot_acc);
                    } else {
                        __builtin_nontemporal_store(alpha * sum, y + ((long long)li * n + j));
                    }
                }
            }
        };
        if constexpr (kSym) {
            if (__builtin_amdgcn_readfirstlane(tile_class) != 0) {
                if (skip != 0) return false;
                finish(std::true_type{});
            } else {
                const long long r0 = (long long)li * n + j0 + lane;
#pragma unroll
                for (int h = 0; h < 2; ++h) {
                    ce[h] = d2{0.0, 0.0};
                    cs[h] = cn[h] = 0.0;
                    if (j0 + lane + 64 * h < n) {
                        ce[h] = __builtin_nontemporal_load(reinterpret_cast<const d2*>(sp.ce) + r0 + 64 * h);
                        cs[h] = sp.s[r0 + 64 * h];
                        cn[h] = sp.s[r0 + 64 * h - n];
                    }
                }
                if (lane == 0 && j0 > 0) cw = sp.ce[2 * (r0 - 1) + 1];
                if (skip != 0) return false;
                finish(std::false_type{});
            }
        } else {
            if (skip != 0) return false;
            finish(std::false_type{});
        }
    } else {
        if (skip != 0) return false;
#pragma unroll
        for (int h = 0; h < 2; ++h) {
            const int j = j0 + lane + 64 * h;
            if (j < n) {
                const long long lr = (long long)li * n + j;
                const double sum = row_reference<false>(m, x, (int)lr, gi, j);
                if (kDot) dot_acc = fma(x[lr], sum, dot_acc);
                if constexpr (kCheb) {
                    const double rl = step.r[lr];
                    const double t = fma(-1.0, sum, rl);
                    const double u = step.dinv[lr] * t;
                    const double dn = fma(step.g, u, step.h * step.d[lr]);
                    const double zn = x[lr] + dn;
                    step.d[lr] = dn;
                    step.z_out[lr] = zn;
                    if (step.last) dot_acc = fma(rl, zn, dot_acc);
                } else if (kInit) {
                    const double rv = fma(-1.0, alpha * sum, res.b[lr]);
                    res.r[lr] = rv;
                    res.p[lr] = rv;
                    dot_acc = fma(rv, rv, dot_acc);
                } else {
                    y[lr] = alpha * sum;
                }
            }
        }
    }
    if (kDot || kInit || kCheb) dot_acc = wave_sum(dot_acc);
    *dot = dot_acc;
    return true;
}

__device__ __forceinline__ int rowlds_tile_class(const SymPlanes& sp, int li, int col_tiles, int col_tile) {
    return sp.cls != nullptr ? (int)sp.cls[li * col_tiles + col_tile] : 0;
}

__device__ __forceinline__ int rowlds_tile_of_block(int b, int run, int total, int reverse) {
    const int tile = xcd_run_tile<int>(b, run);
    if (tile >= total) return -1;
    return reverse ? total - 1 - tile : tile;
}

template <int kMode>
__global__ __launch_bounds__(64) void stencil5_rowlds_kernel(
    SlabCsr m, const double* __restrict__ x, double* __restrict__ y, double alpha, int gi_lo, int row_step,
    int gfirst, int col_tiles, int total_tiles, int run, int reverse, double* __restrict__ dot_partials,
    const int* __restrict__ skip_flag, ResidualOut res, SymPlanes sp, ChebStep step) {
    __shared__ double strip[5 * kLdsTileCols];
    __shared__ double xrow[kLdsTileCols + 2];
    const int skip = skip_flag != nullptr ? __builtin_nontemporal_load(skip_flag) : 0;
    const int tile = rowlds_tile_of_block((int)blockIdx.x, run, total_tiles, reverse);
    if (tile < 0) return;
    const int row_group = tile / col_tiles;
    const int col_tile = tile - row_group * col_tiles;
    const int li = gi_lo + row_group * row_step;
    const int uniform = rowlds_tile_class(sp, li, col_tiles, col_tile);
    double dot = 0.0;
    if constexpr (kMode == 3) {
        if (!rowlds_tile<3>(m, x, y, alpha, li, gfirst + li, col_tile * kLdsTileCols, (int)threadIdx.x, skip, strip, xrow, res, &dot, sp, 0, step))
            return;
        if (threadIdx.x == 0) {
            if (step.last) dot_partials[tile] = dot;
            if (tile == 0 && step.work_count != nullptr) *step.work_count += 1;
        }
        return;
    }
    const bool live = sp.ce != nullptr
                          ? rowlds_tile<kMode, false, true>(m, x, y, alpha, li, gfirst + li, col_tile * kLdsTileCols, (int)threadIdx.x, skip, strip,
                                                            xrow, res, &dot, sp, uniform)
                          : rowlds_tile<kMode>(m, x, y, alpha, li, gfirst + li, col_tile * kLdsTileCols, (int)threadIdx.x, skip, strip, xrow, res, &dot);
    if (!live) return;
    if (kMode != 0 && threadIdx.x == 0) dot_partials[tile] = dot;
}

template <int kRows>
__global__ __launch_bounds__(64) void stencil5_rowlds_block_kernel(
    SlabCsr m, const double* __restrict__ x, double* __restrict__ y, double alpha, int gi_lo, int gi_hi, int gfirst, int col_tiles,
    int total_blocks, int run, int reverse, double* __restrict__ dot_partials, const int* __restrict__ skip_flag,
    const unsigned char* __restrict__ block_map, SymPlanes sp) {
    constexpr int kRowDoubles = kLdsTileCols + 2;
    constexpr int kFastDoubles = kRows * kRowDoubles, kOneRowDoubles = 5 * kLdsTileCols + kRowDoubles;
    __shared__ double lds[kFastDoubles > kOneRowDoubles ? kFastDoubles : kOneRowDoubles];
    const int skip = skip_flag != nullptr ? __builtin_nontemporal_load(skip_flag) : 0;
    const int block = rowlds_tile_of_block((int)blockIdx.x, run, total_blocks, reverse);
    if (block < 0) return;
    const int row_block = block / col_tiles;
    const int col_tile = block - row_block * col_tiles;
    const int li0 = gi_lo + row_block * kRows;
    const int j0 = col_tile * kLdsTileCols, lane = (int)threadIdx.x;
    const int n = m.grid_size;
    const int fast = (int)block_map[block];
    const int row_lo = -(m.halo_before / n), row_hi = (m.n_local + m.halo_after) / n;
    double xv[kRows + 2][2];
    double xo[kRows];
#pragma unroll
    for (int r = 0; r < kRows + 2; ++r) {
        const int li = li0 - 1 + r;
        xv[r][0] = xv[r][1] = 0.0;
        if (li >= row_lo && li < row_hi) {
            const double* __restrict__ xr = x + ((long long)li * n + j0);
            if (j0 + lane < n) xv[r][0] = xr[lane];
            if (j0 + lane + 64 < n) xv[r][1] = xr[lane + 64];
        }
    }
#pragma unroll
    for (int r = 0; r < kRows; ++r) {
        const int li = li0 + r;
        xo[r] = 0.0;
        if (li < row_hi) {
            const double* __restrict__ xr = x + ((long long)li * n + j0);
            if (lane == 0 && j0 > 0) xo[r] = xr[-1];
            if (lane == 63 && j0 + kLdsTileCols < n) xo[r] = xr[kLdsTileCols];
        }
    }
    if (__builtin_amdgcn_readfirstlane(fast) != 0) {
        if (skip != 0) return;
#pragma unroll
        for (int r = 0; r < kRows; ++r) {
            lds[r * kRowDoubles + 1 + lane] = xv[r + 1][0];
            lds[r * kRowDoubles + 65 + lane] = xv[r + 1][1];
        }
        wave_lds_sync();
#pragma unroll
        for (int r = 0; r < kRows; ++r) {
            const int li = li0 + r;
            double xw[2], xe[2];
            tile_west_east(lds + r * kRowDoubles, lane, j0, n, xo[r], xo[r], xw, xe);
            double dot = 0.0;
#pragma unroll
            for (int h = 0; h < 2; ++h) {
                const int j = j0 + lane + 64 * h;
                if (j < n) {
                    const double xc = xv[r + 1][h], xn = xv[r][h], xs = xv[r + 2][h];
                    const double sum = stencil5_row(j, n, sp.w, xw[h], sp.c, xc, sp.e, xe[h], sp.n, xn, sp.s5, xs);
                    dot = fma(xc, sum, dot);
                    __builtin_nontemporal_store(alpha * sum, y + ((long long)li * n + j));
                }
            }
            dot = wave_sum(dot);
            if (lane == 0) dot_partials[(li - gi_lo) * col_tiles + col_tile] = dot;
        }
    } else {
        double* __restrict__ strip = lds;
        double* __restrict__ xrow = lds + 5 * kLdsTileCols;
        const ResidualOut none{nullptr, nullptr, nullptr};
        const int held = gi_hi - li0 < kRows ? gi_hi - li0 : kRows;
#pragma unroll 1
        for (int r = 0; r < held; ++r) {
            const int li = li0 + r;
            const int uniform = rowlds_tile_class(sp, li, col_tiles, col_tile);
            double dot = 0.0;
            if (!rowlds_tile<1, false, true>(m, x, y, alpha, li, gfirst + li, j0, lane, skip, strip, xrow, none, &dot, sp, uniform)) return;
            if (lane == 0) dot_partials[(li - gi_lo) * col_tiles + col_tile] = dot;
            wave_lds_sync();
        }
    }
}

__global__ __launch_bounds__(kBlock) void block_map_kernel(const unsigned char* __restrict__ cls, int col_tiles, int gi_lo, int gi_hi,
                                                           int block_rows, int total_blocks, unsigned char* __restrict__ out) {
    const int block = (int)(blockIdx.x * (unsigned)kBlock + threadIdx.x);
    if (block >= total_blocks) return;
    const int row_block = block / col_tiles, col_tile = block - row_block * col_tiles;
    const int li0 = gi_lo + row_block * block_rows;
    bool fast = li0 + block_rows <= gi_hi;
    for (int r = 0; fast && r < block_rows; ++r) fast = cls[(long long)(li0 + r) * col_tiles + col_tile] == 1;
    out[block] = fast ? 1 : 0;
}

__global__ __launch_bounds__(kReduceBlock) void stencil5_rowlds_edges_reduce_kernel(
    SlabCsr m, const double* __restrict__ x, double* __restrict__ y, double alpha, int li_first, int li_step, int gfirst,
    int col_tiles, int edge_tiles, int edge_blocks, const double* __restrict__ interior_partials, int interior_count, int slice,
    int slice_blocks, ReduceStage stage, ReduceTail tail, HaloArrival halo, SymPlanes sp) {
    __shared__ double strip[kWavesPerBlock][5 * kLdsTileCols];
    __shared__ double xrow[kWavesPerBlock][kLdsTileCols + 2];
    __shared__ double s[kReduceBlock];
    __shared__ int s_last;
    const int skip = tail.skip_flag != nullptr ? __builtin_nontemporal_load(tail.skip_flag) : 0;
    const int tickets = edge_blocks + slice_blocks;
    if ((int)blockIdx.x < edge_blocks) {
        const int wave = (int)(threadIdx.x >> 6), lane = (int)(threadIdx.x & 63);
        const int tile = (int)blockIdx.x * kWavesPerBlock + wave;
        if (tile < edge_tiles) {
            const int row_group = tile / col_tiles;
            const int li = li_first + row_group * li_step;
            const int uniform = rowlds_tile_class(sp, li, col_tiles, tile - row_group * col_tiles);
            double dot = 0.0;
            const ResidualOut none{nullptr, nullptr, nullptr};
            bool live;
            if (halo.flag != nullptr) {
                if (skip == 0 && lane == 0) {
                    const long long t0 = wall_clock64();
                    while ((int)(__hip_atomic_load(halo.flag, __ATOMIC_RELAXED, __HIP_MEMORY_SCOPE_AGENT) - halo.expected) < 0) {
                        if (wall_clock64() - t0 > halo.timeout_ticks) {
                            __hip_atomic_store(halo.late, 1, __ATOMIC_RELAXED, __HIP_MEMORY_SCOPE_SYSTEM);
                            break;
                        }
                        __builtin_amdgcn_s_sleep(4);
                    }
                }
                __builtin_amdgcn_wave_barrier();
                __builtin_amdgcn_fence(__ATOMIC_ACQUIRE, "wavefront");
                const int j0 = (tile - row_group * col_tiles) * kLdsTileCols;
                live = sp.ce != nullptr ? rowlds_tile<1, true, true>(m, x, y, alpha, li, gfirst + li, j0, lane, skip, strip[wave], xrow[wave], none, &dot, sp, uniform)
                                        : rowlds_tile<1, true>(m, x, y, alpha, li, gfirst + li, j0, lane, skip, strip[wave], xrow[wave], none, &dot);
            } else {
                const int j0 = (tile - row_group * col_tiles) * kLdsTileCols;
                live = sp.ce != nullptr ? rowlds_tile<1, false, true>(m, x, y, alpha, li, gfirst + li, j0, lane, skip, strip[wave], xrow[wave], none, &dot, sp, uniform)
                                        : rowlds_tile<1>(m, x, y, alpha, li, gfirst + li, j0, lane, skip, strip[wave], xrow[wave], none, &dot);
            }
            if (live && lane == 0) publish(stage.extra + tile, dot);
        }
        if (skip != 0) {
            reduce_skipped(tail, blockIdx.x == 0);
            return;
        }
        draw_ticket_and_finish_if_last(stage, slice_blocks, stage.extra, edge_tiles, tickets, tail, s, &s_last);
    } else {
        if (skip != 0) return;
        reduce_slice_block(interior_partials, interior_count, slice, (int)blockIdx.x - edge_blocks, slice_blocks, stage.extra, edge_tiles,
                           tickets, stage, tail, s, &s_last);
    }
}

template <bool kAnalytic, bool kDot>
__global__ __launch_bounds__(kBlock) void stencil5_row_kernel(SlabCsr m, const double* __restrict__ x,
                                                              double* __restrict__ y, double alpha,
                                                              int first_row, int last_row,
                                                              double* __restrict__ dot_partials,
                                                              const int* __restrict__ skip_flag) {
    if (skip_flag != nullptr && *skip_flag != 0) return;
    const long long row = (long long)first_row + (long long)blockIdx.x * kBlock + threadIdx.x;
    double dot_acc = 0.0;
    if (row < last_row) {
        int i = -1, j = 0;
        if (kAnalytic) {
            const int g = m.row_offset + (int)row;
            i = g / m.grid_size;
            j = g - i * m.grid_size;
        }
        const double sum = row_reference<kAnalytic>(m, x, (int)row, i, j);
        if (kDot) dot_acc = x[row] * sum;
        y[row] = alpha * sum;
    }
    if (kDot) {
#pragma unroll
        for (int off = 32; off > 0; off >>= 1) dot_acc += __shfl_down(dot_acc, off);
        if ((threadIdx.x & 63) == 0) dot_partials[blockIdx.x * kWavesPerBlock + (threadIdx.x >> 6)] = dot_acc;
    }
}

__global__ __launch_bounds__(kBlock) void csr_row_scalar_kernel(SlabCsr m, const double* __restrict__ x,
                                                                double* __restrict__ y, double alpha) {
    const long long row = (long long)blockIdx.x * kBlock + threadIdx.x;
    if (row >= m.n_local) return;
    const int lo = -m.halo_before, hi = m.n_local + m.halo_after;
    const int k0 = m.row_ptr[row], k1 = m.row_ptr[row + 1];
    double sum = 0.0;
    for (int base = k0; base < k1; base += 8) {
        int c[8];
        double v[8], xv[8];
#pragma unroll
        for (int u = 0; u < 8; ++u) {
            const bool live = base + u < k1;
            c[u] = live ? m.col_idx[base + u] : m.row_offset;
            v[u] = live ? m.values[base + u] : 0.0;
        }
#pragma unroll
        for (int u = 0; u < 8; ++u) xv[u] = x_at(x, (long long)c[u] - m.row_offset, lo, hi);
#pragma unroll
        for (int u = 0; u < 8; ++u)
            if (base + u < k1) sum = fma(v[u], xv[u], sum);
    }
    y[row] = alpha * sum;
}

template <int kThreads, int kPerThread, bool kVectorLong = false>
__global__ __launch_bounds__(kThreads) void csr_stream_kernel(SlabCsr m, const double* __restrict__ x,
                                                              double* __restrict__ y, double alpha,
                                                              int rows_per_block, int xcd_group, int total_blocks,
                                                              double* __restrict__ dot_partials) {
    constexpr int kCsrStreamCap = kThreads * kPerThread;
    constexpr int kCsrStreamPerThread = kPerThread;
    __shared__ double sv[kCsrStreamCap];
    __shared__ double sx[kCsrStreamCap];
    __shared__ int s_owner[2];
    __shared__ double s_wave[kThreads / 64];
    const int lo = -m.halo_before, hi = m.n_local + m.halo_after;
    const long long blk = logical_block(xcd_group, total_blocks);
    if (blk < 0) return;
    const long long r0 = blk * rows_per_block;
    const long long r1 = min(r0 + rows_per_block, (long long)m.n_local);
    const int kb = m.row_ptr[r0], ke = m.row_ptr[r1];
    const long long row = r0 + threadIdx.x;
    const bool has_row = (int)threadIdx.x < rows_per_block && row < r1;
    int k0 = 0, k1 = 0;
    if (has_row) {
        k0 = m.row_ptr[row];
        k1 = m.row_ptr[row + 1];
    }
    double row_sum = 0.0;
    if (ke - kb <= kCsrStreamCap) {
        int c[kCsrStreamPerThread];
        double v[kCsrStreamPerThread], xv[kCsrStreamPerThread];
#pragma unroll
        for (int u = 0; u < kCsrStreamPerThread; ++u) {
            const int e = kb + (int)threadIdx.x + u * kThreads;
            const bool live = e < ke;
            c[u] = live ? m.col_idx[e] : m.row_offset;
// ... 353 lines not shown
}

void launch_verify_sym_planes(const SlabCsr& m, const SymPlanes& planes, int* d_mismatch, hipStream_t stream) {
    if (m.n_local == 0) return;
    hipLaunchKernelGGL(verify_sym_planes_kernel, dim3(blocks_for(m.n_local)), dim3(kBlock), 0, stream, m, planes, d_mismatch);
}

int rowlds_col_tiles(int n) { return (n + kLdsTileCols - 1) / kLdsTileCols; }

void launch_classify_tiles(const SlabCsr& m, const double q[5], unsigned char* cls, unsigned long long* d_uniform, hipStream_t stream) {
    const int n = m.grid_size;
    if (m.n_local == 0 || n <= 0 || m.n_local % n != 0) return;
    const int col_tiles = rowlds_col_tiles(n);
    hipLaunchKernelGGL(classify_tiles_kernel, dim3((unsigned)(m.n_local / n) * (unsigned)col_tiles), dim3(64), 0, stream, m, q[0], q[1], q[2], q[3],
                       q[4], col_tiles, cls, d_uniform);
}

int rowlds_xcd_run_rule(int n) {
    if (n < 8000) return 4;
    const int tiles = (n + kLdsTileCols - 1) / kLdsTileCols;
    const int run = (int)(1.05 * tiles / 8.0 + 0.5);
    return run < 1 ? 1 : (run > 64 ? 64 : run);
}

Stencil5Plan plan_stencil5(const SlabCsr& m, int first_row, int last_row, Stencil5Variant variant,
                           const LaunchShape& shape) {
    Stencil5Plan p;
    const Tunables& knobs = shape.knobs;
    const int n = m.grid_size;
    const bool direct_ok = m.verified_stencil && n >= 2 && m.row_offset % n == 0 &&
                           m.n_local % n == 0 && first_row % n == 0 && last_row % n == 0;
    if (variant == Stencil5Variant::Auto)
        variant = !direct_ok ? Stencil5Variant::RowGeneric : n >= knobs.rowlds_min_grid ? Stencil5Variant::RowLds : Stencil5Variant::RowDirect;
    if (variant != Stencil5Variant::RowGeneric && !direct_ok) variant = Stencil5Variant::RowGeneric;
    p.variant = variant;
    if (variant == Stencil5Variant::RowGeneric) {
        p.row_blocks = (int)blocks_for((long long)last_row - first_row);
        p.partials = p.row_blocks * kWavesPerBlock;
        p.name = m.verified_stencil ? "stencil5/row-generic" : "stencil5/row-generic(csr-loop)";
    } else {
        p.gi_lo = first_row / n;
        p.gi_hi = last_row / n;
        if (variant == Stencil5Variant::RowDirect) {
            p.row_blocks = (int)blocks_for(n);
            p.name = "stencil5/row-direct";
        } else {
            p.row_blocks = (n + kLdsTileCols - 1) / kLdsTileCols;
            p.xcd_run = knobs.rowlds_group > 0 ? knobs.rowlds_group : rowlds_xcd_run_rule(n);
            if (p.xcd_run < 1 || p.xcd_run > 64) p.xcd_run = 4;
            p.name = "stencil5/row-lds";
            p.block_rows = knobs.rowlds_block_rows == 4 || knobs.rowlds_block_rows == 8 ? knobs.rowlds_block_rows : 0;
        }
        p.partials = p.row_blocks * (p.gi_hi - p.gi_lo);
    }
    p.first_row = first_row;
    p.last_row = last_row;
    return p;
}

int launch_stencil5_spmv(const SlabCsr& m, const double* x, double* y, double alpha,
                         int first_row, int last_row, double* d_dot_partials,
                         const int* d_skip_flag, Stencil5Variant variant,
                         const LaunchShape& shape, hipStream_t stream) {
    if (last_row <= first_row) return 0;
    return launch_stencil5_spmv(m, plan_stencil5(m, first_row, last_row, variant, shape), x, y, alpha, d_dot_partials,
                                d_skip_flag, shape.reverse, stream);
}

namespace {
void launch_rowlds(const SlabCsr& m, const Stencil5Plan& p, const double* x, double* y, double alpha, int gi_lo, int row_step,
                   int tiles, double* d_dot_partials, const int* d_skip_flag, bool reverse, hipStream_t stream, const ResidualOut* init,
                   const SymPlanes* planes, const ChebStep* step = nullptr) {
    const dim3 grid((unsigned)xcd_padded_grid(tiles, p.xcd_run));
    const int gfirst = m.row_offset / m.grid_size;
    const ResidualOut res = init ? *init : ResidualOut{nullptr, nullptr, nullptr};
    const SymPlanes sp = planes ? *planes : SymPlanes{};
#define SPMV_AMD_LAUNCH_ROWLDS(MODE)                                                                                   \
    hipLaunchKernelGGL((stencil5_rowlds_kernel<MODE>), grid, dim3(64), 0, stream, m, x, y, alpha, gi_lo, row_step, gfirst, \
                       p.row_blocks, tiles, p.xcd_run, reverse ? 1 : 0, d_dot_partials, d_skip_flag, res, sp, cs)
    const ChebStep cs = step ? *step : ChebStep{};
    if (step) SPMV_AMD_LAUNCH_ROWLDS(3);
    else if (init) SPMV_AMD_LAUNCH_ROWLDS(2);
    else if (d_dot_partials) SPMV_AMD_LAUNCH_ROWLDS(1);
    else SPMV_AMD_LAUNCH_ROWLDS(0);
#undef SPMV_AMD_LAUNCH_ROWLDS
}

void launch_rowlds_block(const SlabCsr& m, const Stencil5Plan& p, const double* x, double* y, double alpha, double* d_dot_partials,
                         const int* d_skip_flag, bool reverse, hipStream_t stream, const SymPlanes& sp) {
    const int blocks = rowlds_block_tiles(p);
    const dim3 grid((unsigned)xcd_padded_grid(blocks, p.xcd_run));
    const int gfirst = m.row_offset / m.grid_size;
#define SPMV_AMD_LAUNCH_ROWLDS_BLOCK(ROWS)                                                                                      \
    hipLaunchKernelGGL((stencil5_rowlds_block_kernel<ROWS>), grid, dim3(64), 0, stream, m, x, y, alpha, p.gi_lo, p.gi_hi, gfirst, \
                       p.row_blocks, blocks, p.xcd_run, reverse ? 1 : 0, d_dot_partials, d_skip_flag, p.block_map, sp)
    if (p.block_rows == 4) SPMV_AMD_LAUNCH_ROWLDS_BLOCK(4);
    else SPMV_AMD_LAUNCH_ROWLDS_BLOCK(8);
#undef SPMV_AMD_LAUNCH_ROWLDS_BLOCK
}
}

int rowlds_block_tiles(const Stencil5Plan& p) {
    if (p.variant != Stencil5Variant::RowLds || p.block_rows <= 0 || p.gi_hi <= p.gi_lo) return 0;
    return (p.gi_hi - p.gi_lo + p.block_rows - 1) / p.block_rows * p.row_blocks;
}

void launch_block_map(const unsigned char* cls, const Stencil5Plan& p, unsigned char* out, hipStream_t stream) {
    const int blocks = rowlds_block_tiles(p);
    if (blocks <= 0) return;
    hipLaunchKernelGGL(block_map_kernel, dim3(blocks_for(blocks)), dim3(kBlock), 0, stream, cls, p.row_blocks, p.gi_lo, p.gi_hi, p.block_rows,
                       blocks, out);
}

int launch_stencil5_spmv(const SlabCsr& m, const Stencil5Plan& p, const double* x, double* y, double alpha,
                         double* d_dot_partials, const int* d_skip_flag, bool reverse, hipStream_t stream,
                         const ResidualOut* init, const SymPlanes* planes) {
    if (p.last_row <= p.first_row) return 0;
    if (init != nullptr && (p.variant != Stencil5Variant::RowLds || d_dot_partials == nullptr)) {
        fprintf(stderr, "[spmv] the fused initial residual exists for the row-lds kernel only\n");
        exit(EXIT_FAILURE);
    }
    const bool dot = d_dot_partials != nullptr;
    if (p.variant == Stencil5Variant::RowLds && p.block_rows > 0 && p.block_map != nullptr && dot && init == nullptr && planes != nullptr &&
        planes->ce != nullptr && planes->cls != nullptr) {
        launch_rowlds_block(m, p, x, y, alpha, d_dot_partials, d_skip_flag, reverse, stream, *planes);
    } else if (p.variant == Stencil5Variant::RowLds) {
        launch_rowlds(m, p, x, y, alpha, p.gi_lo, 1, p.partials, d_dot_partials, d_skip_flag, reverse, stream, init, planes);
    } else if (p.variant == Stencil5Variant::RowDirect) {
        const dim3 grid((unsigned)p.partials);
        if (dot)
            hipLaunchKernelGGL((stencil5_rowdirect_kernel<true>), grid, dim3(kBlock), 0, stream, m, x, y, alpha, p.gi_lo, p.row_blocks,
                               d_dot_partials, d_skip_flag);
        else
            hipLaunchKernelGGL((stencil5_rowdirect_kernel<false>), grid, dim3(kBlock), 0, stream, m, x, y, alpha, p.gi_lo, p.row_blocks,
                               d_dot_partials, d_skip_flag);
    } else {
        const dim3 grid((unsigned)p.row_blocks);
        const bool analytic = m.verified_stencil && m.grid_size >= 2;
#define SPMV_AMD_LAUNCH_ROWS(AN, DOT)                                                                           \
    hipLaunchKernelGGL((stencil5_row_kernel<AN, DOT>), grid, dim3(kBlock), 0, stream, m, x, y, alpha, p.first_row, \
                       p.last_row, d_dot_partials, d_skip_flag)
        if (analytic) {
            if (dot) SPMV_AMD_LAUNCH_ROWS(true, true);
            else SPMV_AMD_LAUNCH_ROWS(true, false);
        } else {
            if (dot) SPMV_AMD_LAUNCH_ROWS(false, true);
            else SPMV_AMD_LAUNCH_ROWS(false, false);
        }
#undef SPMV_AMD_LAUNCH_ROWS
    }
    return dot ? p.partials : 0;
}

int launch_stencil5_cheb_step(const SlabCsr& m, const Stencil5Plan& p, const double* z, const ChebStep& step, double* d_dot_partials,
                              const int* d_skip_flag, hipStream_t stream) {
    if (p.variant != Stencil5Variant::RowLds || p.last_row <= p.first_row) return -1;
    launch_rowlds(m, p, z, nullptr, 1.0, p.gi_lo, 1, p.partials, d_dot_partials, d_skip_flag, false, stream, nullptr, nullptr, &step);
    return p.partials;
}

int launch_stencil5_spmv_first_and_last_gridrow(const SlabCsr& m, const Stencil5Plan& head, const Stencil5Plan& tail, const double* x,
                                                double* y, double alpha, double* d_dot_partials, const int* d_skip_flag,
                                                hipStream_t stream, const ResidualOut* init, const SymPlanes* planes) {
    const int n = m.grid_size;
    const int local_gridrows = n > 0 ? m.n_local / n : 0;
    if (head.variant != Stencil5Variant::RowLds || tail.variant != Stencil5Variant::RowLds || local_gridrows < 2) {
        int used = launch_stencil5_spmv(m, head, x, y, alpha, d_dot_partials, d_skip_flag, false, stream, init, planes);
        used += launch_stencil5_spmv(m, tail, x, y, alpha, d_dot_partials ? d_dot_partials + used : nullptr, d_skip_flag, false, stream, init,
                                     planes);
        return used;
    }
    const int tiles = 2 * head.row_blocks;
    launch_rowlds(m, head, x, y, alpha, 0, local_gridrows - 1, tiles, d_dot_partials, d_skip_flag, false, stream, init, planes);
    return d_dot_partials ? tiles : 0;
}

namespace {
__global__ void halo_arrived_kernel(unsigned* flag, unsigned sequence) {
    if (threadIdx.x == 0 && blockIdx.x == 0) __hip_atomic_store(flag, sequence, __ATOMIC_RELAXED, __HIP_MEMORY_SCOPE_AGENT);
}
}

void launch_halo_arrived(unsigned* d_flag, unsigned sequence, hipStream_t stream) {
    hipLaunchKernelGGL(halo_arrived_kernel, dim3(1), dim3(64), 0, stream, d_flag, sequence);
}

bool launch_stencil5_edges_and_reduce(const SlabCsr& m, const Stencil5Plan& interior, bool first_gridrow, bool last_gridrow, const double* x,
                                      double* y, double alpha, const double* d_interior_partials, double* d_out, const int* d_skip_flag,
                                      const ReduceScratch& scratch, int* host_progress, int progress_value, const PeerMailbox* mailbox,
                                      hipStream_t stream, const HaloArrival& halo, const SymPlanes* planes) {
    const int n = m.grid_size;
    if (interior.variant != Stencil5Variant::RowLds || scratch.base == nullptr || (!first_gridrow && !last_gridrow) ||
        interior.partials <= 0 || n <= 0 || m.n_local % n != 0)
        return false;
    const int local_gridrows = m.n_local / n;
    const int col_tiles = interior.row_blocks;
    const int edge_tiles = (first_gridrow && last_gridrow ? 2 : 1) * col_tiles;
    if (local_gridrows < 3 || edge_tiles > kReduceExtraMax) return false;
    const int edge_blocks = (edge_tiles + kWavesPerBlock - 1) / kWavesPerBlock;
    int slice = 0, slice_blocks = 0;
    reduce_geometry(interior.partials, &slice, &slice_blocks);
    const ReduceTail tail{d_out, d_skip_flag, host_progress, progress_value, mailbox, StepArgs{nullptr, 0.0, nullptr, nullptr, 0, nullptr, 0}};
    hipLaunchKernelGGL(stencil5_rowlds_edges_reduce_kernel, dim3((unsigned)(edge_blocks + slice_blocks)), dim3(kReduceBlock), 0, stream, m, x, y,
                       alpha, first_gridrow ? 0 : local_gridrows - 1, local_gridrows - 1, m.row_offset / n, col_tiles, edge_tiles, edge_blocks,
                       d_interior_partials, interior.partials, slice, slice_blocks, reduce_stage_of(scratch.base), tail, halo,
                       planes ? *planes : SymPlanes{});
    return true;
}

CsrVariant csr_auto_variant(const SlabCsr& m) {
    const double mean = m.n_local > 0 ? (double)m.nnz_local / (double)m.n_local : 0.0;
    if (mean > 192.0) return CsrVariant::Wavefront;
    return m.max_row_nnz > 1024 ? CsrVariant::Adaptive : CsrVariant::Stream;
}

namespace {
constexpr int kCsrStreamThreads = 256, kCsrStreamCap = 1024;
void csr_stream_geometry(const SlabCsr& m, int* per_block_out, long long* blocks_out) {
    const long long rows = m.n_local;
    const double avg = rows > 0 ? (double)m.nnz_local / rows : 1.0;
    int per_block = (int)(0.9 * kCsrStreamCap / (avg > 1.0 ? avg : 1.0));
    per_block = per_block > kCsrStreamThreads ? kCsrStreamThreads : (per_block < 16 ? 16 : per_block & ~15);
    *per_block_out = per_block;
    *blocks_out = (rows + per_block - 1) / per_block;
}
}

int csr_fused_dot_partials(const SlabCsr& m, CsrVariant variant) {
    if (variant == CsrVariant::Auto) variant = csr_auto_variant(m);
    if ((variant != CsrVariant::Stream && variant != CsrVariant::Adaptive) || m.n_local == 0) return 0;
    int per_block = 0;
    long long blocks = 0;
    csr_stream_geometry(m, &per_block, &blocks);
    return blocks <= 0x7fffffffLL ? (int)blocks : 0;
}

void launch_csr_spmv(const SlabCsr& m, const double* x, double* y, double alpha,
                     CsrVariant variant, hipStream_t stream, double* d_dot_partials) {
    if (m.n_local == 0) return;
    if (variant == CsrVariant::Auto) variant = csr_auto_variant(m);
    const long long rows = m.n_local;
    switch (variant) {
        case CsrVariant::Adaptive:
        case CsrVariant::Stream: {
            int per_block = 0;
            long long blocks = 0;
            csr_stream_geometry(m, &per_block, &blocks);
            const dim3 grid((unsigned)blocks);
            if (variant == CsrVariant::Adaptive)
                hipLaunchKernelGGL((csr_stream_kernel<256, 4, true>), grid, dim3(256), 0, stream, m, x, y, alpha, per_block, 1, (int)blocks, d_dot_partials);
            else
                hipLaunchKernelGGL((csr_stream_kernel<256, 4, false>), grid, dim3(256), 0, stream, m, x, y, alpha, per_block, 1, (int)blocks, d_dot_partials);
            break;
        }
        case CsrVariant::RowScalar:
            hipLaunchKernelGGL(csr_row_scalar_kernel, dim3(blocks_for(rows)), dim3(kBlock), 0, stream, m, x, y, alpha);
            break;
        default:
            hipLaunchKernelGGL(csr_wavefront_kernel, dim3((unsigned)((rows + kWavesPerBlock - 1) / kWavesPerBlock)), dim3(kBlock), 0, stream, m, x, y, alpha);
            break;
    }
}

void launch_ell_transpose(int rows, int width, const int* idx_rowmajor, const double* val_rowmajor,
                          int* idx_slotmajor, double* val_slotmajor, hipStream_t stream) {
    if (rows == 0) return;
    hipLaunchKernelGGL(ell_transpose_kernel, dim3(blocks_for(rows)), dim3(kBlock), 0, stream, rows,
                       width, idx_rowmajor, val_rowmajor, idx_slotmajor, val_slotmajor);
}

constexpr int kEllBlock = 256;

int ell_fused_dot_partials(int rows) { return (int)(((long long)rows + kEllBlock - 1) / kEllBlock); }

void launch_ell_spmv(int rows, int width, const int* idx, const double* val, const double* x,
                     double* y, double alpha, double beta, hipStream_t stream, int grid_hint,
                     double* d_dot_partials) {
    if (rows == 0) return;
    const int run = grid_hint > 0 ? xcd_run_group(grid_hint, kEllBlock, 7) + 1 : 8;
    const int blocks = ell_fused_dot_partials(rows);
    hipLaunchKernelGGL((ell_spmv_kernel<kEllBlock, true>), dim3((unsigned)xcd_padded_grid(blocks, run)), dim3(kEllBlock), 0, stream, rows,
                       width, idx, val, x, y, alpha, beta, run, blocks, d_dot_partials);
}

void launch_ell_stencil5_spmv(int rows, int width, int grid_size, const int* idx,
                              const double* val, const double* x, double* y, double alpha,
                              double beta, hipStream_t stream, double* d_dot_partials) {
    if (rows == 0) return;
    if (grid_size < 3 || (long long)grid_size * grid_size != rows) {
        launch_ell_spmv(rows, width, idx, val, x, y, alpha, beta, stream, 0, d_dot_partials);
        return;
    }
    const int run = xcd_run_group(grid_size, kEllBlock, 8);
    const int blocks = ell_fused_dot_partials(rows);
    hipLaunchKernelGGL((ell_stencil5_kernel<kEllBlock, true>), dim3((unsigned)xcd_padded_grid(blocks, run)), dim3(kEllBlock), 0, stream, rows,
                       width, grid_size, idx, val, x, y, alpha, beta, run, blocks, d_dot_partials);
}

}
```

### include/spmv_amd/lab.h

```cpp
#ifndef SPMV_AMD_LAB_H
#define SPMV_AMD_LAB_H

#include "spmv_amd/api.h"

#ifdef __cplusplus
extern "C" {
#endif

SpmvAmdCgSlab* spmv_amd_cg_slab_create_stencil5_as(int n, int as_rank, int as_world, SpmvAmdComm* comm);

int spmv_amd_cg_slab_set_option(SpmvAmdCgSlab* s, const char* name, long long value);

long long spmv_amd_cg_slab_tile_classes(const SpmvAmdCgSlab* s, unsigned char* out, long long cap);

long long spmv_amd_cg_slab_block_map(const SpmvAmdCgSlab* s, int which, unsigned char* out, long long cap);

typedef struct SpmvAmdPcgScalars {
    double rz;
    double pAp, alpha, beta;
    double b_norm;
    double residual;
    int iterations;
    int converged;
    int breakdown;
    int skip_update;
} SpmvAmdPcgScalars;

typedef struct SpmvAmdPcgStageArgs {
    size_t n;
    const double* b;
    const double* Ap;
    const double* dinv;
    double* r;
    double* p;
    double* x;
    double* partials;
    int count;
    int which;
    double tol;
    double* hist;
    int hist_cap;
} SpmvAmdPcgStageArgs;

int spmv_amd_pcg_stage(const char* stage, const char* kind, SpmvAmdPcgStageArgs* a, SpmvAmdPcgScalars* scalars);

int spmv_amd_pcg_last_step_launches(void);

typedef struct SpmvAmdMultiColumn {
    double rr_old;
    double pAp, alpha, beta;
    double b_norm;
    double residual;
    int active;
    int done;
    int iterations;
    int pad;
} SpmvAmdMultiColumn;

typedef struct SpmvAmdCgMultiStageArgs {
    const char* mode;
    size_t n;
    double* X;
    double* R;
    double* P;
    double* AP;
    SpmvAmdMultiColumn* cols;
    double* partials;
    long long count;
    int which;
    double tol;
    double* hist;
    int hist_cap;
    int xcd_run;
} SpmvAmdCgMultiStageArgs;

int spmv_amd_cg_multi_stage(const char* stage, int k, SpmvAmdCgMultiStageArgs* a);

#ifdef __cplusplus
}
#endif

#endif
```

Before: 212.7 CG iterations/s.

## Fuse CG direction update p = r + beta*p into the block SpMV kernel

Adds a kernel that computes the new search direction from r and the old p inside the row-LDS block SpMV. It writes p_out and computes Ap and the pAp partials in the same pass. Slow (non-uniform) blocks only write the direction and are finished afterwards by a second list-driven kernel over a precomputed slow-block list. The goal is to drop the separate AXPBY pass over p, saving one read and write of the vectors per iteration. In exchange the kernel needs more registers and launches an extra small kernel, and the path only turns on for single-rank ring-buffered slabs with few slow blocks.

```diff
diff --git a/cuda-spmv-benchmark_amd/binding.py b/cuda-spmv-benchmark_amd/binding.py
--- a/cuda-spmv-benchmark_amd/binding.py
+++ b/cuda-spmv-benchmark_amd/binding.py
@@ -117,7 +117,8 @@
     "spmv_amd_precond_inverse_diagonal", "spmv_amd_pcg_solve_device", "spmv_amd_pcg_last_history", "spmv_amd_pcg_release_workspace",
     "spmv_amd_precond_create_chebyshev", "spmv_amd_precond_chebyshev_info", "spmv_amd_precond_apply_device",
 ]
-LAB_ONLY_SYMBOLS = ["spmv_amd_cg_slab_create_stencil5_as", "spmv_amd_cg_slab_set_option", "spmv_amd_cg_slab_tile_classes", "spmv_amd_cg_slab_block_map", "spmv_amd_pcg_stage",
+LAB_ONLY_SYMBOLS = ["spmv_amd_cg_slab_create_stencil5_as", "spmv_amd_cg_slab_set_option", "spmv_amd_cg_slab_tile_classes", "spmv_amd_cg_slab_block_map", "spmv_amd_cg_slab_slow_blocks",
+                    "spmv_amd_cg_slab_direction_spmv", "spmv_amd_cg_slab_spmv_dot", "spmv_amd_pcg_stage",
                     "spmv_amd_pcg_last_step_launches", "spmv_amd_cg_multi_stage"]
 DECLARED_CXX_SYMBOLS = [
     "SPMV_CSR", "SPMV_STENCIL5_CSR", "SPMV_STENCIL_HALO_MGPU", "SPMV_ELLPACK", "SPMV_STENCIL5_ELLPACK",
@@ -210,6 +211,13 @@
         L.spmv_amd_cg_slab_tile_classes.restype = C.c_longlong
         L.spmv_amd_cg_slab_block_map.argtypes = [C.c_void_p, C.c_int, C.c_void_p, C.c_longlong]
         L.spmv_amd_cg_slab_block_map.restype = C.c_longlong
+        L.spmv_amd_cg_slab_slow_blocks.argtypes = [C.c_void_p, C.c_int, C.c_void_p, C.c_longlong]
+        L.spmv_amd_cg_slab_slow_blocks.restype = C.c_longlong
+        L.spmv_amd_cg_slab_direction_spmv.argtypes = [C.c_void_p, C.c_void_p, C.c_void_p, C.c_double, C.c_int, C.c_int, C.c_void_p, C.c_void_p,
+                                                      C.POINTER(C.c_double), C.c_void_p, C.c_int]
+        L.spmv_amd_cg_slab_direction_spmv.restype = C.c_int
+        L.spmv_amd_cg_slab_spmv_dot.argtypes = [C.c_void_p, C.POINTER(C.c_double), C.c_void_p, C.c_int]
+        L.spmv_amd_cg_slab_spmv_dot.restype = C.c_int
         L.spmv_amd_pcg_stage.argtypes = [C.c_char_p, C.c_char_p, C.POINTER(PcgStageArgs), C.POINTER(PcgScalars)]
         L.spmv_amd_pcg_stage.restype = C.c_int
         L.spmv_amd_pcg_last_step_launches.argtypes = []
@@ -862,6 +870,38 @@
         lib().spmv_amd_cg_slab_block_map(self.h, int(which), out.ctypes.data, count)
         return out
 
+    def slow_blocks(self, which):
+        if not is_lab():
+            raise RuntimeError("the slow-block lists are read through the LAB build only (binding.use_lab(), lib/libspmv_amd_lab.so)")
+        count = int(lib().spmv_amd_cg_slab_slow_blocks(self.h, int(which), None, 0))
+        out = np.zeros(max(count, 0), dtype=np.int32)
+        if count > 0:
+            lib().spmv_amd_cg_slab_slow_blocks(self.h, int(which), out.ctypes.data, count)
+        return out
+
+    def spmv_dot(self):
+        if not is_lab():
+            raise RuntimeError("the in-loop SpMV's sum is read through the LAB build only (binding.use_lab(), lib/libspmv_amd_lab.so)")
+        pAp = C.c_double(0.0)
+        count = lib().spmv_amd_cg_slab_spmv_dot(self.h, C.byref(pAp), None, 0)
+        partials = np.empty(count, dtype=np.float64)
+        lib().spmv_amd_cg_slab_spmv_dot(self.h, C.byref(pAp), partials.ctypes.data, count)
+        return partials, pAp.value
+
+    def direction_spmv(self, r, p_in, beta, iteration_matches=1, converged=0):
+        if not is_lab():
+            raise RuntimeError("the fused launch alone runs in the LAB build only (binding.use_lab(), lib/libspmv_amd_lab.so)")
+        r = np.ascontiguousarray(r, dtype=np.float64)
+        p_in = np.ascontiguousarray(p_in, dtype=np.float64)
+        p_out, Ap = np.empty_like(r), np.empty_like(r)
+        partials = np.empty(len(r), dtype=np.float64)
+        pAp = C.c_double(0.0)
+        used = lib().spmv_amd_cg_slab_direction_spmv(self.h, r.ctypes.data, p_in.ctypes.data, float(beta), int(iteration_matches), int(converged),
+                                                     p_out.ctypes.data, Ap.ctypes.data, C.byref(pAp), partials.ctypes.data, len(partials))
+        if used < 0:
+            raise RuntimeError("this slab cannot take the direction update inside the block SpMV (no block map, neighbours, or ring 1)")
+        return p_out, Ap, partials[:used], pAp.value
+
     def set_block_rows(self, rows):
         self.set_option("block_rows", rows)
 
diff --git a/cuda-spmv-benchmark_amd/csrc/cg_kernels.hip b/cuda-spmv-benchmark_amd/csrc/cg_kernels.hip
--- a/cuda-spmv-benchmark_amd/csrc/cg_kernels.hip
+++ b/cuda-spmv-benchmark_amd/csrc/cg_kernels.hip
@@ -2,6 +2,7 @@
 
 #include <stdlib.h>
 
+#include "direction_device.hpp"
 #include "reduce_device.hpp"
 #include "spmv_amd/hip_check.h"
 #include "stream_device.hpp"
@@ -197,9 +198,6 @@
     if (threadIdx.x == 0) partials[block] = acc;
 }
 
-__device__ __forceinline__ double direction(double r, double beta, double p, int fma_form) {
-    return fma_form ? fma(beta, p, r) : fma(1.0, r, beta * p);
-}
 
 __global__ __launch_bounds__(kStream) void cg_update_px_kernel(size_t n, const CgScalars* __restrict__ s,
                                                               const double* __restrict__ r,
diff --git a/cuda-spmv-benchmark_amd/csrc/cg_slab.hip b/cuda-spmv-benchmark_amd/csrc/cg_slab.hip
--- a/cuda-spmv-benchmark_amd/csrc/cg_slab.hip
+++ b/cuda-spmv-benchmark_amd/csrc/cg_slab.hip
@@ -5,6 +5,7 @@
 #include <algorithm>
 #include <atomic>
 #include <chrono>
+#include <limits>
 #include <mutex>
 #include <thread>
 #include <vector>
@@ -47,6 +48,9 @@
     double quintuple[5] = {0.0, 0.0, 0.0, 0.0, 0.0};
     bool stream_everywhere = false;
     unsigned char *block_map_whole = nullptr, *block_map_interior = nullptr;
+    int *slow_list_whole = nullptr, *slow_list_interior = nullptr;
+    int slow_count_whole = 0, slow_count_interior = 0;
+    int fused_direction = 1;
     bool spmv_with_dot = false;
     const SymPlanes* sym() const { return planes_on ? &planes : nullptr; }
     std::vector<double> placement;
@@ -195,6 +199,9 @@
     HIP_CHECK(hipStreamSynchronize(s->compute));
     device_release(s->block_map_whole);
     device_release(s->block_map_interior);
+    device_release(s->slow_list_whole);
+    device_release(s->slow_list_interior);
+    s->slow_count_whole = s->slow_count_interior = 0;
     if (s->tile_classes != nullptr) {
         const auto map_of = [&](const Stencil5Plan& p) -> unsigned char* {
             const int blocks = rowlds_block_tiles(p);
@@ -205,6 +212,26 @@
         s->block_map_whole = map_of(s->plan_whole);
         s->block_map_interior = map_of(s->plan_interior);
         HIP_CHECK(hipStreamSynchronize(s->compute));
+        const auto list_of = [&](const Stencil5Plan& p, const unsigned char* map, int* count) -> int* {
+            *count = 0;
+            if (map == nullptr) return nullptr;
+            std::vector<unsigned char> h((size_t)rowlds_block_tiles(p));
+            HIP_CHECK(hipMemcpy(h.data(), map, h.size(), hipMemcpyDeviceToHost));
+            std::vector<int> slow;
+            for (size_t b = 0; b < h.size(); ++b)
+                if (h[b] == 0) slow.push_back((int)b);
+            if (slow.empty()) return nullptr;
+            int* list = device_try_alloc<int>(slow.size());
+            if (list == nullptr) {
+                *count = -1;
+                return nullptr;
+            }
+            HIP_CHECK(hipMemcpy(list, slow.data(), slow.size() * sizeof(int), hipMemcpyHostToDevice));
+            *count = (int)slow.size();
+            return list;
+        };
+        s->slow_list_whole = list_of(s->plan_whole, s->block_map_whole, &s->slow_count_whole);
+        s->slow_list_interior = list_of(s->plan_interior, s->block_map_interior, &s->slow_count_interior);
     }
     attach_block_maps(s);
 }
@@ -320,6 +347,7 @@
         HIP_CHECK(hipMemset(s->d_alpha_ring, 0, kMaxRingSlots * sizeof(double)));
     }
     if (const char* v = getenv("SPMV_AMD_NO_OVERLAP")) s->no_overlap = v[0] == '1';
+    if (const char* v = getenv("SPMV_AMD_FUSED_DIRECTION")) s->fused_direction = v[0] == '1' ? 1 : 0;
 #ifdef SPMV_AMD_LAB
     if (const char* v = getenv("SPMV_AMD_TEST_WEDGE_OVERLAPPED_EXCHANGE")) s->test_wedge_overlapped_exchange = atoi(v);
 #endif
@@ -558,6 +586,24 @@
     return used;
 }
 
+bool direction_spmv_available(const SpmvAmdCgSlab* s, bool cap) {
+    const Stencil5Plan& p = s->plan_whole;
+    const SymPlanes* sp = s->sym();
+    if (s->op != nullptr || !s->fused_dot || sp == nullptr || sp->ce == nullptr || sp->cls == nullptr) return false;
+    if (p.variant != Stencil5Variant::RowLds || p.block_rows <= 0 || p.block_map == nullptr || s->slow_count_whole < 0) return false;
+    return !cap || 16LL * s->slow_count_whole <= rowlds_block_tiles(p);
+}
+
+int slab_direction_spmv(SpmvAmdCgSlab* s, const double* p_in, double* p_out, int iteration, hipEvent_t spmv_done = nullptr) {
+    s->spmv_split_at = -1;
+    const DirectionSpmv d{s->d_s, iteration, s->device_form, s->r, p_in, p_out, s->slow_list_whole, s->slow_count_whole};
+    const int used = launch_stencil5_direction_spmv(s->A.view, s->plan_whole, d, s->Ap, 1.0, s->partials_spmv, s->shape.reverse, s->compute, *s->sym());
+    if (s->tl_after_interior) HIP_CHECK(hipEventRecord(s->tl_after_interior, s->compute));
+    if (spmv_done) HIP_CHECK(hipEventRecord(spmv_done, s->compute));
+    reduce_spmv_partials(s, used, &s->d_s->pAp, &s->d_s->converged, s->spmv_progress, s->spmv_progress_value, s->reduce_mailbox);
+    return used;
+}
+
 const char* query_name(hipError_t e) {
     return e == hipSuccess ? "idle (all work done)" : e == hipErrorNotReady ? "busy (work pending)" : hipGetErrorString(e);
 }
@@ -642,6 +688,7 @@
     bool detail = false;
     bool pipeline = false;
     bool late = false;
+    bool fused_direction = false;
     int slots = 1;
     EdgeRows edges{0, 0, 0};
     size_t bulk_lo = 0, bulk_hi = 0;
@@ -658,7 +705,9 @@
     L.separate = L.reduce && L.mailbox == nullptr;
     L.detail = config->enable_detailed_timers != 0;
     L.slots = s->ring_slots;
-    L.late = s->late_bulk && !L.detail && L.slots > 1;
+    L.fused_direction = s->fused_direction != 0 && !L.multi && s->op == nullptr && L.slots > 1 && !L.detail &&
+                        direction_spmv_available(s, s->fused_direction != 2);
+    L.late = s->late_bulk && !L.detail && L.slots > 1 && !L.fused_direction;
     constexpr size_t kAlign = 512;
     const size_t head_rows = s->has_prev ? ((size_t)s->halo + kAlign - 1) / kAlign * kAlign : 0;
     const size_t tail_start = s->has_next ? (nl - (size_t)s->halo) / kAlign * kAlign : nl;
@@ -765,7 +814,10 @@
 extern "C" SpmvAmdCgSlab* spmv_amd_cg_slab_create(MatrixData* mat, SpmvAmdComm* comm) { return create_from_matrix(mat, comm, true); }
 
 extern "C" const char* spmv_amd_cg_slab_loop_shape(const SpmvAmdCgSlab* s) {
-    if (!s->comm->exchanges_halos()) return "single rank";
+    if (!s->comm->exchanges_halos()) {
+        const CGConfigMultiGPU any = {1, 0.0, 0, 0};
+        return loop_shape(s, &any).fused_direction ? "single rank: direction update inside the block SpMV" : "single rank";
+    }
     if (!s->no_overlap) {
         const CGConfigMultiGPU any = {1, 0.0, 0, 0};
         if (!loop_shape(s, &any).pipeline) return "plain: the in-place form (ring 1) or a slab too thin to split";
@@ -842,6 +894,7 @@
     int tl_exchanges = 0;
     bool halo_in_flight = false;
     bool step_in_direction = false;
+    const double* direction_from = nullptr;
     int sequence0 = 0, records_read = 0;
     bool backward = false;
     int enqueued = 0, sampled = 0;
@@ -995,12 +1048,16 @@
     s->spmv_progress = &s->h_poll->progress;
     s->spmv_progress_value = 4 * (s->poll_sequence + 1) + 1;
     mark(enqueued, 0);
+    const auto spmv = [&](hipEvent_t spmv_done) {
+        if (L.fused_direction && enqueued > 0) return slab_direction_spmv(s, direction_from, s->p, enqueued, spmv_done);
+        return slab_spmv(s, true, halo_in_flight, skip, nullptr, spmv_done);
+    };
     if (timeline) {
         s->tl_after_interior = tl_event(s->tl_compute, mark_index(enqueued, 1));
-        slab_spmv(s, true, halo_in_flight, skip, nullptr, tl_event(s->tl_compute, mark_index(enqueued, 2)));
+        spmv(tl_event(s->tl_compute, mark_index(enqueued, 2)));
         s->tl_after_interior = nullptr;
     } else if (L.detail) {
-        timed(&stats->time_spmv_ms, nullptr, [&] { slab_spmv(s, true, halo_in_flight, skip); });
+        timed(&stats->time_spmv_ms, nullptr, [&] { spmv(nullptr); });
     } else if (s->spmv_event_stride > 0 && (enqueued + s->spmv_event_phase) % s->spmv_event_stride == 0) {
         while (s->spmv_ev.size() < 2 * (size_t)(sampled + 1)) {
             hipEvent_t e;
@@ -1008,11 +1065,11 @@
             s->spmv_ev.push_back(e);
         }
         HIP_CHECK(hipEventRecord(s->spmv_ev[2 * sampled], s->compute));
-        slab_spmv(s, true, halo_in_flight, skip, nullptr, s->spmv_ev[2 * sampled + 1]);
+        spmv(s->spmv_ev[2 * sampled + 1]);
         sampled_iteration.push_back(enqueued);
         ++sampled;
     } else {
-        slab_spmv(s, true, halo_in_flight, skip);
+        spmv(nullptr);
     }
     s->spmv_progress = nullptr;
 }
@@ -1133,7 +1190,8 @@
             }
             trace.push("BLAS_AXPBY");
         };
-        if (L.pipeline) pieces(fused, plain);
+        if (L.fused_direction) direction_from = p_in;
+        else if (L.pipeline) pieces(fused, plain);
         else pieces(plain, plain);
         s->p = p_next;
     }
@@ -1390,6 +1448,10 @@
             if (p->variant == Stencil5Variant::RowLds) p->block_rows = (int)value;
         build_block_maps(s);
     }
+    else if (strcmp(name, "fused_direction") == 0) {
+        if (value < 0 || value > 2) return -1;
+        s->fused_direction = (int)value;
+    }
     else if (strcmp(name, "spmv_with_dot") == 0) s->spmv_with_dot = value != 0;
     else return -1;
     return 0;
@@ -1403,6 +1465,53 @@
     return count;
 }
 
+extern "C" long long spmv_amd_cg_slab_slow_blocks(const SpmvAmdCgSlab* s, int which, int* out, long long cap) {
+    const int* list = which == 0 ? s->slow_list_whole : s->slow_list_interior;
+    const long long count = which == 0 ? s->slow_count_whole : s->slow_count_interior;
+    if (count <= 0) return count;
+    if (out != nullptr && cap > 0) HIP_CHECK(hipMemcpy(out, list, (size_t)std::min(count, cap) * sizeof(int), hipMemcpyDeviceToHost));
+    return count;
+}
+
+extern "C" int spmv_amd_cg_slab_spmv_dot(const SpmvAmdCgSlab* s, double* pAp, double* partials, int cap) {
+    HIP_CHECK(hipStreamSynchronize(s->compute));
+    HIP_CHECK(hipMemcpy(pAp, &s->d_s->pAp, sizeof(double), hipMemcpyDeviceToHost));
+    const int count = s->plan_whole.partials;
+    if (partials != nullptr && cap > 0) HIP_CHECK(hipMemcpy(partials, s->partials_spmv, (size_t)std::min(count, cap) * sizeof(double), hipMemcpyDeviceToHost));
+    return count;
+}
+
+extern "C" int spmv_amd_cg_slab_direction_spmv(SpmvAmdCgSlab* s, const double* r, const double* p_in, double beta, int iteration_matches,
+                                               int converged, double* p_out, double* Ap, double* pAp, double* partials, int cap) {
+    if (s->ring.size() < 2 || s->comm->exchanges_halos() || !direction_spmv_available(s, false)) return -1;
+    const size_t nl = (size_t)s->n_local;
+    const int iteration = 3;
+    CgScalars sc;
+    memset(&sc, 0, sizeof sc);
+    sc.beta = beta;
+    sc.iterations = iteration;
+    sc.converged = converged != 0 ? 1 : 0;
+    sc.pAp = std::numeric_limits<double>::quiet_NaN();
+    HIP_CHECK(hipMemcpy(s->d_s, &sc, sizeof sc, hipMemcpyHostToDevice));
+    upload(s->r, r, nl);
+    upload(s->ring[0], p_in, nl);
+    HIP_CHECK(hipMemsetAsync(s->ring[1], 0xFF, nl * sizeof(double), s->compute));
+    HIP_CHECK(hipMemsetAsync(s->Ap, 0xFF, nl * sizeof(double), s->compute));
+    HIP_CHECK(hipMemsetAsync(s->partials_spmv, 0xFF, (size_t)s->plan_whole.partials * sizeof(double), s->compute));
+    s->shape.reverse = false;
+    s->reduce_mailbox = nullptr;
+    const int used = slab_direction_spmv(s, s->ring[0], s->ring[1], iteration_matches != 0 ? iteration : iteration + 1);
+    HIP_CHECK(hipStreamSynchronize(s->compute));
+    HIP_CHECK(hipGetLastError());
+    download(p_out, s->ring[1], nl);
+    download(Ap, s->Ap, nl);
+    if (partials != nullptr && cap > 0) download(partials, s->partials_spmv, (size_t)std::min(used, cap));
+    HIP_CHECK(hipMemcpy(&sc, s->d_s, sizeof sc, hipMemcpyDeviceToHost));
+    *pAp = sc.pAp;
+    s->p = s->ring[0];
+    return used;
+}
+
 extern "C" long long spmv_amd_cg_slab_tile_classes(const SpmvAmdCgSlab* s, unsigned char* out, long long cap) {
     if (s->tile_classes == nullptr) return 0;
     const long long count = (long long)s->tile_class_count;
@@ -1420,10 +1529,24 @@
 extern "C" int spmv_amd_cg_slab_time_spmv(SpmvAmdCgSlab* s, int reps, float* ms_each) {
     HIP_CHECK(hipMemsetAsync(&s->d_s->converged, 0, sizeof(int), s->compute));
     EventTimer t;
+    const CGConfigMultiGPU any = {1, 0.0, 0, 0};
+    const bool fused = loop_shape(s, &any).fused_direction;
+    if (fused) {
+        CgScalars sc;
+        memset(&sc, 0, sizeof sc);
+        sc.beta = 0.5, sc.iterations = 1;
+        HIP_CHECK(hipMemcpyAsync(s->d_s, &sc, sizeof sc, hipMemcpyHostToDevice, s->compute));
+        HIP_CHECK(hipStreamSynchronize(s->compute));
+    }
     for (int i = 0; i < reps; ++i) {
         t.begin(s->compute);
-        (void)launch_stencil5_spmv(s->A.view, s->plan_whole, s->p, s->Ap, 1.0, s->fused_dot ? s->partials_spmv : nullptr,
-                                   nullptr, false, s->compute, nullptr, s->sym());
+        if (fused) {
+            const DirectionSpmv d{s->d_s, 1, s->device_form, s->r, s->ring[0], s->ring[1], s->slow_list_whole, s->slow_count_whole};
+            (void)launch_stencil5_direction_spmv(s->A.view, s->plan_whole, d, s->Ap, 1.0, s->partials_spmv, false, s->compute, *s->sym());
+        } else {
+            (void)launch_stencil5_spmv(s->A.view, s->plan_whole, s->p, s->Ap, 1.0, s->fused_dot ? s->partials_spmv : nullptr,
+                                       nullptr, false, s->compute, nullptr, s->sym());
+        }
         t.end(s->compute);
         ms_each[i] = t.elapsed_ms();
     }
@@ -1445,6 +1568,8 @@
     device_release(s->tile_classes);
     device_release(s->block_map_whole);
     device_release(s->block_map_interior);
+    device_release(s->slow_list_whole);
+    device_release(s->slow_list_interior);
     s->planes_on = false;
     s->r = s->Ap = s->p_alloc = s->p = nullptr;
     s->ring_alloc.clear();
diff --git a/cuda-spmv-benchmark_amd/csrc/direction_device.hpp b/cuda-spmv-benchmark_amd/csrc/direction_device.hpp
--- /dev/null
+++ b/cuda-spmv-benchmark_amd/csrc/direction_device.hpp
@@ -0,0 +1,11 @@
+#pragma once
+
+#include <hip/hip_runtime.h>
+
+namespace spmv_amd {
+
+__device__ __forceinline__ double direction(double r, double beta, double p, int fma_form) {
+    return fma_form ? fma(beta, p, r) : fma(1.0, r, beta * p);
+}
+
+}
diff --git a/cuda-spmv-benchmark_amd/csrc/kernels.hpp b/cuda-spmv-benchmark_amd/csrc/kernels.hpp
--- a/cuda-spmv-benchmark_amd/csrc/kernels.hpp
+++ b/cuda-spmv-benchmark_amd/csrc/kernels.hpp
@@ -90,6 +90,19 @@
 int launch_stencil5_spmv(const SlabCsr& m, const Stencil5Plan& plan, const double* x, double* y, double alpha,
                          double* d_dot_partials, const int* d_skip_flag, bool reverse, hipStream_t stream,
                          const ResidualOut* init = nullptr, const SymPlanes* planes = nullptr);
+struct CgScalars;
+struct DirectionSpmv {
+    const CgScalars* s;
+    int iteration;
+    bool fma_form;
+    const double* r;
+    const double* p_in;
+    double* p_out;
+    const int* slow_list;
+    int slow_count;
+};
+int launch_stencil5_direction_spmv(const SlabCsr& m, const Stencil5Plan& plan, const DirectionSpmv& d, double* y, double alpha,
+                                   double* d_dot_partials, bool reverse, hipStream_t stream, const SymPlanes& planes);
 int launch_stencil5_cheb_step(const SlabCsr& m, const Stencil5Plan& plan, const double* z, const ChebStep& step, double* d_dot_partials,
                               const int* d_skip_flag, hipStream_t stream);
 int launch_stencil5_spmv(const SlabCsr& m, const double* x, double* y, double alpha,
diff --git a/cuda-spmv-benchmark_amd/csrc/spmv_kernels.hip b/cuda-spmv-benchmark_amd/csrc/spmv_kernels.hip
--- a/cuda-spmv-benchmark_amd/csrc/spmv_kernels.hip
+++ b/cuda-spmv-benchmark_amd/csrc/spmv_kernels.hip
@@ -4,6 +4,7 @@
 
 #include <type_traits>
 
+#include "direction_device.hpp"
 #include "reduce_device.hpp"
 #include "stencil_geometry.hpp"
 #include "stencil_row_device.hpp"
@@ -309,6 +310,25 @@
     if (kMode != 0 && threadIdx.x == 0) dot_partials[tile] = dot;
 }
 
+__device__ __forceinline__ bool rowlds_block_slow_rows(const SlabCsr& m, const double* __restrict__ x, double* __restrict__ y, double alpha,
+                                                       int gi_lo, int gi_hi, int gfirst, int col_tiles, int li0, int block_rows, int col_tile, int j0, int lane, int skip,
+                                                       double* __restrict__ lds, double* __restrict__ dot_partials, const SymPlanes& sp) {
+    double* __restrict__ strip = lds;
+    double* __restrict__ xrow = lds + 5 * kLdsTileCols;
+    const ResidualOut none{nullptr, nullptr, nullptr};
+    const int held = gi_hi - li0 < block_rows ? gi_hi - li0 : block_rows;
+#pragma unroll 1
+    for (int r = 0; r < held; ++r) {
+        const int li = li0 + r;
+        const int uniform = rowlds_tile_class(sp, li, col_tiles, col_tile);
+        double dot = 0.0;
+        if (!rowlds_tile<1, false, true>(m, x, y, alpha, li, gfirst + li, j0, lane, skip, strip, xrow, none, &dot, sp, uniform)) return false;
+        if (lane == 0) dot_partials[(li - gi_lo) * col_tiles + col_tile] = dot;
+        wave_lds_sync();
+    }
+    return true;
+}
+
 template <int kRows>
 __global__ __launch_bounds__(64) void stencil5_rowlds_block_kernel(
     SlabCsr m, const double* __restrict__ x, double* __restrict__ y, double alpha, int gi_lo, int gi_hi, int gfirst, int col_tiles,
@@ -377,20 +397,112 @@
             if (lane == 0) dot_partials[(li - gi_lo) * col_tiles + col_tile] = dot;
         }
     } else {
-        double* __restrict__ strip = lds;
-        double* __restrict__ xrow = lds + 5 * kLdsTileCols;
-        const ResidualOut none{nullptr, nullptr, nullptr};
+        rowlds_block_slow_rows(m, x, y, alpha, gi_lo, gi_hi, gfirst, col_tiles, li0, kRows, col_tile, j0, lane, skip, lds, dot_partials, sp);
+    }
+}
+
+template <int kRows>
+__global__ __launch_bounds__(64) void stencil5_direction_block_kernel(
+    SlabCsr m, const CgScalars* __restrict__ s, int iteration, int fma_form, const double* __restrict__ rvec, const double* __restrict__ p_in,
+    double* __restrict__ p_out, double* __restrict__ y, double alpha, int gi_lo, int gi_hi, int col_tiles, int total_blocks, int run, int reverse,
+    double* __restrict__ dot_partials, const unsigned char* __restrict__ block_map, SymPlanes sp) {
+    constexpr int kRowDoubles = kLdsTileCols + 2;
+    __shared__ double lds[kRows * kRowDoubles];
+    if (s->iterations != iteration || s->converged != 0) return;
+    const double beta = s->beta;
+    const int block = rowlds_tile_of_block((int)blockIdx.x, run, total_blocks, reverse);
+    if (block < 0) return;
+    const int row_block = block / col_tiles;
+    const int col_tile = block - row_block * col_tiles;
+    const int li0 = gi_lo + row_block * kRows;
+    const int j0 = col_tile * kLdsTileCols, lane = (int)threadIdx.x;
+    const int n = m.grid_size;
+    const int fast = (int)block_map[block];
+    const int rows = m.n_local / n;
+    const bool in0 = j0 + lane < n, in1 = j0 + lane + 64 < n;
+    double rv[kRows + 2][2], pv[kRows + 2][2];
+    double ro[kRows], po[kRows];
+#pragma unroll
+    for (int r = 0; r < kRows + 2; ++r) {
+        const int li = li0 - 1 + r;
+        rv[r][0] = rv[r][1] = pv[r][0] = pv[r][1] = 0.0;
+        if (li >= 0 && li < rows) {
+            const double* __restrict__ rr = rvec + ((long long)li * n + j0);
+            const double* __restrict__ pr = p_in + ((long long)li * n + j0);
+            if (in0) rv[r][0] = rr[lane], pv[r][0] = pr[lane];
+            if (in1) rv[r][1] = rr[lane + 64], pv[r][1] = pr[lane + 64];
+        }
+    }
+    const bool outer = (lane == 0 && j0 > 0) || (lane == 63 && j0 + kLdsTileCols < n);
+    const int outer_col = lane == 0 ? -1 : kLdsTileCols + lane - 63;
+#pragma unroll
+    for (int r = 0; r < kRows; ++r) {
+        const int li = li0 + r;
+        ro[r] = po[r] = 0.0;
+        if (li < rows && outer) {
+            const long long at = (long long)li * n + j0 + outer_col;
+            ro[r] = rvec[at], po[r] = p_in[at];
+        }
+    }
+    if (__builtin_amdgcn_readfirstlane(fast) != 0) {
+#pragma unroll
+        for (int r = 0; r < kRows + 2; ++r) {
+            pv[r][0] = in0 ? direction(rv[r][0], beta, pv[r][0], fma_form) : 0.0;
+            pv[r][1] = in1 ? direction(rv[r][1], beta, pv[r][1], fma_form) : 0.0;
+        }
+#pragma unroll
+        for (int r = 0; r < kRows; ++r) {
+            po[r] = outer ? direction(ro[r], beta, po[r], fma_form) : 0.0;
+            double* __restrict__ out = p_out + ((long long)(li0 + r) * n + j0);
+            if (in0) out[lane] = pv[r + 1][0];
+            if (in1) out[lane + 64] = pv[r + 1][1];
+            lds[r * kRowDoubles + 1 + lane] = pv[r + 1][0];
+            lds[r * kRowDoubles + 65 + lane] = pv[r + 1][1];
+        }
+        wave_lds_sync();
+#pragma unroll
+        for (int r = 0; r < kRows; ++r) {
+            const int li = li0 + r;
+            double xw[2], xe[2];
+            tile_west_east(lds + r * kRowDoubles, lane, j0, n, po[r], po[r], xw, xe);
+            double dot = 0.0;
+#pragma unroll
+            for (int h = 0; h < 2; ++h) {
+                const int j = j0 + lane + 64 * h;
+                if (j < n) {
+                    const double xc = pv[r + 1][h], xn = pv[r][h], xs = pv[r + 2][h];
+                    const double sum = stencil5_row(j, n, sp.w, xw[h], sp.c, xc, sp.e, xe[h], sp.n, xn, sp.s5, xs);
+                    dot = fma(xc, sum, dot);
+                    __builtin_nontemporal_store(alpha * sum, y + ((long long)li * n + j));
+                }
+            }
+            dot = wave_sum(dot);
+            if (lane == 0) dot_partials[(li - gi_lo) * col_tiles + col_tile] = dot;
+        }
+    } else {
         const int held = gi_hi - li0 < kRows ? gi_hi - li0 : kRows;
-#pragma unroll 1
-        for (int r = 0; r < held; ++r) {
-            const int li = li0 + r;
-            const int uniform = rowlds_tile_class(sp, li, col_tiles, col_tile);
-            double dot = 0.0;
-            if (!rowlds_tile<1, false, true>(m, x, y, alpha, li, gfirst + li, j0, lane, skip, strip, xrow, none, &dot, sp, uniform)) return;
-            if (lane == 0) dot_partials[(li - gi_lo) * col_tiles + col_tile] = dot;
-            wave_lds_sync();
-        }
-    }
+#pragma unroll
+        for (int r = 0; r < kRows; ++r) {
+            if (r < held) {
+                double* __restrict__ out = p_out + ((long long)(li0 + r) * n + j0);
+                if (in0) out[lane] = direction(rv[r + 1][0], beta, pv[r + 1][0], fma_form);
+                if (in1) out[lane + 64] = direction(rv[r + 1][1], beta, pv[r + 1][1], fma_form);
+            }
+        }
+    }
+}
+
+__global__ __launch_bounds__(64) void stencil5_block_list_kernel(SlabCsr m, const CgScalars* __restrict__ s, int iteration,
+                                                                 const double* __restrict__ x, double* __restrict__ y, double alpha, int gi_lo,
+                                                                 int gi_hi, int gfirst, int col_tiles, int block_rows, const int* __restrict__ list,
+                                                                 double* __restrict__ dot_partials, SymPlanes sp) {
+    __shared__ double lds[5 * kLdsTileCols + kLdsTileCols + 2];
+    if (s->iterations != iteration || s->converged != 0) return;
+    const int block = list[blockIdx.x];
+    const int row_block = block / col_tiles;
+    const int col_tile = block - row_block * col_tiles;
+    const int li0 = gi_lo + row_block * block_rows;
+    rowlds_block_slow_rows(m, x, y, alpha, gi_lo, gi_hi, gfirst, col_tiles, li0, block_rows, col_tile, col_tile * kLdsTileCols, (int)threadIdx.x, 0, lds, dot_partials, sp);
 }
 
 __global__ __launch_bounds__(kBlock) void block_map_kernel(const unsigned char* __restrict__ cls, int col_tiles, int gi_lo, int gi_hi,
@@ -1050,6 +1162,28 @@
     return dot ? p.partials : 0;
 }
 
+int launch_stencil5_direction_spmv(const SlabCsr& m, const Stencil5Plan& p, const DirectionSpmv& d, double* y, double alpha,
+                                   double* d_dot_partials, bool reverse, hipStream_t stream, const SymPlanes& sp) {
+    const int blocks = rowlds_block_tiles(p);
+    if (blocks <= 0 || p.block_map == nullptr || d_dot_partials == nullptr || sp.cls == nullptr || (d.slow_count > 0 && d.slow_list == nullptr)) {
+        fprintf(stderr, "[spmv] the direction update inside the SpMV exists for row-lds plans with a block map only\n");
+        exit(EXIT_FAILURE);
+    }
+    const dim3 grid((unsigned)xcd_padded_grid(blocks, p.xcd_run));
+    const int gfirst = m.row_offset / m.grid_size;
+#define SPMV_AMD_LAUNCH_DIRECTION_BLOCK(ROWS)                                                                                          \
+    hipLaunchKernelGGL((stencil5_direction_block_kernel<ROWS>), grid, dim3(64), 0, stream, m, d.s, d.iteration, d.fma_form ? 1 : 0, d.r, \
+                       d.p_in, d.p_out, y, alpha, p.gi_lo, p.gi_hi, p.row_blocks, blocks, p.xcd_run, reverse ? 1 : 0, d_dot_partials,    \
+                       p.block_map, sp)
+    if (p.block_rows == 4) SPMV_AMD_LAUNCH_DIRECTION_BLOCK(4);
+    else SPMV_AMD_LAUNCH_DIRECTION_BLOCK(8);
+#undef SPMV_AMD_LAUNCH_DIRECTION_BLOCK
+    if (d.slow_count > 0)
+        hipLaunchKernelGGL(stencil5_block_list_kernel, dim3((unsigned)d.slow_count), dim3(64), 0, stream, m, d.s, d.iteration, d.p_out, y, alpha,
+                           p.gi_lo, p.gi_hi, gfirst, p.row_blocks, p.block_rows, d.slow_list, d_dot_partials, sp);
+    return p.partials;
+}
+
 int launch_stencil5_cheb_step(const SlabCsr& m, const Stencil5Plan& p, const double* z, const ChebStep& step, double* d_dot_partials,
                               const int* d_skip_flag, hipStream_t stream) {
     if (p.variant != Stencil5Variant::RowLds || p.last_row <= p.first_row) return -1;
diff --git a/include/spmv_amd/lab.h b/include/spmv_amd/lab.h
--- a/include/spmv_amd/lab.h
+++ b/include/spmv_amd/lab.h
@@ -14,6 +14,13 @@
 long long spmv_amd_cg_slab_tile_classes(const SpmvAmdCgSlab* s, unsigned char* out, long long cap);
 
 long long spmv_amd_cg_slab_block_map(const SpmvAmdCgSlab* s, int which, unsigned char* out, long long cap);
+
+long long spmv_amd_cg_slab_slow_blocks(const SpmvAmdCgSlab* s, int which, int* out, long long cap);
+
+int spmv_amd_cg_slab_spmv_dot(const SpmvAmdCgSlab* s, double* pAp, double* partials, int cap);
+
+int spmv_amd_cg_slab_direction_spmv(SpmvAmdCgSlab* s, const double* r, const double* p_in, double beta, int iteration_matches, int converged,
+                                    double* p_out, double* Ap, double* pAp, double* partials, int cap);
 
 typedef struct SpmvAmdPcgScalars {
     double rz;
```

After: 228.5 CG iterations/s, median of 6. 1.07x the previous value.
